# solomontesema/yolo-fpga-accelerator

Measured on AMD Instinct MI355X. Metric: YOLOv2 INT16 416x416 frames/sec, higher is better.
Workload: dtype int16

## Files before the change

### include/yolo2_hip.h

```cpp
#ifndef YOLO2_HIP_H
#define YOLO2_HIP_H

#include <stddef.h>
#include <stdint.h>

#ifdef __cplusplus
extern "C" {
#endif

#define YOLO2_SUCCESS     0
#define YOLO2_ERROR      -1
#define YOLO2_TIMEOUT    -2
#define YOLO2_INIT_ERROR -3
#define YOLO2_MMAP_ERROR -4
#define YOLO2_DMA_ERROR  -5


int  yolo2_accel_init(void);
void yolo2_accel_cleanup(void);
int  yolo2_hip_select_device(int device);
int  yolo2_hip_device_count(void);
const char *yolo2_hip_last_error(void);

void yolo2_set_q_values(int32_t qw, int32_t qa_in, int32_t qa_out, int32_t qb);
int  yolo2_is_busy(void);
int  yolo2_is_done(void);
int  yolo2_wait_for_completion(uint32_t timeout_ms);

uint32_t yolo2_get_status(void);
uint32_t yolo2_read_reg(uint32_t offset);
void     yolo2_write_reg(uint32_t offset, uint32_t value);
long yolo2_hip_driver_calls(void);

int yolo2_execute_conv_layer(uint64_t input_addr, uint64_t output_addr, uint64_t weight_addr,
                             uint64_t beta_addr, int ifm_num, int ofm_num, int ksize, int kstride,
                             int input_w, int input_h, int output_w, int output_h, int padding,
                             int is_nl, int is_bn, int tm, int tn, int tr, int tc, int ofm_num_bound,
                             int mloopsxTM, int mloops_a1xTM, int layer_type, int qw, int qa_in,
                             int qa_out, int qb, uint32_t timeout_ms);

int yolo2_execute_maxpool_layer(uint64_t input_addr, uint64_t output_addr, int channels, int ksize,
                                int kstride, int input_w, int input_h, int output_w, int output_h,
                                int padding, int tm, int tr, int tc, int ofm_num_bound, int mloopsxTM,
                                int mloops_a1xTM, uint32_t timeout_ms);

int yolo2_hip_last_layer_path(void);
int yolo2_hip_last_layer_edge(void);

int yolo2_execute_conv_layer_f32(uint64_t input_addr, uint64_t output_addr, uint64_t weight_addr,
                                 uint64_t beta_addr, int ifm_num, int ofm_num, int ksize, int kstride,
                                 int input_w, int input_h, int output_w, int output_h, int padding,
                                 int is_nl, uint32_t timeout_ms);

#ifndef DMA_BUFFER_MANAGER_H
typedef struct {
    void *ptr;
    size_t size;
    uint64_t phys_addr;
} memory_buffer_t;
typedef struct {
    void *virt_addr;
    uint64_t phys_addr;
    size_t size;
    int fd;
    char device_name[64];
} dma_buffer_t;
#endif
int      dma_buffer_init(void);
void     dma_buffer_cleanup(void);
int      dma_buffer_alloc(size_t size, dma_buffer_t *buffer);
void     dma_buffer_free(dma_buffer_t *buffer);
void     dma_buffer_sync_for_device(dma_buffer_t *buffer, size_t offset, size_t size);
void     dma_buffer_sync_for_cpu(dma_buffer_t *buffer, size_t offset, size_t size);
uint64_t dma_buffer_get_phys(dma_buffer_t *buffer, size_t offset);
int      memory_allocate_ddr(size_t size, size_t alignment, memory_buffer_t *buffer);
void     memory_free_ddr(memory_buffer_t *buffer);
int      memory_allocate_weights(size_t size, memory_buffer_t *buffer);
int      memory_allocate_bias(size_t size, memory_buffer_t *buffer);
int      memory_allocate_inference_buffer(memory_buffer_t *buffer);
uint64_t memory_get_phys_addr(void *virt_addr);
void     memory_flush_cache(void *addr, size_t size);
void     memory_invalidate_cache(void *addr, size_t size);

int  yolo2_hip_alloc(size_t bytes, uint64_t *dev_addr);
void yolo2_hip_free(uint64_t dev_addr);
int  yolo2_hip_memcpy_h2d(uint64_t dst, const void *src, size_t bytes);
int  yolo2_hip_memcpy_d2h(void *dst, uint64_t src, size_t bytes);
int  yolo2_hip_memset(uint64_t dst, int value, size_t bytes);


typedef struct yolo2_hip_ctx yolo2_hip_ctx;

#define YOLO2_N_CONV       23
#define YOLO2_N_WEIGHTS    50941792
#define YOLO2_N_BIAS       10761
#define YOLO2_REGION_ELEMS (425 * 13 * 13)
#define YOLO2_FRAME_ELEMS  (3 * 416 * 416)

int  yolo2_hip_create(int device, yolo2_hip_ctx **ctx);
void yolo2_hip_destroy(yolo2_hip_ctx *ctx);
int  yolo2_hip_ctx_device(yolo2_hip_ctx *ctx);
int  yolo2_hip_alloc_on(yolo2_hip_ctx *ctx, size_t bytes, uint64_t *dev_addr);

int yolo2_hip_load_weights_int16(yolo2_hip_ctx *ctx, const int16_t *weights_reorg, size_t n_weights,
                                 const int16_t *bias, size_t n_bias, const int32_t *weight_q,
                                 int n_weight_q, const int32_t *bias_q, int n_bias_q,
                                 const int32_t *act_q, int n_act_q);
int yolo2_hip_load_weights_int16_dev(yolo2_hip_ctx *ctx, uint64_t weights_reorg_dev, size_t n_weights,
                                     uint64_t bias_dev, size_t n_bias, const int32_t *weight_q,
                                     int n_weight_q, const int32_t *bias_q, int n_bias_q,
                                     const int32_t *act_q, int n_act_q);

int yolo2_hip_layer_path(yolo2_hip_ctx *ctx, int conv_ordinal);
int yolo2_hip_layer_path_counts(yolo2_hip_ctx *ctx, int conv_ordinal, int counts[5]);

int yolo2_hip_set_batch(yolo2_hip_ctx *ctx, int batch);

int yolo2_hip_run_batch_int16(yolo2_hip_ctx *ctx, uint64_t frames_dev, int batch,
                              uint64_t region_dev, int *final_q, void *stream);

int yolo2_hip_run_batch_int16_host(yolo2_hip_ctx *ctx, const float *frames, int batch,
                                   int16_t *region, int *final_q);

int yolo2_hip_run_frames_int16(yolo2_hip_ctx *ctx, const float *frames, int n_frames, int batch,
                               int16_t *region, int *final_q);

int yolo2_hip_load_weights_fp32(yolo2_hip_ctx *ctx, const float *weights_reorg, size_t n_weights,
                                const float *bias, size_t n_bias);
int yolo2_hip_load_weights_fp32_dev(yolo2_hip_ctx *ctx, uint64_t weights_reorg_dev, size_t n_weights,
                                    uint64_t bias_dev, size_t n_bias);
int yolo2_hip_run_batch_fp16(yolo2_hip_ctx *ctx, uint64_t frames_dev, int batch, uint64_t region_dev,
                             void *stream);
int yolo2_hip_run_batch_fp16_host(yolo2_hip_ctx *ctx, const float *frames, int batch, float *region);
const char *yolo2_hip_fp16_layer_kernel(yolo2_hip_ctx *ctx, int layer_idx);
int yolo2_hip_f16_store_check(int store, int pool, int B, int H, int W, int Cp_out, int out_ch_off, int n_store, int dst_B,
                              int dst_H, int dst_W, int dst_Cp);

int yolo2_hip_debug_layer_output(yolo2_hip_ctx *ctx, int layer_idx, int frame, int16_t *out,
                                 size_t capacity_elems, size_t *out_elems);

int yolo2_hip_debug_f16_tensor(yolo2_hip_ctx *ctx, int split, int layer_idx, int frame, int which, uint16_t *out,
                               size_t capacity_halves, int *geom);

int yolo2_hip_set_profiling(yolo2_hip_ctx *ctx, int enable);
int yolo2_hip_layer_times_ms(yolo2_hip_ctx *ctx, float *ms32 );

int yolo2_hip_num_lanes(yolo2_hip_ctx *ctx);
int yolo2_hip_num_lanes_fp16(yolo2_hip_ctx *ctx);
int yolo2_hip_set_fp16_lanes(yolo2_hip_ctx *ctx, int lanes);

int yolo2_hip_run_batch_f32tol(yolo2_hip_ctx *ctx, uint64_t frames_dev, int batch, uint64_t region_dev, void *stream);
int yolo2_hip_run_batch_f32tol_host(yolo2_hip_ctx *ctx, const float *frames, int batch, float *region);
const char *yolo2_hip_f32tol_layer_kernel(yolo2_hip_ctx *ctx, int layer_idx);
int yolo2_hip_num_lanes_f32tol(yolo2_hip_ctx *ctx);

int yolo2_hip_layer_pool_fused(yolo2_hip_ctx *ctx, int layer_idx);

int yolo2_hip_conv_launch_info(yolo2_hip_ctx *ctx, int conv_ordinal, int *grid_x, int *grid_y,
                               int *block, int *lds_bytes, int *pixels_per_lane);

int yolo2_hip_conv_plan_string(yolo2_hip_ctx *ctx, int conv_ordinal, char *buf, int cap);
int yolo2_hip_plan_source(yolo2_hip_ctx *ctx);

int yolo2_hip_set_option(yolo2_hip_ctx *ctx, const char *name, const char *value);
int yolo2_hip_options_string(yolo2_hip_ctx *ctx, char *buf, int cap);

int yolo2_hip_set_plan_cache(yolo2_hip_ctx *ctx, const char *path);
int yolo2_hip_plan_cache_info(yolo2_hip_ctx *ctx, uint64_t *weights_hash, int *bounds_from_file, int *n_lines, int *n_batches);
int yolo2_hip_plan_cache_check(const char *path, uint64_t weights_hash, int *n_lines);

int yolo2_hip_i16_plan_check(int splits, int cg_out, int npix, size_t cap_bytes);
size_t yolo2_hip_ks_scratch_bytes(yolo2_hip_ctx *ctx);
int yolo2_hip_i16_edge_map(int B, int H, int W, int cap, int *tile_cls, int *tile_mask, int *pix, long long *steps);

int yolo2_hip_run_frame_fp32_host(yolo2_hip_ctx *ctx, const float *frame, float *region);

int yolo2_hip_run_batch_fp32(yolo2_hip_ctx *ctx, uint64_t frames_dev, int batch, uint64_t region_dev, void *stream);
int yolo2_hip_run_batch_fp32_host(yolo2_hip_ctx *ctx, const float *frames, int batch, float *region);

int yolo2_hip_letterbox_u8(uint64_t image_dev, int w, int h, int channels, uint64_t frame_dev,
                           int net_w, int net_h, void *stream);

int yolo2_hip_run_images_u8_host(yolo2_hip_ctx *ctx, const uint8_t *const *images, const int *widths,
                                 const int *heights, int channels, int n, int batch,
                                 int16_t *region_host, int *final_q);

typedef struct {
    int frame, det, cls;
    float prob, x, y, w, h;
} yolo2_hip_det;
int yolo2_hip_postprocess_int16(yolo2_hip_ctx *ctx, uint64_t region_dev, int batch, int final_q, const int *im_w,
                                const int *im_h, float thresh, float nms, yolo2_hip_det *dets, int cap_per_frame,
                                int *counts, float *rows, int *totals, float *proc, void *stream);
int yolo2_hip_postprocess_f32(yolo2_hip_ctx *ctx, uint64_t region_dev, int batch, const int *im_w, const int *im_h,
                              float thresh, float nms, yolo2_hip_det *dets, int cap_per_frame, int *counts,
                              float *rows, int *totals, float *proc, void *stream);

#define YOLO2_DETS_BEST_CLASS 1
int yolo2_hip_run_images_u8_dets(yolo2_hip_ctx *ctx, const uint8_t *const *images, const int *widths, const int *heights,
                                 int channels, int n, int batch, float thresh, float nms, int flags, yolo2_hip_det *dets,
                                 int cap_per_frame, int *counts, int *final_q);

int yolo2_hip_run_images_u8_f16_host(yolo2_hip_ctx *ctx, int split, const uint8_t *const *images, const int *widths,
                                     const int *heights, int channels, int n, int batch, float *region_host);
int yolo2_hip_run_images_u8_dets_f16(yolo2_hip_ctx *ctx, int split, const uint8_t *const *images, const int *widths,
                                     const int *heights, int channels, int n, int batch, float thresh, float nms, int flags,
                                     yolo2_hip_det *dets, int cap_per_frame, int *counts);
const char *yolo2_hip_images_layer0_kernel(yolo2_hip_ctx *ctx, int split);

enum { YOLO2_PIX_GREY8 = 1, YOLO2_PIX_RGB24 = 3, YOLO2_PIX_YUYV = 0x56595559  };
int yolo2_hip_letterbox_pix(uint64_t image_dev, int w, int h, int pixfmt, uint64_t frame_dev, int net_w, int net_h, void *stream);
int yolo2_hip_run_images_pix_host(yolo2_hip_ctx *ctx, const uint8_t *const *images, const int *widths, const int *heights,
                                  int pixfmt, int n, int batch, int16_t *region_host, int *final_q);
int yolo2_hip_run_images_pix_dets(yolo2_hip_ctx *ctx, const uint8_t *const *images, const int *widths, const int *heights,
                                  int pixfmt, int n, int batch, float thresh, float nms, int flags, yolo2_hip_det *dets,
                                  int cap_per_frame, int *counts, int *final_q);
int yolo2_hip_run_images_pix_f16_host(yolo2_hip_ctx *ctx, int split, const uint8_t *const *images, const int *widths,
                                      const int *heights, int pixfmt, int n, int batch, float *region_host);
int yolo2_hip_run_images_pix_dets_f16(yolo2_hip_ctx *ctx, int split, const uint8_t *const *images, const int *widths,
                                      const int *heights, int pixfmt, int n, int batch, float thresh, float nms, int flags,
                                      yolo2_hip_det *dets, int cap_per_frame, int *counts);


int yolo2_hip_shard_range(int total, int rank, int world, int *lo, int *hi);

typedef struct yolo2_hip_multi yolo2_hip_multi;
int  yolo2_hip_multi_create(const int *devices, int n_devices, yolo2_hip_multi **m);
void yolo2_hip_multi_destroy(yolo2_hip_multi *m);
int  yolo2_hip_multi_num_devices(yolo2_hip_multi *m);
int  yolo2_hip_multi_uses_rccl(yolo2_hip_multi *m);
yolo2_hip_ctx *yolo2_hip_multi_ctx(yolo2_hip_multi *m, int i);
int  yolo2_hip_multi_load_weights_int16(yolo2_hip_multi *m, const int16_t *weights_reorg, size_t n_weights,
                                        const int16_t *bias, size_t n_bias, const int32_t *weight_q, int n_weight_q,
                                        const int32_t *bias_q, int n_bias_q, const int32_t *act_q, int n_act_q);
int  yolo2_hip_multi_load_weights_fp32(yolo2_hip_multi *m, const float *weights_reorg, size_t n_weights,
                                       const float *bias, size_t n_bias);
int  yolo2_hip_multi_run_frames_int16(yolo2_hip_multi *m, const float *frames, int n_frames, int batch_per_device,
                                      int16_t *region, int *final_q);
int  yolo2_hip_multi_run_images_u8_host(yolo2_hip_multi *m, const uint8_t *const *images, const int *widths,
                                        const int *heights, int channels, int n, int batch_per_device,
                                        int16_t *region_host, int *final_q);

int  yolo2_hip_multi_run_images_u8_dets(yolo2_hip_multi *m, const uint8_t *const *images, const int *widths, const int *heights,
                                        int channels, int n, int batch_per_device, float thresh, float nms, int flags,
                                        yolo2_hip_det *dets, int cap_per_frame, int *counts, int *final_q);
int  yolo2_hip_multi_run_images_u8_dets_f16(yolo2_hip_multi *m, int split, const uint8_t *const *images, const int *widths,
                                            const int *heights, int channels, int n, int batch_per_device, float thresh, float nms,
                                            int flags, yolo2_hip_det *dets, int cap_per_frame, int *counts);
int  yolo2_hip_multi_run_images_pix_host(yolo2_hip_multi *m, const uint8_t *const *images, const int *widths,
                                         const int *heights, int pixfmt, int n, int batch_per_device,
                                         int16_t *region_host, int *final_q);
int  yolo2_hip_multi_run_images_pix_dets(yolo2_hip_multi *m, const uint8_t *const *images, const int *widths, const int *heights,
                                         int pixfmt, int n, int batch_per_device, float thresh, float nms, int flags,
                                         yolo2_hip_det *dets, int cap_per_frame, int *counts, int *final_q);
int  yolo2_hip_multi_run_images_pix_dets_f16(yolo2_hip_multi *m, int split, const uint8_t *const *images, const int *widths,
                                             const int *heights, int pixfmt, int n, int batch_per_device, float thresh, float nms,
                                             int flags, yolo2_hip_det *dets, int cap_per_frame, int *counts);

int  yolo2_hip_rccl_unique_id(void *id128);
int  yolo2_hip_rccl_init_rank(yolo2_hip_ctx *ctx, int device, const void *id128, int nranks, int rank);
void yolo2_hip_rccl_finalize(yolo2_hip_ctx *ctx);
int  yolo2_hip_load_weights_int16_bcast(yolo2_hip_ctx *ctx, const int16_t *weights_reorg, size_t n_weights,
                                        const int16_t *bias, size_t n_bias, const int32_t *weight_q, int n_weight_q,
                                        const int32_t *bias_q, int n_bias_q, const int32_t *act_q, int n_act_q, int root);
int  yolo2_hip_load_weights_fp32_bcast(yolo2_hip_ctx *ctx, const float *weights_reorg, size_t n_weights,
                                       const float *bias, size_t n_bias, int root);

typedef struct {
    int nranks, rank, device;
    int version;
    int bcasts;
    double last_bcast_ms;
    uint64_t last_bcast_bytes;
    char lib_path[256];
} yolo2_hip_rccl_info_t;
int  yolo2_hip_rccl_info(yolo2_hip_ctx *ctx, yolo2_hip_rccl_info_t *out);
int  yolo2_hip_multi_rccl_info(yolo2_hip_multi *m, yolo2_hip_rccl_info_t *out);


int yolo2_hip_num_layers(void);
int yolo2_hip_layer_desc(int layer_idx, int desc[9]);

long yolo2_strip_int16_layer_pad(const int16_t *file, size_t file_elems, const int *layer_len,
                                 int n_layers, int16_t *dst);
extern const int yolo2_weight_len[YOLO2_N_CONV];
extern const int yolo2_bias_len[YOLO2_N_CONV];

#ifdef __cplusplus
}
#endif
#endif
```

### yolo-fpga-accelerator_amd/csrc/conv_common.hpp

```cpp
#pragma once
#include <hip/hip_runtime.h>
#include <cstdint>
#include <type_traits>

#include "layout.hpp"

namespace y2 {

typedef short short2_t __attribute__((ext_vector_type(2)));

struct ConvArgs {
    int B, H, W, Wp, PL;
    int CGin;
    int CGout;
    int npix;
    long in_cg_stride;
    long out_cg_stride;
    long out_base;
    int shift, round;
    int sh_right, sh_left;
    int bs_right, bs_left, bs_mag;
    int leaky;
    int lt_max;
    int xcd_remap;
    const int *mb_list;
    int nwin;
    int oWp, oPL;
    long pool_cg_stride;
    long pool_base;
    unsigned mHW, sHW, mW, sW, mOHW, sOHW, mOW, sOW;
    int ks_S, ks_Q, ks_mb;
    int *ks_trip;
    int edge;
    int e_nt, e_nb;
    int e_band[4];
    int e_int;
    int e_n[5];
    int e_rem[6];
    unsigned mH2, sH2, mW2, sW2, mI2, sI2;
};

inline void set_conv_div(ConvArgs &a)
{
    auto one = [](unsigned d, unsigned &m, unsigned &s) { if (d < 2) { m = 0; s = 32; } else fast_div_magic(d, m, s); };
    one((unsigned)(a.H * a.W), a.mHW, a.sHW);
    one((unsigned)a.W, a.mW, a.sW);
    one((unsigned)((a.H / 2) * (a.W / 2)), a.mOHW, a.sOHW);
    one((unsigned)(a.W / 2), a.mOW, a.sOW);
}
__device__ __forceinline__ int div_c(int n, unsigned m, unsigned s) { return s >= 32 ? n : (int)fast_div((unsigned)n, m, s); }

__device__ __forceinline__ int leaky_i16(int v)
{
    const unsigned u = (unsigned)(-v);
    const int q = (int)((u * 52429u) >> 19);
    return v < 0 ? -q : v;
}

__device__ __forceinline__ int clamp16(int v) { return min(max(v, -32768), 32767); }

__device__ __forceinline__ long shift64(long v, int right, int left, int mag, long round)
{
    if (right) return (v + round) >> mag;
    if (left) return (long)((unsigned long)v << mag);
    return v;
}

__device__ __forceinline__ int flat_of(const ConvArgs &a, int q)
{
    const int b = div_c(q, a.mHW, a.sHW);
    const int r = q - b * (a.H * a.W);
    const int y = div_c(r, a.mW, a.sW);
    const int x = r - y * a.W;
    return b * a.PL + (y + 1) * a.Wp + x;
}

enum { kEdgeTop = 0, kEdgeBottom = 1, kEdgeLeft = 2, kEdgeRight = 3, kEdgeInterior = 4, kEdgeMixed = 5 };

__host__ __device__ constexpr int edge_class_mask(int cls)
{
    return cls == kEdgeTop ? 0x1f8 : cls == kEdgeBottom ? 0x03f : cls == kEdgeLeft ? 0x1b6 : cls == kEdgeRight ? 0x0db : 0x1ff;
}

__host__ __device__ inline unsigned edge_div(unsigned n, unsigned m, unsigned s)
{
    if (s >= 32) return n;
    const unsigned t = (unsigned)(((unsigned long long)m * n) >> 32);
    return (t + ((n - t) >> 1)) >> s;
}

__host__ __device__ inline int edge_tile_class(const ConvArgs &a, int tile, int &ct)
{
    const unsigned nb = (unsigned)a.e_nb, nt = (unsigned)a.e_nt;
    const int c0 = (int)((unsigned)tile * nb / nt), c1 = (int)((unsigned)(tile + 1) * nb / nt);
    if (c1 > c0) {
        int c = 0;
        while (c < 3 && c0 >= a.e_band[c]) ++c;
        ct = c0 - (c ? a.e_band[c - 1] : 0);
        return c;
    }
    const int o = tile - c0;
    if (o < a.e_int) { ct = o; return kEdgeInterior; }
    ct = o - a.e_int;
    return kEdgeMixed;
}

__host__ __device__ inline bool edge_lane_pixel(const ConvArgs &a, int cls, int ct, int lane, int &b, int &y, int &x)
{
    int i = ct * 64 + lane;
    bool valid = true;
    if (cls == kEdgeMixed) {
        const int nm = a.e_rem[5];
        valid = i < nm;
        if (!valid) i = nm - 1;
        int c = 0;
        while (c < 4 && i >= a.e_rem[c + 1]) ++c;
        i = a.e_n[c] - (a.e_rem[c + 1] - a.e_rem[c]) + (i - a.e_rem[c]);
        cls = c;
    }
    if (cls == kEdgeTop || cls == kEdgeBottom) {
        b = (int)edge_div((unsigned)i, a.mW, a.sW);
        x = i - b * a.W;
        y = cls == kEdgeTop ? 0 : a.H - 1;
    } else if (cls == kEdgeLeft || cls == kEdgeRight) {
        b = (int)edge_div((unsigned)i, a.mH2, a.sH2);
        y = 1 + i - b * (a.H - 2);
        x = cls == kEdgeLeft ? 0 : a.W - 1;
    } else {
        b = (int)edge_div((unsigned)i, a.mI2, a.sI2);
        const int r = i - b * ((a.H - 2) * (a.W - 2));
        const int yy = (int)edge_div((unsigned)r, a.mW2, a.sW2);
        y = 1 + yy;
        x = 1 + r - yy * (a.W - 2);
    }
    return valid;
}

constexpr int kEdgeGatherItems = 3 * 64 * 3;

__host__ __device__ inline void edge_band_patch(const ConvArgs &a, int cls, int &org, int &Lf, int &pitch)
{
    const bool rows = cls == kEdgeTop || cls == kEdgeBottom;
    Lf = rows ? 2 * a.Wp + 1 : 2 * a.H;
    pitch = rows ? a.Wp : 2;
    org = cls == kEdgeTop ? a.Wp - 1 : cls == kEdgeBottom ? (a.H - 1) * a.Wp - 1 : cls == kEdgeLeft ? a.Wp : a.Wp + a.W - 2;
}

inline int edge_tiles_plan(ConvArgs &a)
{
    a.edge = 0;
    if (a.H < 3 || a.W < 3) return 0;
    const long B = a.B, H = a.H, W = a.W;
    const long n[5] = {B * W, B * W, B * (H - 2), B * (H - 2), B * (H - 2) * (W - 2)};
    if (n[4] + 2 * n[0] + 2 * n[2] >= (1L << 30)) return 0;
    a.e_rem[0] = 0;
    int nb = 0;
    for (int c = 0; c < 5; ++c) {
        a.e_n[c] = (int)n[c];
        a.e_rem[c + 1] = a.e_rem[c] + (int)(n[c] % 64);
        if (c < 4) { nb += (int)(n[c] / 64); a.e_band[c] = nb; }
    }
    a.e_int = (int)(n[4] / 64);
    a.e_nb = nb;
    a.e_nt = nb + a.e_int + (a.e_rem[5] + 63) / 64;
    if ((unsigned long long)a.e_nt * (unsigned long long)(a.e_nb + 1) >= (1ULL << 32)) return 0;
    auto magic = [](unsigned d, unsigned &m, unsigned &s) { if (d < 2) { m = 0; s = 32; } else fast_div_magic(d, m, s); };
    magic((unsigned)(H - 2), a.mH2, a.sH2);
    magic((unsigned)(W - 2), a.mW2, a.sW2);
    magic((unsigned)((H - 2) * (W - 2)), a.mI2, a.sI2);
    int lt = kEdgeGatherItems;
    for (int c = kEdgeTop; c <= kEdgeRight; ++c) {
        int org, Lf, pitch;
        edge_band_patch(a, c, org, Lf, pitch);
        for (int t = 0; t < a.e_band[c] - (c ? a.e_band[c - 1] : 0); ++t) {
            int b0, b1, y, x;
            edge_lane_pixel(a, c, t, 0, b0, y, x);
            edge_lane_pixel(a, c, t, 63, b1, y, x);
            lt = lt > (b1 - b0 + 1) * Lf ? lt : (b1 - b0 + 1) * Lf;
        }
    }
    for (int t = 0; t < a.e_int; ++t) {
        int b0, y0, x0, b1, y1, x1;
        edge_lane_pixel(a, kEdgeInterior, t, 0, b0, y0, x0);
        edge_lane_pixel(a, kEdgeInterior, t, 63, b1, y1, x1);
        const int f0 = b0 * a.PL + (y0 + 1) * a.Wp + x0, f1 = b1 * a.PL + (y1 + 1) * a.Wp + x1;
        lt = lt > f1 - f0 + 1 + 2 * (a.Wp + 1) ? lt : f1 - f0 + 1 + 2 * (a.Wp + 1);
    }
    a.edge = 1;
    return lt;
}

inline long edge_tiles_steps(const ConvArgs &a)
{
    return 64L * (6L * a.e_nb + 9L * (a.e_nt - a.e_nb));
}

__device__ inline void xcd_partition(int xm_log2, int &tile, int &yb)
{
    const int gx = gridDim.x, gy = gridDim.y, total = gx * gy;
    const int lin = blockIdx.x + blockIdx.y * gx;
    const int xcd = lin & 7, slot = lin >> 3;
    const int q = total >> 3, r = total & 7;
    int L = xcd * q + min(xcd, r) + slot;
    const int Xm = 1 << xm_log2, Xt = 8 >> xm_log2;
    const int qt = gx / Xt, rt = gx - qt * Xt, qm = gy / Xm, rm = gy - qm * Xm;
    tile = 0; yb = 0;
    for (int k = 0; k < 8; ++k) {
        const int kt = k >> xm_log2, km = k & (Xm - 1);
        const int nt = qt + (kt < rt), nm = qm + (km < rm), cnt = nt * nm;
        if (L < cnt) {
            const int dt = L / nm;
            tile = kt * qt + min(kt, rt) + dt;
            yb = km * qm + min(km, rm) + (L - dt * nm);
            break;
        }
        L -= cnt;
    }
}

template <typename T>
__global__ void k_repack_weights(const T *__restrict__ src, T *__restrict__ dst, int C, int N, int KK)
{
    const int CG = (C + kTn - 1) / kTn, MB = (N + kTm - 1) / kTm;
    const long n = (long)MB * CG * KK * 128;
    const long t = (long)blockIdx.x * blockDim.x + threadIdx.x;
    if (t >= n) return;
    const int tn = (int)(t & 3), tm = (int)((t >> 2) & 31);
    const long r = t >> 7;
    const int tap = (int)(r % KK);
    const int cg = (int)((r / KK) % CG);
    const int mb = (int)(r / ((long)KK * CG));
    const int m0 = mb * kTm, n0 = cg * kTn;
    const int tm_min = min(kTm, N - m0), tn_min = min(kTn, C - n0);
    T v = 0;
    if (tm < tm_min && tn < tn_min)
        v = src[(long)m0 * C * KK + (long)tm_min * n0 * KK + (long)tap * tm_min * tn_min + tm * tn_min + tn];
    dst[t] = v;
}

template <typename T>
__global__ void k_pool_ref(const T *__restrict__ in, T *__restrict__ out, int C, int K, int stride, int W, int H,
                           int OW, int OH, T padv)
{
    const int t = blockIdx.x * blockDim.x + threadIdx.x;
    if (t >= C * OH * OW) return;
    const int x = t % OW, y = (t / OW) % OH, c = t / (OW * OH);
    const int W8 = (W + 7) & ~7, OW8 = (OW + 7) & ~7;
    T best = padv;
    for (int i = 0; i < K; ++i)
        for (int j = 0; j < K; ++j) {
            const int sy = y * stride + i, sx = x * stride + j;
            const T v = (sy < H && sx < W) ? in[((long)c * H + sy) * W8 + sx] : padv;
            if (v > best) best = v;
        }
    out[((long)c * OH + y) * OW8 + x] = best;
}

}
```

### yolo-fpga-accelerator_amd/csrc/kernels_int16.hpp

```cpp
#pragma once

#include "conv_common.hpp"
#include "layout.hpp"

namespace y2 {


__device__ __forceinline__ int stepA(int acc, const int2 x, const int2 w, const int r, const int s)
{
    int d = __builtin_amdgcn_sdot2(__builtin_bit_cast(short2_t, x.x), __builtin_bit_cast(short2_t, w.x), r, false);
    d = __builtin_amdgcn_sdot2(__builtin_bit_cast(short2_t, x.y), __builtin_bit_cast(short2_t, w.y), d, false);
    return clamp16(acc + (d >> s));
}

__device__ __forceinline__ void stepC4(int &acc01, int &acc23, const int2 x, const int2 w0, const int2 w1, const int2 w2,
                                       const int2 w3, const int r, const int s)
{
    int t0, t1, t2, t3;
    asm("v_dot2_i32_i16 %2, %6, %14, %16\n\t"
        "v_dot2_i32_i16 %3, %7, %14, %16\n\t"
        "v_dot2_i32_i16 %4, %8, %14, %16\n\t"
        "v_dot2_i32_i16 %5, %9, %14, %16\n\t"
        "v_dot2_i32_i16 %2, %10, %15, %2\n\t"
        "v_dot2_i32_i16 %3, %11, %15, %3\n\t"
// ... 95 lines not shown

__device__ __forceinline__ long step64(long acc, int2 x, int2 w, const ConvArgs &a)
{
    const int x0 = (short)(x.x & 0xffff), x1 = x.x >> 16, x2 = (short)(x.y & 0xffff), x3 = x.y >> 16;
    const int w0 = (short)(w.x & 0xffff), w1 = w.x >> 16, w2 = (short)(w.y & 0xffff), w3 = w.y >> 16;
    const long p = (long)(w0 * x0) + (long)(w1 * x1) + (long)(w2 * x2) + (long)(w3 * x3);
    long v = acc + shift64(p, a.sh_right, a.sh_left, a.shift, a.sh_right && a.shift > 0 ? (1L << (a.shift - 1)) : 0);
    v = v > 32767 ? 32767 : v;
    v = v < -32768 ? -32768 : v;
    return v;
}



#ifndef PREX_MAX_P
#define PREX_MAX_P 2
#endif
#ifndef Y2_I16_ABL
#define Y2_I16_ABL 0
#endif
template <int KS, int P, int MODE, int NST, int GRP = 1, bool EDGE = false>
__global__ __launch_bounds__(256, 2) void k_conv_i16(const int2 *__restrict__ in, int2 *__restrict__ out,
                                                   const int2 *__restrict__ wpk,
                                                   const short *__restrict__ bias, const ConvArgs a)
{
    static_assert(!EDGE || (KS == 3 && P == 1 && GRP == 1 && (MODE == 3 || MODE == 4)), "edge-class tiles: forms C / D, P = 1, 3x3");
    extern __shared__ int2 lds[];
    constexpr bool X64 = MODE == 2;
    typedef typename std::conditional<X64, long, int>::type acc_t;
    constexpr int T = 64 * P;
    constexpr int KT = KS * KS;
    constexpr int KK = KT * GRP;
    constexpr int PFG = KS == 1 ? GRP : 1;
    static_assert(GRP == 1 || KS == 1 || (KS == 3 && GRP == 2), "grouping: 1x1 convs (8 groups per barrier); 3x3 with 2 groups works but measured slower, not launched");
    const int tid = threadIdx.x;
    const int lane = tid & 63;
    const int wave = __builtin_amdgcn_readfirstlane(tid >> 6);
    int tile = blockIdx.x, yb = blockIdx.y;
    if (a.xcd_remap) xcd_partition(a.xcd_remap - 1, tile, yb);
    const int mb = a.mb_list ? a.mb_list[yb] : yb;
    const int halo = (KS == 3) ? a.Wp + 1 : 0;
    int fo[P];
    int rowaddr[P][KS];
    bool valid[P];
    int tile_start, Lt;
    int ecls = kEdgeInterior;
    int soff[NST], loff[NST];
    if (EDGE) {
        int ct, b, y, x;
        ecls = edge_tile_class(a, tile, ct);
        valid[0] = edge_lane_pixel(a, ecls, ct, lane, b, y, x);
        fo[0] = b * a.PL + (y + 1) * a.Wp + x;
        if (ecls == kEdgeInterior) {
            const int fmin = __builtin_amdgcn_readfirstlane(fo[0]), fmax = __builtin_amdgcn_readlane(fo[0], 63);
            tile_start = fmin - halo;
            Lt = min(fmax - fmin + 1 + 2 * halo, a.lt_max);
            const int lo = fo[0] - tile_start;
#pragma unroll
            for (int i = 0; i < KS; ++i) rowaddr[0][i] = (lo + (i - 1) * a.Wp - 1) * 8;
#pragma unroll
            for (int k = 0; k < NST; ++k) { soff[k] = tile_start + tid + k * 256; loff[k] = tid + k * 256; }
        } else if (ecls != kEdgeMixed) {
            const int b0 = __builtin_amdgcn_readfirstlane(b), b1 = __builtin_amdgcn_readlane(b, 63);
            const bool rows = ecls == kEdgeTop || ecls == kEdgeBottom;
            int org, Lf, pitch;
            edge_band_patch(a, ecls, org, Lf, pitch);
            tile_start = 0;
            Lt = min((b1 - b0 + 1) * Lf, a.lt_max);
            const int lo = (b - b0) * Lf + (rows ? fo[0] - b * a.PL - org : 2 * y + (ecls == kEdgeRight));
#pragma unroll
            for (int i = 0; i < KS; ++i) rowaddr[0][i] = (lo + (i - 1) * pitch - 1) * 8;
#pragma unroll
            for (int k = 0; k < NST; ++k) {
                const int s_ = tid + k * 256, fr = s_ / Lf, r_ = s_ - fr * Lf;
                soff[k] = (b0 + fr) * a.PL + org + (rows ? r_ : (r_ >> 1) * a.Wp + (r_ & 1));
                loff[k] = s_;
            }
        } else {
            tile_start = 0;
            Lt = kEdgeGatherItems;
#pragma unroll
            for (int i = 0; i < KS; ++i) rowaddr[0][i] = (i * 64 + lane) * 3 * 8;
#pragma unroll
            for (int k = 0; k < NST; ++k) {
                const int t = wave + 4 * k, ti = t / 3, tj = t - 3 * ti;
                soff[k] = fo[0] + (ti - 1) * a.Wp + (tj - 1);
                loff[k] = (ti * 64 + lane) * 3 + tj;
            }
        }
    } else {
        const int q0 = tile * T;
        const int qlast = min(q0 + T, a.npix) - 1;
        const int fmin = flat_of(a, q0);
        const int fmax = flat_of(a, qlast);
        tile_start = fmin - halo;
        Lt = min(fmax - fmin + 1 + 2 * halo, a.lt_max);
#pragma unroll
        for (int p = 0; p < P; ++p) {
            const int q = q0 + p * 64 + lane;
            valid[p] = q <= qlast;
            fo[p] = flat_of(a, min(q, qlast));
            const int lo = fo[p] - tile_start;
#pragma unroll
            for (int i = 0; i < KS; ++i)
                rowaddr[p][i] = (KS == 3) ? (lo + (i - 1) * a.Wp - 1) * 8 : lo * 8;
        }
    }

    acc_t acc[P][8];
    {
        const short *bp = bias + mb * 32 + wave * 8;
#pragma unroll
        for (int m = 0; m < 8; ++m) {
            acc_t b0;
            if (X64) {
                b0 = (acc_t)shift64((long)bp[m], a.bs_right, a.bs_left, a.bs_mag,
                                    a.bs_right && a.bs_mag > 0 ? (1L << (a.bs_mag - 1)) : 0);
            } else {
                const int b = bp[m];
                b0 = a.bs_right ? (acc_t)((b + (a.bs_mag > 0 ? (1 << (a.bs_mag - 1)) : 0)) >> a.bs_mag)
                                : (a.bs_left ? (acc_t)(b << a.bs_mag) : (acc_t)b);
                if (MODE == 1) b0 = (acc_t)(((int)b0 << a.shift) + a.round);
            }
#pragma unroll
            for (int p = 0; p < P; ++p) acc[p][m] = b0;
        }
        if (MODE == 5) {
#pragma unroll
            for (int p = 0; p < P; ++p)
#pragma unroll
                for (int m = 0; m < 8; ++m) acc[p][m] = (acc_t)((int)acc[p][m] << 16);
        }
        if (MODE == 3 || MODE == 4) {
            int pk[4];
#pragma unroll
            for (int j = 0; j < 4; ++j) pk[j] = ((int)acc[0][2 * j] & 0xffff) | ((int)acc[0][2 * j + 1] << 16);
#pragma unroll
            for (int p = 0; p < P; ++p)
#pragma unroll
                for (int j = 0; j < 4; ++j) acc[p][j] = (acc_t)pk[j];
        }
    }

    const int r = a.round, s = a.shift;
    const int nmask = ~((1 << s) - 1), lo_b = (int)(0xffff8000u << s) + r, hi_b = (32767 << s) + r;
    int r_vgpr = r;
    if (MODE != 2) asm volatile("" : "+v"(r_vgpr));
    const char *lds_b = reinterpret_cast<const char *>(lds);
    const int2 *src = in + kLead + (EDGE ? 0 : tile_start);
    const int2 *wq = wpk + ((long)mb * a.CGin * KT * 32 + wave * 8);

    int2 stage[NST];
    const int buf_items = a.lt_max * GRP;
    auto src_off = [&](int i) -> long { if (GRP == 1) return i; const int g = i / Lt; return (long)g * a.in_cg_stride + (i - g * Lt); };
    auto lds_off = [&](int i) -> int { if (GRP == 1) return i; const int g = i / Lt; return g * a.lt_max + (i - g * Lt); };
    const int LtG = Lt * GRP;
#pragma unroll
    for (int k = 0; k < NST; ++k) {
        const int i = tid + k * 256;
        if (i < LtG) stage[k] = src[EDGE ? soff[k] : src_off(i)];
    }
#pragma unroll
    for (int k = 0; k < NST; ++k) {
        const int i = tid + k * 256;
        if (i < LtG) lds[EDGE ? loff[k] : lds_off(i)] = stage[k];
    }
    __syncthreads();

    int chain = 0;
#if (Y2_I16_ABL & 8)
    int2 abl_w[8];
#pragma unroll
    for (int m = 0; m < 8; ++m) abl_w[m] = wq[m];
#endif
#if (Y2_I16_ABL & 16)
    int2 abl_x = lds[tid & 63];
#endif
    const int niter = a.CGin / GRP;
    auto group_loop = [&](auto mask_c) __attribute__((always_inline)) {
    constexpr int MASK = decltype(mask_c)::value;
    for (int cg = 0; cg < niter; ++cg) {
        src += (cg + 1 < niter) ? a.in_cg_stride * GRP : 0;
#if !(Y2_I16_ABL & 2)
#pragma unroll
        for (int k = 0; k < NST; ++k) {
            const int i = tid + k * 256;
            if (i < LtG) stage[k] = src[EDGE ? soff[k] : src_off(i)];
        }
#endif
        const char *tile = lds_b + (cg & 1) * buf_items * 8;
        constexpr bool PREX = (MODE == 3 || MODE == 4 || MODE == 5) && P <= PREX_MAX_P;
        auto xaddr = [&](int t, int p) -> const int2 * {
            return reinterpret_cast<const int2 *>(tile + (t / KT) * (a.lt_max * 8) + rowaddr[p][(t % KT) / KS] + ((t % KT) % KS) * 8);
        };
#pragma unroll
        for (int gb = 0; gb < GRP / PFG; ++gb) {
        int2 xv[PREX ? KT * PFG : 1][P];
        if (PREX && !(Y2_I16_ABL & 16)) {
#pragma unroll
            for (int tt = 0; tt < KT * PFG; ++tt)
#pragma unroll
                for (int p = 0; p < P; ++p) if ((MASK >> (tt % KT)) & 1) xv[tt][p] = *xaddr(gb * KT * PFG + tt, p);
        }
#pragma unroll
        for (int tt = 0; tt < KT * PFG; ++tt) {
            if (!((MASK >> (tt % KT)) & 1)) continue;
            const int tap = gb * KT * PFG + tt;
            int2 w[8];
#if (Y2_I16_ABL & 8)
#pragma unroll
            for (int m = 0; m < 8; ++m) { w[m] = abl_w[m]; asm volatile("" : "+s"(w[m].x), "+s"(w[m].y)); }
#else
#pragma unroll
            for (int m = 0; m < 8; ++m) w[m] = wq[tap * 32 + m];
#endif
#pragma unroll
            for (int p = 0; p < P; ++p) {
                int2 x;
#if (Y2_I16_ABL & 16)
                x = abl_x; asm volatile("" : "+v"(x.x), "+v"(x.y));
#else
                if (PREX) x = xv[tt][p];
                else x = *xaddr(tap, p);
#endif
                if (MODE == 0) asm volatile("" : "+v"(x.x) : "v"(chain));
                if (MODE == 5) {
                    int ae[8];
#pragma unroll
                    for (int m = 0; m < 8; ++m) ae[m] = (int)acc[p][m];
                    stepE8(ae, x, w, r_vgpr);
#pragma unroll
                    for (int m = 0; m < 8; ++m) acc[p][m] = (acc_t)ae[m];
                } else if (MODE == 4) {
                    int a01 = (int)acc[p][0], a23 = (int)acc[p][1], a45 = (int)acc[p][2], a67 = (int)acc[p][3];
                    stepD8(a01, a23, a45, a67, x, w, r_vgpr, 0x07060302);
                    acc[p][0] = (acc_t)a01; acc[p][1] = (acc_t)a23; acc[p][2] = (acc_t)a45; acc[p][3] = (acc_t)a67;
                } else if (MODE == 3) {
                    int a01 = (int)acc[p][0], a23 = (int)acc[p][1], a45 = (int)acc[p][2], a67 = (int)acc[p][3];
                    stepC4(a01, a23, x, w[0], w[1], w[2], w[3], r_vgpr, s);
                    stepC4(a45, a67, x, w[4], w[5], w[6], w[7], r_vgpr, s);
                    acc[p][0] = (acc_t)a01; acc[p][1] = (acc_t)a23; acc[p][2] = (acc_t)a45; acc[p][3] = (acc_t)a67;
                } else
#pragma unroll
                for (int m = 0; m < 8; ++m) {
                    if (MODE == 2) acc[p][m] = (acc_t)step64((long)acc[p][m], x, w[m], a);
                    else if (MODE == 1) acc[p][m] = (acc_t)stepB((int)acc[p][m], x, w[m], nmask, r_vgpr, lo_b, hi_b);
                    else acc[p][m] = (acc_t)stepA((int)acc[p][m], x, w[m], r_vgpr, s);
                }
                if (MODE == 0) chain = (int)acc[p][7];
            }
            if (MODE == 0) __builtin_amdgcn_sched_barrier(0);
        }
        }
#if !(Y2_I16_ABL & 2)
        {
            int2 *nxt = lds + ((cg + 1) & 1) * buf_items;
#pragma unroll
            for (int k = 0; k < NST; ++k) {
                const int i = tid + k * 256;
                if (i < LtG) nxt[EDGE ? loff[k] : lds_off(i)] = stage[k];
            }
        }
#endif
#if !(Y2_I16_ABL & 1)
        wq += KK * 32;
#else
        asm volatile("" : "+s"(wq));
#endif
#if !(Y2_I16_ABL & 4)
        __syncthreads();
#endif
    }
    };
    if (!EDGE) {
        group_loop(std::integral_constant<int, 0x1ff>());
    } else {
        switch (ecls) {
        case kEdgeTop: group_loop(std::integral_constant<int, edge_class_mask(kEdgeTop)>()); break;
        case kEdgeBottom: group_loop(std::integral_constant<int, edge_class_mask(kEdgeBottom)>()); break;
        case kEdgeLeft: group_loop(std::integral_constant<int, edge_class_mask(kEdgeLeft)>()); break;
        case kEdgeRight: group_loop(std::integral_constant<int, edge_class_mask(kEdgeRight)>()); break;
        default: group_loop(std::integral_constant<int, 0x1ff>()); break;
        }
    }

#pragma unroll
    for (int g = 0; g < 2; ++g) {
        const int cgo = mb * 8 + wave * 2 + g;
        if (cgo >= a.CGout) continue;
        int2 *dst = out + a.out_base + (long)cgo * a.out_cg_stride;
#pragma unroll
        for (int p = 0; p < P; ++p) {
            int v[4];
#pragma unroll
            for (int t = 0; t < 4; ++t) {
                int e = (int)acc[p][g * 4 + t];
                if (MODE == 1) e >>= s;
                if (MODE == 5) e >>= 16;
                if (MODE == 3 || MODE == 4) {
                    const int pr = (int)acc[p][(g * 4 + t) >> 1];
                    e = (t & 1) ? (pr >> 16) : (int)(short)(pr & 0xffff);
                }
                v[t] = a.leaky ? leaky_i16(e) : e;
            }
            int2 o;
            o.x = (v[0] & 0xffff) | (v[1] << 16);
            o.y = (v[2] & 0xffff) | (v[3] << 16);
            if (valid[p]) dst[fo[p]] = o;
        }
    }
}

template <int KS, int P, int MODE, int NST>
__global__ __launch_bounds__(128, 4) void k_conv_i16_w16(const int2 *__restrict__ in, int2 *__restrict__ out, const int2 *__restrict__ wpk,
                                                          const short *__restrict__ bias, const ConvArgs a)
{
    static_assert(MODE == 3 || MODE == 4, "packed-accumulator forms only");
    extern __shared__ int2 lds[];
    constexpr int T = 64 * P, KT = KS * KS;
    const int tid = threadIdx.x, lane = tid & 63;
    const int wave = __builtin_amdgcn_readfirstlane(tid >> 6);
    int tile = blockIdx.x, yb = blockIdx.y;
    if (a.xcd_remap) xcd_partition(a.xcd_remap - 1, tile, yb);
    const int mb = a.mb_list ? a.mb_list[yb] : yb;
    const int q0 = tile * T, qlast = min(q0 + T, a.npix) - 1;
    const int halo = (KS == 3) ? a.Wp + 1 : 0;
    const int fmin = flat_of(a, q0), fmax = flat_of(a, qlast);
    const int tile_start = fmin - halo;
    const int Lt = min(fmax - fmin + 1 + 2 * halo, a.lt_max);

    int fo[P], rowaddr[P][KS];
    bool valid[P];
#pragma unroll
    for (int p = 0; p < P; ++p) {
        const int q = q0 + p * 64 + lane;
        valid[p] = q <= qlast;
        fo[p] = flat_of(a, min(q, qlast));
        const int lo = fo[p] - tile_start;
#pragma unroll
        for (int i = 0; i < KS; ++i) rowaddr[p][i] = (KS == 3) ? (lo + (i - 1) * a.Wp - 1) * 8 : lo * 8;
// ... 787 lines not shown
```

### yolo-fpga-accelerator_amd/csrc/y2_internal.hpp

```cpp
#pragma once
#include <hip/hip_runtime.h>

#include <algorithm>
#include <cstdint>
#include <cstdio>
#include <cstdlib>
#include <cstring>
#include <map>
#include <memory>
#include <mutex>
#include <string>
#include <utility>
#include <vector>

#include "../../include/yolo2_hip.h"
#include "conv_common.hpp"
#include "layout.hpp"


int y2_fail(int code, const char *fmt, ...) __attribute__((format(printf, 2, 3)));
#define fail y2_fail

#define HIP_TRY(expr, code)                                                                      \
    do {                                                                                         \
        hipError_t e_ = (expr);                                                                  \
        if (e_ != hipSuccess) return fail(code, "%s failed: %s (%s:%d)", #expr, hipGetErrorString(e_), __FILE__, __LINE__); \
    } while (0)


struct Y2Options {
    int autotune = -1;
    std::string plan_file;
    std::string plan_write;
    int lanes = 0;
    bool no_lanes = false;
    std::string lane_split;
    int lane_priority = 1;
    bool verbose = false;
    bool no_plan_cache = false;
    int splitk = -1;
    int poolfuse = -1;
    bool no_poolfuse = false, no_hiacc = false, no_ks = false, no_w16 = false, no_grp = false, grp16 = false, no_xcd_remap = false, splitk_no_pack = false,
         no_edge_tiles = false;
    int f16_lanes = 2;
    bool f16_no_lanes = false, f16_no_mfma0 = false, f16_no_glds = false, f16_no_poolfuse = false, f16_no_halo = false, f16_no_persist = false,
         f16_persist_all = false, f16_ring_all = false, f16_no_ring = false, f16_no_c32 = false, f16_m16 = false, f16_w8 = false, f16_no_wide = false,
         f16_no_fuse1x1 = false, f16_no_rw = false, f16_no_rwb = false, f16_no_rwc = false, f16_ring256 = false, f16_ring_sq = false;
    int stamp_layer = -1;
    int f16_skip = 0;
    int force_path = -1, force_p = 0, force_ks = 0, f32_p = 0;
    bool force_w16 = false, force_hiacc = false;

    static Y2Options from_env();
    int set(const char *name, const char *value);
    std::string describe() const;
    bool steered() const { return splitk >= 0 || poolfuse >= 0 || no_poolfuse || no_w16 || no_hiacc || no_ks || no_grp || no_xcd_remap; }
};
const Y2Options &y2_process_options();


struct Y2PlanLine { int path, P, pad, splitk, pp, w16, fuse, hiacc, ks; };
typedef std::pair<int, std::pair<int, int>> Y2PlanKey;
bool y2_plan_line_parse(const char *text, Y2PlanKey *key, Y2PlanLine *pl);
bool y2_plan_table_has_batch(const Y2Options &opt, int B);
bool y2_plan_table_lookup(const Y2Options &opt, int B, int L, int S, Y2PlanLine *out);

bool y2_ks_fits(int splits, int cg_out, int npix, size_t cap_bytes);
size_t y2_ks_bytes(int splits, int cg_out, int npix);

struct Y2PlanCache {
    std::mutex mu;
    std::string path;
    uint64_t hash = 0;
    bool bounds_valid = false;
    struct Bounds { int maxsum = 0, maxbias = 0; std::vector<int> sum_mb, bias_mb, abs_mb, form, scale; };
    Bounds bounds[YOLO2_N_CONV];
    std::map<Y2PlanKey, Y2PlanLine> lines;
    std::map<int, int> per_batch;
    bool dirty = false;
    bool load(uint64_t want_hash, std::string *why);
    bool save();
};
uint64_t y2_hash_bytes(uint64_t seed, const void *data, size_t n);


enum LType { L_CONV, L_MAX, L_ROUTE, L_REORG, L_REGION };
struct LayerDesc {
    LType type;
    int c, h, w, n, size, leaky;
};
extern const LayerDesc kNet[32];

static inline unsigned blocks_for(long n, int bs) { return (unsigned)((n + bs - 1) / bs); }
static inline int round_up(int v, int m) { return (v + m - 1) / m * m; }
static inline long packed_weight_elems(int C, int N, int K)
{
    return (long)((N + y2::kTm - 1) / y2::kTm) * ((C + y2::kTn - 1) / y2::kTn) * K * K * 128;
}


constexpr int kMaxTileItems = 2048;

struct ConvPlan {
    int C = 0, N = 0, K = 0, H = 0, W = 0, leaky = 0;
    int Qw = 0, Qa_in = 0, Qa_out = 0, Qb = 0;
    int path = 0;
    int P = 8;
    int mb_count = 0;
    int splitk_ok = 0;
    int splitk = 0;
    int splitk_pp = 1;
    int splitk_pack = 0;
    size_t ks_cap = 0;
    int ks = 0;
    int hiacc = 0;
    int w16 = 0;
    int grp = 1;
    int pool_fused = 0;
    int lds_pad = 0;
    dim3 grid;
    int lds_bytes = 0;
    y2::ConvArgs args;
};


struct Tensor {
    y2::ActGeom g;
    int2 *d = nullptr;
};

struct Y2PostBufs {
    int cap_frames = 0;
    size_t cap_dets = 0;
    float *rows = nullptr, *rows2 = nullptr;
    int *totals = nullptr, *counts = nullptr;
    void *geom = nullptr;
    yolo2_hip_det *dets = nullptr;
};

struct PipeBufs {
    size_t host_in = 0, dev_in = 0;
    int batch = 0;
    uint8_t *hin[2] = {nullptr, nullptr}, *dbytes[2] = {nullptr, nullptr};
    float *din[2] = {nullptr, nullptr};
    int16_t *hout[2] = {nullptr, nullptr}, *dout[2] = {nullptr, nullptr};
    hipStream_t s_in = nullptr, s_run = nullptr, s_out = nullptr;
    hipEvent_t e_in[2] = {nullptr, nullptr}, e_run[2] = {nullptr, nullptr}, e_out[2] = {nullptr, nullptr};
    hipEvent_t e_lane[2][8] = {};
    int post_batch = 0, post_cap = 0;
    Y2PostBufs post[2];
    uint8_t *hgeom[2] = {nullptr, nullptr};
    yolo2_hip_det *hdets[2] = {nullptr, nullptr};
    int *hcounts[2] = {nullptr, nullptr};
    int regf_batch = 0;
    float *dregf[2] = {nullptr, nullptr}, *hregf[2] = {nullptr, nullptr};
};

struct F16Plan;

struct yolo2_hip_ctx {
    PipeBufs pipe;
    int device = 0;
    Y2Options opt;
    std::shared_ptr<Y2PlanCache> plan_cache;
    bool weights_loaded = false;
    short *wpk = nullptr;
    short *bias_pk = nullptr;
    long wpk_off[YOLO2_N_CONV], bias_off[YOLO2_N_CONV];
    int maxsum[YOLO2_N_CONV], maxbias[YOLO2_N_CONV];
    std::vector<int> weight_q, bias_q, act_q;
    ConvPlan plan[32];
    std::vector<ConvPlan> extra[32];
    std::vector<int> maxsum_mb[YOLO2_N_CONV], maxbias_mb[YOLO2_N_CONV], maxabs_mb[YOLO2_N_CONV];
    std::vector<signed char> wscale_mb[YOLO2_N_CONV];
    std::vector<signed char> form_mb[YOLO2_N_CONV];
    int *mb_lists = nullptr;
    int plan_source = 0;
    int *ks_trip = nullptr;
    size_t ks_trip_bytes = 0;
    std::vector<yolo2_hip_ctx *> lanes;
    std::vector<int> lane_first;
    std::vector<yolo2_hip_ctx *> f16_lanes;
    bool is_lane = false, laned = false;
    hipStream_t lane_stream = nullptr;
    hipEvent_t ev_fork = nullptr, ev_join = nullptr;
    bool fuse_pool[32] = {false};
    ConvPlan fplan[32];
    std::vector<ConvPlan> fextra[32];
    int path_counts[YOLO2_N_CONV][5];
    int reorg_shift = 0, final_q = 0;
    int batch = 0;
    Tensor t_in, t_out[32], t_cat;
    struct HalfTensor {
        int C = 0, Cp = 0, H = 0, W = 0, Wp = 0, PL = 0, B = 0;
        size_t items = 0;
        _Float16 *d = nullptr;
    };
    bool f16_loaded = false;
    bool split = false;
    bool borrows_f32 = false;
    yolo2_hip_ctx *tol = nullptr;
    _Float16 *wh = nullptr;
    float *biasf = nullptr;
    float *w0f = nullptr;
    float *wf32 = nullptr, *bf32 = nullptr;
    F16Plan *f16_plan = nullptr;
    std::string images_l0[2];
    float *wpkf = nullptr, *biasf32_pk = nullptr;
    long wpkf_off[YOLO2_N_CONV], biasf32_off[YOLO2_N_CONV];
    struct FTensor {
        y2::ActGeom g;
        float4 *d = nullptr;
    };
    int f32_batch = 0;
    FTensor f_in, f_out[32], f_cat;
    ConvPlan fp32_plan[32];
    long wh_off[YOLO2_N_CONV], biasf_off[YOLO2_N_CONV];
    int f16_batch = 0;
    int f16_last_batch = 0;
    bool f16_last_laned = false;
    HalfTensor h_in, h_out[32], h_cat;
    static constexpr int kProfSlots = 32;
    bool prof = false;
    hipEvent_t ev[kProfSlots][33];
    bool ev_made = false;
    long prof_runs = 0;
};


void y2_free_activations(yolo2_hip_ctx *c);
void y2_free_f16_activations(yolo2_hip_ctx *c);
void y2_free_f32_activations(yolo2_hip_ctx *c);
void y2_destroy_lanes(yolo2_hip_ctx *c);
int y2_lane_stream_create(hipStream_t *s);
bool y2_lane0_own_stream();
int y2_ensure_prof_events(yolo2_hip_ctx *c);
int y2_ensure(void **p, size_t *cap, size_t need);

void y2_f16_plan_free(yolo2_hip_ctx *c);
int y2_f16_images_ctx(yolo2_hip_ctx *c, int split, yolo2_hip_ctx **run);
bool y2_f16_images_fused(const yolo2_hip_ctx *run);
int y2_f16_run_images(yolo2_hip_ctx *run, const uint8_t *lb, bool yuyv, int batch, float *region_dev, hipStream_t st);
const char *y2_f16_images_kernel(const yolo2_hip_ctx *run, bool yuyv);

int y2_drv_conv_i16(const short *in, short *out, const short *w, const short *beta, int ifm, int ofm, int ksize, int kstride,
                    int iw, int ih, int ow, int oh, int pad, int is_nl, int qw, int qa_in, int qa_out, int qb, int *path_out);
void y2_drv_pool_i16(const short *in, short *out, int channels, int ksize, int kstride, int iw, int ih, int ow, int oh);
void y2_drv_release_i16(void);
void y2_drv_conv_f32(const float *in, float *out, const float *w, const float *beta, int ifm, int ofm, int ksize, int kstride, int iw,
                     int ih, int ow, int oh, int pad, int is_nl);

int y2_post_alloc(int device, int batch, int cap, Y2PostBufs *b);
void y2_post_free(Y2PostBufs *b);
size_t y2_post_geom_bytes(void);
int y2_post_fill_geom(void *geom_host, const int *im_w, const int *im_h, int n);
int y2_post_enqueue_int16(int device, const int16_t *region_dev, int batch, int final_q, float thresh, float nms, int cap, int best_only,
                          Y2PostBufs *b, hipStream_t st);
int y2_post_enqueue_f32(const float *region_dev, int batch, float thresh, float nms, int cap, int best_only, Y2PostBufs *b, hipStream_t st,
                        float *proc_dev = nullptr, float **final_rows = nullptr);
```

### yolo-fpga-accelerator_amd/csrc/yolo2_int16.hip

```cpp
#include <hip/hip_runtime.h>

#include <dlfcn.h>

#include <algorithm>
#include <cstdio>
#include <cstdlib>
#include <cstring>
#include <map>
#include <mutex>
#include <string>
#include <type_traits>
#include <vector>

#include "y2_internal.hpp"
#include "kernels_int16.hpp"

using namespace y2;

constexpr int kKsMaxBatch = 4;


struct ShiftSpec {
    int right, left, mag;
};
static ShiftSpec make_shift(int s)
{
    ShiftSpec sh;
    sh.right = s > 0;
    sh.left = s < 0;
    int a = sh.right ? s : (sh.left ? -s : 0);
    sh.mag = a > 30 ? 30 : a;
    return sh;
}

static int choose_path(int so, int sb, int maxsum, int max_abs_bias, int max_abs_w = -1, int force = -1)
{
    if (so < 0) return 2;
    const ShiftSpec o = make_shift(so), b = make_shift(sb);
    const long long round = o.mag > 0 ? (1LL << (o.mag - 1)) : 0;
    long long bias0 = max_abs_bias;
    if (b.right) bias0 = ((bias0 + (b.mag > 0 ? (1LL << (b.mag - 1)) : 0)) >> b.mag) + 1;
    else if (b.left) bias0 = bias0 << b.mag;
    const long long accmax = std::max<long long>(32768, bias0);
    const long long pmax = (long long)maxsum * 32768;
    if (bias0 > 2147483647LL) return 2;
    int path = 2;
    const bool okA = pmax + round + accmax <= 2147483647LL;
    const bool okB = (accmax << o.mag) + round + pmax <= 2147483647LL;
    const bool okC = okA && bias0 <= 32767 && ((pmax + round) >> o.mag) <= 32767;
    const int k = 16 - so;
    const bool okD = okC && max_abs_w >= 0 && k >= 0 && k <= 15 && ((long long)max_abs_w << k) <= 32767 &&
                     (((long long)maxsum << k) * 32768 + 32768) <= 2147483647LL;
    if (okA) path = 0;
    if (okB) path = 1;
    if (okC) path = 3;
    if (okD) path = 4;
    if (force >= 0) {
        const int f = force;
        if (f == 2 || (f == 0 && okA) || (f == 1 && okB) || (f == 3 && okC) || (f == 4 && okD)) path = f;
    }
    return path;
}

static void plan_conv(ConvPlan &p, const ActGeom &gin, long out_cg_stride, long out_base, int CGout, const Y2Options &opt, int forceP = 0)
{
    const ShiftSpec so = make_shift(p.Qa_in + p.Qw - p.Qa_out), sb = make_shift(p.Qb - p.Qa_out);
    const int npix = gin.B * gin.H * gin.W;
    const int maxP = (p.path == 1 || p.path == 3 || p.path == 4) ? 8 : 4;
    if (forceP) {
        p.P = std::min(forceP, maxP);
    } else {
        p.P = maxP;
        while (p.P > 1 && (long)((npix + 64 * p.P - 1) / (64 * p.P)) * (p.mb_count ? p.mb_count : (p.N + 31) / 32) < 1024) p.P >>= 1;
    }
    const int halo = p.K == 3 ? gin.Wp + 1 : 0;
    while (p.P > 1 && tile_items_bound(gin, 64 * p.P, halo) > kMaxTileItems) p.P >>= 1;
    if (p.splitk) {
        if (p.splitk_pp > 1 && !(p.splitk == 4 && p.K == 3 && p.path == 4 && !opt.splitk_no_pack)) p.splitk_pp = 1;
        const int S = p.splitk, lt = tile_items_bound(gin, 64 / S * p.splitk_pp, halo);
        if ((S != 4 && !(S == 8 && p.K == 1)) || gin.CG % S != 0 || gin.CG < 4 * S || S * (lt + p.K * p.K * 32) > kMaxTileItems) p.splitk = 0;
    }
    if (p.ks) {
        if (p.splitk || p.mb_count || p.path != 4 || p.K != 3 || gin.CG % p.ks != 0 || gin.CG / p.ks < 2 || tile_items_bound(gin, 64, halo) > kMaxTileItems ||
            !y2_ks_fits(p.ks, CGout, npix, p.ks_cap))
            p.ks = 0;
        else { p.P = 1; p.w16 = 0; p.hiacc = 0; }
    }
    if (p.splitk) p.P = 1;
    p.splitk_pack = p.splitk && p.path == 4 && !opt.splitk_no_pack;
    if (p.w16 && (p.splitk || p.K != 3 || (p.path != 3 && p.path != 4) || p.P > 2 || tile_items_bound(gin, 64 * p.P, halo) > 1024)) p.w16 = 0;
    const int T = p.splitk ? 64 / p.splitk * p.splitk_pp : 64 * p.P;
    ConvArgs &a = p.args;
    a.B = gin.B; a.H = gin.H; a.W = gin.W; a.Wp = gin.Wp; a.PL = gin.PL;
    a.CGin = gin.CG;
    a.CGout = CGout;
    a.npix = npix;
    set_conv_div(a);
    a.in_cg_stride = gin.cg_stride;
    a.out_cg_stride = out_cg_stride;
    a.out_base = out_base;
    a.shift = so.mag;
    a.round = (so.right && so.mag > 0) ? (1 << (so.mag - 1)) : 0;
    if (p.path == 4) { a.shift = 16; a.round = 32768; }
    a.sh_right = so.right; a.sh_left = so.left;
    a.bs_right = sb.right; a.bs_left = sb.left; a.bs_mag = sb.mag;
    a.leaky = p.leaky;
    a.lt_max = tile_items_bound(gin, T, halo);
    if (p.w16) p.lds_pad = 0;
    if (p.hiacc && (p.path != 4 || p.splitk || p.w16 || p.P > 4)) p.hiacc = 0;
    p.grp = (!p.splitk && p.K == 1 && p.path != 2 && gin.CG % 8 == 0 && a.lt_max * 8 <= kMaxTileItems && !opt.no_grp) ? 8 : 1;
    if (p.grp == 8 && opt.grp16 && gin.CG % 16 == 0 && a.lt_max * 16 <= kMaxTileItems && p.P <= 2 && (p.path == 3 || p.path == 4) && !p.hiacc) p.grp = 16;
    p.lds_bytes = p.splitk ? p.splitk * (a.lt_max + p.K * p.K * 32 + 4) * 8 * 2 : std::max(a.lt_max * p.grp * 8 * 2, p.lds_pad);
    p.grid = dim3((npix + T - 1) / T, p.mb_count ? p.mb_count : (p.N + 31) / 32, 1);
    a.ks_S = p.ks; a.ks_Q = p.ks ? gin.CG / p.ks : 0; a.ks_mb = (int)p.grid.y;
    if (p.ks) { p.grid.y *= p.ks; p.lds_pad = 0; }
    a.edge = 0;
    if (!opt.no_edge_tiles && p.K == 3 && p.P == 1 && p.grp == 1 && (p.path == 3 || p.path == 4) && !p.hiacc && !p.w16 && !p.splitk && !p.ks) {
        ConvArgs e = a;
        const int lt = edge_tiles_plan(e);
        if (lt > 0 && lt <= kMaxTileItems) {
            a = e;
            a.lt_max = lt;
            p.lds_bytes = std::max(lt * 8 * 2, p.lds_pad);
            p.grid.x = a.e_nt;
        }
    }
    a.xcd_remap = 0;
    if (!opt.no_xcd_remap) {
        const double in_bytes = (double)gin.B * gin.CG * gin.PL * 8;
        const double w_mb = (double)gin.CG * p.K * p.K * 32 * 8;
        const int gy = (int)p.grid.y, gx = (int)p.grid.x;
        double best = 0;
        for (int lg = 0; lg < 4; ++lg) {
            const int Xm = 1 << lg, Xt = 8 >> lg;
            if (Xm > gy || Xt > gx) continue;
            const int own = (gy + Xm - 1) / Xm;
            double G = 1;
            if (own * w_mb > 3.0e6) G = std::max(1.0, ((double)gx / Xt) / std::max(1, 128 / own));
            const double cost = in_bytes * Xm + w_mb * gy * Xt * G;
            if (!a.xcd_remap || cost < best) { best = cost; a.xcd_remap = 1 + lg; }
        }
    }
}

static int pool_tile_items_bound(const ActGeom &g)
{
    const int OW = g.W / 2, OHW = (g.H / 2) * OW;
    const int wraps = std::min(63, (63 + OW - 1) / OW), frames = std::min(63, (63 + OHW - 1) / OHW);
    return 126 + wraps * (g.W + 2) + frames * (g.W + 1) + 3 * g.Wp + 4;
}

static bool plan_conv_pool(ConvPlan &p, const ActGeom &gin, const ActGeom &gpool, int full)
{
    if (p.K != 3 || (p.path != 3 && p.path != 4) || (gin.H & 1) || (gin.W & 1)) return false;
    const int lt = pool_tile_items_bound(gin);
    if (lt > 12 * 256) return false;
    ConvArgs &a = p.args;
    p.splitk = 0; p.splitk_pp = 1; p.grp = 1; p.P = 4; p.lds_pad = 0; p.w16 = 0; p.hiacc = 0; p.ks = 0;
    a.edge = 0;
    p.pool_fused = full ? 2 : 1;
    a.lt_max = lt;
    a.nwin = gin.B * (gin.H / 2) * (gin.W / 2);
    a.oWp = gpool.Wp; a.oPL = gpool.PL;
    a.pool_cg_stride = gpool.cg_stride;
    a.pool_base = kLead;
    p.lds_bytes = lt * 8 * (gin.CG > 1 ? 2 : 1);
    p.grid = dim3((a.nwin + 63) / 64, p.mb_count ? p.mb_count : (p.N + 31) / 32, 1);
    return true;
}

template <int MODE, bool FULL>
static void launch_conv_pool_n(const ConvPlan &p, const int2 *in, int2 *out, int2 *out_pool, const int2 *wpk, const short *bias,
                               hipStream_t st)
{
    const int nst = (p.args.lt_max + 255) / 256;
#define Y2_POOL(NSTV, SINGLEV) hipLaunchKernelGGL((k_conv_i16_pool<MODE, NSTV, FULL, SINGLEV>), p.grid, dim3(256), p.lds_bytes, st, in, out, out_pool, wpk, bias, p.args)
    if (p.args.CGin == 1) {
        if (nst <= 4) Y2_POOL(4, true);
        else Y2_POOL(12, true);
    } else if (nst <= 2) Y2_POOL(2, false);
    else if (nst <= 3) Y2_POOL(3, false);
    else if (nst <= 5) Y2_POOL(5, false);
    else if (nst <= 8) Y2_POOL(8, false);
    else Y2_POOL(12, false);
#undef Y2_POOL
}

template <int KS, int MODE, int P>
static void launch_conv_n(const ConvPlan &p, const int2 *in, int2 *out, const int2 *wpk, const short *bias, hipStream_t st)
{
    const int nst = (p.args.lt_max * p.grp + 255) / 256;
    if (KS == 1 && p.grp == 16 && (MODE == 3 || MODE == 4) && P <= 2) {
        hipLaunchKernelGGL((k_conv_i16<1, (P <= 2 ? P : 1), (MODE == 3 || MODE == 4) ? MODE : 3, 8, KS == 1 ? 16 : 1>), p.grid, dim3(256), p.lds_bytes, st, in, out, wpk, bias, p.args);
        return;
    }
    if (KS == 1 && p.grp == 8 && MODE != 2) {
        if (nst <= 4) hipLaunchKernelGGL((k_conv_i16<1, P, MODE == 2 ? 1 : MODE, 4, KS == 1 ? 8 : 1>), p.grid, dim3(256), p.lds_bytes, st, in, out, wpk, bias, p.args);
        else hipLaunchKernelGGL((k_conv_i16<1, P, MODE == 2 ? 1 : MODE, 8, KS == 1 ? 8 : 1>), p.grid, dim3(256), p.lds_bytes, st, in, out, wpk, bias, p.args);
        return;
    }
    if (nst <= 2) hipLaunchKernelGGL((k_conv_i16<KS, P, MODE, 2>), p.grid, dim3(256), p.lds_bytes, st, in, out, wpk, bias, p.args);
    else if (nst <= 4) hipLaunchKernelGGL((k_conv_i16<KS, P, MODE, 4>), p.grid, dim3(256), p.lds_bytes, st, in, out, wpk, bias, p.args);
    else hipLaunchKernelGGL((k_conv_i16<KS, P, MODE, 8>), p.grid, dim3(256), p.lds_bytes, st, in, out, wpk, bias, p.args);
}

template <int MODE>
static void launch_conv_edge(const ConvPlan &p, const int2 *in, int2 *out, const int2 *wpk, const short *bias, hipStream_t st)
{
    const int nst = (p.args.lt_max + 255) / 256;
    if (nst <= 3) hipLaunchKernelGGL((k_conv_i16<3, 1, MODE, 3, 1, true>), p.grid, dim3(256), p.lds_bytes, st, in, out, wpk, bias, p.args);
    else hipLaunchKernelGGL((k_conv_i16<3, 1, MODE, 8, 1, true>), p.grid, dim3(256), p.lds_bytes, st, in, out, wpk, bias, p.args);
}

template <int KS, int MODE>
static void launch_conv_p(const ConvPlan &p, const int2 *in, int2 *out, const int2 *wpk, const short *bias,
                          hipStream_t st)
{
    switch (p.P) {
    case 8: launch_conv_n<KS, MODE, 8>(p, in, out, wpk, bias, st); break;
    case 4: launch_conv_n<KS, MODE, 4>(p, in, out, wpk, bias, st); break;
    case 2: launch_conv_n<KS, MODE, 2>(p, in, out, wpk, bias, st); break;
    default: launch_conv_n<KS, MODE, 1>(p, in, out, wpk, bias, st); break;
    }
}

static int launch_conv(const ConvPlan &p, const int2 *in, int2 *out, const int2 *wpk, const short *bias, hipStream_t st,
                       int2 *out_pool = nullptr, int *ks_trip = nullptr, size_t ks_trip_bytes = 0)
{
    if (p.pool_fused) {
        if (p.path == 4) {
            if (p.pool_fused == 2) launch_conv_pool_n<4, true>(p, in, out, out_pool, wpk, bias, st);
            else launch_conv_pool_n<4, false>(p, in, out, out_pool, wpk, bias, st);
        } else {
            if (p.pool_fused == 2) launch_conv_pool_n<3, true>(p, in, out, out_pool, wpk, bias, st);
            else launch_conv_pool_n<3, false>(p, in, out, out_pool, wpk, bias, st);
        }
        return YOLO2_SUCCESS;
    }
    if (p.ks) {
        if (!ks_trip || !y2_ks_fits(p.ks, p.args.CGout, p.args.npix, ks_trip_bytes))
            return fail(YOLO2_ERROR, "conv plan asks for a K-split over %d workgroups but the context's triple scratch holds %zu bytes (needs %zu): not launched",
                        p.ks, ks_trip ? ks_trip_bytes : (size_t)0, y2_ks_bytes(p.ks, p.args.CGout, p.args.npix));
        ConvArgs a = p.args;
        a.ks_trip = ks_trip;
        const int nst = (a.lt_max + 255) / 256;
        if (nst <= 2) hipLaunchKernelGGL((k_conv_i16_ks<3, 2>), p.grid, dim3(256), p.lds_bytes, st, in, wpk, a);
        else if (nst <= 4) hipLaunchKernelGGL((k_conv_i16_ks<3, 4>), p.grid, dim3(256), p.lds_bytes, st, in, wpk, a);
        else hipLaunchKernelGGL((k_conv_i16_ks<3, 8>), p.grid, dim3(256), p.lds_bytes, st, in, wpk, a);
        hipLaunchKernelGGL(k_ks_finalize, dim3(blocks_for((long)a.npix * a.CGout, 256)), dim3(256), 0, st, (const int *)ks_trip, out, bias, a);
        return YOLO2_SUCCESS;
    }
    if (p.w16) {
        const int nst = (p.args.lt_max + 127) / 128;
#define Y2_W16(PV, MODEV, NSTV) hipLaunchKernelGGL((k_conv_i16_w16<3, PV, MODEV, NSTV>), p.grid, dim3(128), p.lds_bytes, st, in, out, wpk, bias, p.args)
#define Y2_W16_N(PV, MODEV) do { if (nst <= 2) Y2_W16(PV, MODEV, 2); else if (nst <= 4) Y2_W16(PV, MODEV, 4); else Y2_W16(PV, MODEV, 8); } while (0)
        if (p.path == 4) { if (p.P == 2) Y2_W16_N(2, 4); else Y2_W16_N(1, 4); }
        else { if (p.P == 2) Y2_W16_N(2, 3); else Y2_W16_N(1, 3); }
#undef Y2_W16_N
#undef Y2_W16
        return YOLO2_SUCCESS;
    }
    if (p.splitk) {
        const int nst = (p.splitk * (p.args.lt_max + p.K * p.K * 32) + 255) / 256;
        const bool pack = p.splitk_pack != 0;
#define Y2_SPLITK(KSV, NSTV, PACKV, SV) \
    hipLaunchKernelGGL((k_conv_i16_splitk<KSV, NSTV, PACKV, SV>), p.grid, dim3(256), p.lds_bytes, st, in, out, wpk, bias, p.args)
#define Y2_SPLITK_S(KSV, NSTV, PACKV) do { if (p.splitk == 8) Y2_SPLITK(KSV, NSTV, PACKV, 8); else Y2_SPLITK(KSV, NSTV, PACKV, 4); } while (0)
        if (pack) {
            if (p.K == 3 && p.splitk_pp == 4) hipLaunchKernelGGL((k_conv_i16_splitk<3, 8, true, 4, 4>), p.grid, dim3(256), p.lds_bytes, st, in, out, wpk, bias, p.args);
            else if (p.K == 3 && p.splitk_pp == 2) hipLaunchKernelGGL((k_conv_i16_splitk<3, 8, true, 4, 2>), p.grid, dim3(256), p.lds_bytes, st, in, out, wpk, bias, p.args);
            else if (p.K == 3) Y2_SPLITK(3, 8, true, 4);
            else if (nst <= 2) Y2_SPLITK_S(1, 2, true);
            else Y2_SPLITK_S(1, 8, true);
        } else {
            if (p.K == 3) Y2_SPLITK(3, 8, false, 4);
            else if (nst <= 2) Y2_SPLITK_S(1, 2, false);
            else Y2_SPLITK_S(1, 8, false);
        }
#undef Y2_SPLITK_S
#undef Y2_SPLITK
        return YOLO2_SUCCESS;
    }
    if (p.K == 3) {
        if (p.args.edge && p.path == 4) launch_conv_edge<4>(p, in, out, wpk, bias, st);
        else if (p.args.edge && p.path == 3) launch_conv_edge<3>(p, in, out, wpk, bias, st);
        else if (p.path == 2) launch_conv_p<3, 2>(p, in, out, wpk, bias, st);
        else if (p.path == 4 && p.hiacc) launch_conv_p<3, 5>(p, in, out, wpk, bias, st);
        else if (p.path == 4) launch_conv_p<3, 4>(p, in, out, wpk, bias, st);
        else if (p.path == 3) launch_conv_p<3, 3>(p, in, out, wpk, bias, st);
        else if (p.path == 1) launch_conv_p<3, 1>(p, in, out, wpk, bias, st);
        else launch_conv_p<3, 0>(p, in, out, wpk, bias, st);
    } else {
        if (p.path == 2) launch_conv_p<1, 2>(p, in, out, wpk, bias, st);
        else if (p.path == 4 && p.hiacc) launch_conv_p<1, 5>(p, in, out, wpk, bias, st);
        else if (p.path == 4) launch_conv_p<1, 4>(p, in, out, wpk, bias, st);
        else if (p.path == 3) launch_conv_p<1, 3>(p, in, out, wpk, bias, st);
        else if (p.path == 1) launch_conv_p<1, 1>(p, in, out, wpk, bias, st);
        else launch_conv_p<1, 0>(p, in, out, wpk, bias, st);
    }
    return YOLO2_SUCCESS;
}

static int resolve_q(yolo2_hip_ctx *c)
{
    std::vector<int> lists;
    const int na = (int)c->act_q.size();
    int current_Qa = na ? c->act_q[0] : 0, route24_q = 0, pending = -1, ord = 0;
    c->reorg_shift = 0;
    for (int i = 0; i < 32; ++i) {
        const LayerDesc &l = kNet[i];
        if (l.type == L_CONV) {
// ... 223 lines not shown
    } else {
    HIP_TRY(hipMemcpy(c->maxsum, bound, sizeof(int) * YOLO2_N_CONV, hipMemcpyDeviceToHost), YOLO2_DMA_ERROR);
    {
        std::vector<int> hm(mb_total), ha(mb_total);
        HIP_TRY(hipMemcpy(hm.data(), bound_mb, sizeof(int) * mb_total, hipMemcpyDeviceToHost), YOLO2_DMA_ERROR);
        HIP_TRY(hipMemcpy(ha.data(), bound_abs, sizeof(int) * mb_total, hipMemcpyDeviceToHost), YOLO2_DMA_ERROR);
        int o = 0;
        for (int i = 0; i < 32; ++i)
            if (kNet[i].type == L_CONV) {
                const int MB = (kNet[i].n + 31) / 32;
                c->maxsum_mb[o].assign(hm.begin() + mb_offs[o], hm.begin() + mb_offs[o] + MB);
                c->maxabs_mb[o].assign(ha.begin() + mb_offs[o], ha.begin() + mb_offs[o] + MB);
                o++;
            }
    }
    }
    (void)hipFree(bound);
    (void)hipFree(bound_mb);
    (void)hipFree(bound_abs);
    {
        const int rq = resolve_q(c);
        if (rq) return rq;
    }
    if (pc) {
        std::lock_guard<std::mutex> lk(pc->mu);
        if (bounds_cached) {
            bool same = true;
            for (int o = 0; o < YOLO2_N_CONV && same; ++o)
                for (size_t mb = 0; mb < c->form_mb[o].size() && same; ++mb)
                    same = pc->bounds[o].form[mb] == c->form_mb[o][mb] && pc->bounds[o].scale[mb] == c->wscale_mb[o][mb];
            if (!same) { pc->lines.clear(); pc->per_batch.clear(); }
            pc->bounds_valid = true;
        } else if (pc->hash) {
            pc->lines.clear();
            pc->per_batch.clear();
            pc->bounds_valid = false;
        }
        for (int o = 0; o < YOLO2_N_CONV; ++o) {
            Y2PlanCache::Bounds &b = pc->bounds[o];
            b.maxsum = c->maxsum[o]; b.maxbias = c->maxbias[o];
            b.sum_mb = c->maxsum_mb[o]; b.bias_mb = c->maxbias_mb[o]; b.abs_mb = c->maxabs_mb[o];
            b.form.assign(c->form_mb[o].begin(), c->form_mb[o].end());
            b.scale.assign(c->wscale_mb[o].begin(), c->wscale_mb[o].end());
        }
    }
    c->weights_loaded = true;
    if (c->batch) {
        const int b = c->batch;
        c->batch = 0;
        return yolo2_hip_set_batch(c, b);
    }
    return YOLO2_SUCCESS;
}

extern "C" int yolo2_hip_load_weights_int16_dev(yolo2_hip_ctx *c, uint64_t weights_reorg_dev, size_t n_weights,
                                                uint64_t bias_dev, size_t n_bias, const int32_t *weight_q, int n_weight_q,
                                                const int32_t *bias_q, int n_bias_q, const int32_t *act_q, int n_act_q)
{
    if (!c) return fail(YOLO2_ERROR, "null ctx");
    if (!weights_reorg_dev || !bias_dev || !weight_q || !bias_q || !act_q) return fail(YOLO2_ERROR, "null argument");
    HIP_TRY(hipSetDevice(c->device), YOLO2_INIT_ERROR);
    return load_common(c, (const short *)(uintptr_t)weights_reorg_dev, n_weights, (const short *)(uintptr_t)bias_dev, n_bias,
                       weight_q, n_weight_q, bias_q, n_bias_q, act_q, n_act_q);
}

extern "C" int yolo2_hip_load_weights_int16(yolo2_hip_ctx *c, const int16_t *weights_reorg, size_t n_weights,
                                            const int16_t *bias, size_t n_bias, const int32_t *weight_q, int n_weight_q,
                                            const int32_t *bias_q, int n_bias_q, const int32_t *act_q, int n_act_q)
{
    if (!c) return fail(YOLO2_ERROR, "null ctx");
    if (!weights_reorg || !bias || !weight_q || !bias_q || !act_q) return fail(YOLO2_ERROR, "null argument");
    if (n_weights < YOLO2_N_WEIGHTS) return fail(YOLO2_ERROR, "weights file too small");
    if (n_bias < YOLO2_N_BIAS) return fail(YOLO2_ERROR, "bias file too small");
    HIP_TRY(hipSetDevice(c->device), YOLO2_INIT_ERROR);
    short *wd = nullptr, *bd = nullptr;
    HIP_TRY(hipMalloc((void **)&wd, (size_t)YOLO2_N_WEIGHTS * 2), YOLO2_MMAP_ERROR);
    HIP_TRY(hipMalloc((void **)&bd, (size_t)YOLO2_N_BIAS * 2), YOLO2_MMAP_ERROR);
    HIP_TRY(hipMemcpy(wd, weights_reorg, (size_t)YOLO2_N_WEIGHTS * 2, hipMemcpyHostToDevice), YOLO2_DMA_ERROR);
    HIP_TRY(hipMemcpy(bd, bias, (size_t)YOLO2_N_BIAS * 2, hipMemcpyHostToDevice), YOLO2_DMA_ERROR);
    const int rc = load_common(c, wd, YOLO2_N_WEIGHTS, bd, YOLO2_N_BIAS, weight_q, n_weight_q, bias_q, n_bias_q, act_q, n_act_q);
    (void)hipDeviceSynchronize();
    (void)hipFree(wd);
    (void)hipFree(bd);
    return rc;
}

extern "C" int yolo2_hip_layer_path(yolo2_hip_ctx *c, int ord)
{
    if (!c || !c->weights_loaded || ord < 0 || ord >= YOLO2_N_CONV) return -1;
    int o = 0;
    for (int i = 0; i < 32; ++i)
        if (kNet[i].type == L_CONV) {
            if (o == ord) return c->plan[i].path;
            o++;
        }
    return -1;
}

extern "C" int yolo2_hip_layer_path_counts(yolo2_hip_ctx *c, int ord, int counts[5])
{
    if (!c || !c->weights_loaded || ord < 0 || ord >= YOLO2_N_CONV || !counts) return YOLO2_ERROR;
    for (int k = 0; k < 5; ++k) counts[k] = c->path_counts[ord][k];
    return YOLO2_SUCCESS;
}

static int alloc_tensor(Tensor &t, int C, int H, int W, int B)
{
    t.g = make_geom(C, H, W, B);
    HIP_TRY(hipMalloc((void **)&t.d, (size_t)t.g.items * 8), YOLO2_MMAP_ERROR);
    HIP_TRY(hipMemset(t.d, 0, (size_t)t.g.items * 8), YOLO2_DMA_ERROR);
    return YOLO2_SUCCESS;
}

static int autotune(yolo2_hip_ctx *c)
{
    hipEvent_t e0, e1;
    HIP_TRY(hipEventCreate(&e0), YOLO2_ERROR);
    HIP_TRY(hipEventCreate(&e1), YOLO2_ERROR);
    const size_t flush_bytes = (size_t)64 << 20;
    void *flush = nullptr;
    HIP_TRY(hipMalloc(&flush, flush_bytes), YOLO2_MMAP_ERROR);
    int ord = 0;
    for (int i = 0; i < 32; ++i) {
        if (kNet[i].type != L_CONV) continue;
        const Tensor &tin = i == 0 ? c->t_in : (i == 26 ? c->t_out[16] : (i == 29 ? c->t_cat : c->t_out[i - 1]));
        const Tensor &tout = c->t_out[i];
        const long out_base = kLead + (i == 24 ? (long)64 * tout.g.cg_stride : 0);
        const int CGout = (kNet[i].n + 3) / 4;
        std::vector<ConvPlan *> subs{&c->plan[i]};
        for (auto &e : c->extra[i]) subs.push_back(&e);
        for (ConvPlan *sp : subs) {
            float best = 1e30f;
            int bestP = sp->P, bestPad = 0;
            int bestSplit = 0, bestPP = 1, bestW16 = 0, bestHi = 0, bestKs = 0;
            const Y2Options &o = c->opt;
            const int fs = o.splitk;
            for (int cfgx = 0; cfgx < 18 + 12 + 4; ++cfgx) {
                const int ks = cfgx >= 30 ? 2 << (cfgx - 30) : 0;
                const int cfg = ks ? 3 : (cfgx >= 18 ? cfgx - 18 : cfgx);
                const bool hiacc = cfgx >= 18 && !ks;
                if (hiacc && (sp->path != 4 || o.no_hiacc)) continue;
                if (ks && (c->batch > kKsMaxBatch || !c->ks_trip || o.no_ks || fs >= 0)) continue;
                const bool w16 = cfg >= 16;
                const int P = w16 ? cfg - 15 : (cfg >= 12 ? 1 : 8 >> (cfg & 3));
                const int pad = cfg >= 12 ? 0 : ((cfg >> 2) == 0 ? 0 : ((cfg >> 2) == 1 ? 160 * 1024 / 6 : 160 * 1024 / 4));
                if (pad && P > 2) continue;
                ConvPlan cand = *sp;
                cand.lds_pad = pad;
                cand.splitk = 0;
                cand.splitk_pp = 1;
                cand.w16 = w16 ? 1 : 0;
                cand.hiacc = hiacc ? 1 : 0;
                cand.ks = ks;
                if (w16 && o.no_w16) continue;
                if (cfg >= 12 && !w16) {
                    if (!sp->splitk_ok || !c->extra[i].empty() || fs == 0) continue;
                    cand.splitk = cfg == 13 ? 8 : 4;
                    cand.splitk_pp = cfg == 14 ? 2 : (cfg == 15 ? 4 : 1);
                } else if (fs == 1 && sp->splitk_ok && c->extra[i].empty()) {
                    ConvPlan probe = *sp;
                    probe.splitk = 4;
                    plan_conv(probe, tin.g, tout.g.cg_stride, out_base, CGout, o, 1);
                    if (probe.splitk) continue;
                }
                plan_conv(cand, tin.g, tout.g.cg_stride, out_base, CGout, o, P);
                if (w16 && !cand.w16) continue;
                if (hiacc && !cand.hiacc) continue;
                if (ks && cand.ks != ks) continue;
                if (cfg >= 12 && !w16 && !cand.splitk) continue;
                if (cfg == 14 && cand.splitk_pp != 2) continue;
                if (cfg == 15 && cand.splitk_pp != 4) continue;
                if (cand.P != P) continue;
                float tmin = 1e30f;
                for (int rep = 0; rep < 3; ++rep) {
                    (void)hipMemsetAsync(flush, rep, flush_bytes, nullptr);
                    (void)hipEventRecord(e0, nullptr);
                    const int lrc = launch_conv(cand, tin.d, tout.d, (const int2 *)(c->wpk + c->wpk_off[ord]), c->bias_pk + c->bias_off[ord], nullptr, nullptr,
                                                c->ks_trip, c->ks_trip_bytes);
                    if (lrc) return lrc;
                    (void)hipEventRecord(e1, nullptr);
                    HIP_TRY(hipEventSynchronize(e1), YOLO2_ERROR);
                    float t = 0;
                    HIP_TRY(hipEventElapsedTime(&t, e0, e1), YOLO2_ERROR);
                    tmin = std::min(tmin, t);
                }
                if (o.verbose)
                    fprintf(stderr, "[yolo2_hip] tune L%d path %d: P=%d pad=%d splitk=%d w16=%d hiacc=%d ks=%d grid=(%u,%u) %.1f us\n", i, cand.path, P, pad,
                            cand.splitk, cand.w16, cand.hiacc, cand.ks, cand.grid.x, cand.grid.y, tmin * 1e3);
                if (tmin < best) { best = tmin; bestP = P; bestPad = pad; bestSplit = cand.splitk; bestPP = cand.splitk_pp; bestW16 = cand.w16; bestHi = cand.hiacc; bestKs = cand.ks; }
            }
            sp->lds_pad = bestPad;
            sp->splitk = bestSplit;
            sp->splitk_pp = bestPP;
            sp->w16 = bestW16;
            sp->hiacc = bestHi;
            sp->ks = bestKs;
            plan_conv(*sp, tin.g, tout.g.cg_stride, out_base, CGout, o, bestP);
        }
        ord++;
    }
    (void)hipEventDestroy(e0);
    (void)hipEventDestroy(e1);
    (void)hipFree(flush);
    HIP_TRY(hipGetLastError(), YOLO2_ERROR);
    return YOLO2_SUCCESS;
}

static int set_batch_single(yolo2_hip_ctx *c, int batch);
static int setup_pool_fusion(yolo2_hip_ctx *c, bool timed, bool default_on);


static size_t ks_potential_bytes(const yolo2_hip_ctx *c, int batch)
{
    if (batch > kKsMaxBatch || c->opt.no_ks) return 0;
    return (size_t)16 * 24 * (size_t)64 * 2704 * (size_t)batch;
}

static size_t ks_needed_bytes(const yolo2_hip_ctx *c)
{
    size_t need = 0;
    for (int i = 0; i < 32; ++i)
        if (kNet[i].type == L_CONV && c->plan[i].ks) need = std::max(need, y2_ks_bytes(c->plan[i].ks, c->plan[i].args.CGout, c->plan[i].args.npix));
    return need;
}

static int ensure_ks_scratch(yolo2_hip_ctx *c, size_t bytes)
{
    if (c->ks_trip_bytes == bytes) return YOLO2_SUCCESS;
    HIP_TRY(hipDeviceSynchronize(), YOLO2_ERROR);
    if (c->ks_trip) (void)hipFree(c->ks_trip);
    c->ks_trip = nullptr;
    c->ks_trip_bytes = 0;
    if (bytes) {
        HIP_TRY(hipMalloc((void **)&c->ks_trip, bytes), YOLO2_MMAP_ERROR);
        c->ks_trip_bytes = bytes;
    }
    return YOLO2_SUCCESS;
}

typedef bool (*Y2LineLookup)(yolo2_hip_ctx *c, int B, int L, int S, Y2PlanLine *out);
static bool lookup_table(yolo2_hip_ctx *c, int B, int L, int S, Y2PlanLine *out) { return y2_plan_table_lookup(c->opt, B, L, S, out); }
static bool lookup_cache(yolo2_hip_ctx *c, int B, int L, int S, Y2PlanLine *out)
{
    if (!c->plan_cache) return false;
    std::lock_guard<std::mutex> lk(c->plan_cache->mu);
    auto it = c->plan_cache->lines.find({B, {L, S}});
    if (it == c->plan_cache->lines.end()) return false;
    *out = it->second;
    return true;
}

static int apply_plan_lines(yolo2_hip_ctx *c, Y2LineLookup look, const char *what, bool *known)
{
    *known = false;
    struct Todo { ConvPlan *dst; ConvPlan cand; };
    std::vector<Todo> todo;
    bool fuse[32] = {false};
    for (int i = 0; i < 32; ++i) {
        if (kNet[i].type != L_CONV) continue;
        const Tensor &tin = i == 0 ? c->t_in : (i == 26 ? c->t_out[16] : (i == 29 ? c->t_cat : c->t_out[i - 1]));
        const Tensor &tout = c->t_out[i];
        const long out_base = kLead + (i == 24 ? (long)64 * tout.g.cg_stride : 0);
        std::vector<ConvPlan *> subs{&c->plan[i]};
        for (auto &e : c->extra[i]) subs.push_back(&e);
        for (size_t s = 0; s < subs.size(); ++s) {
            Y2PlanLine pl;
            if (!look(c, c->batch, i, (int)s, &pl) || pl.path != subs[s]->path) return YOLO2_SUCCESS;
            ConvPlan cand = *subs[s];
            cand.lds_pad = pl.pad; cand.splitk = pl.splitk; cand.splitk_pp = pl.pp; cand.w16 = pl.w16; cand.hiacc = pl.hiacc; cand.ks = pl.ks;
            cand.ks_cap = s == 0 ? ks_potential_bytes(c, c->batch) : 0;
            plan_conv(cand, tin.g, tout.g.cg_stride, out_base, (kNet[i].n + 3) / 4, c->opt, pl.P);
            if (cand.P != pl.P || cand.lds_pad != pl.pad || cand.splitk != pl.splitk || cand.splitk_pp != pl.pp || cand.w16 != pl.w16 ||
                cand.hiacc != pl.hiacc || cand.ks != pl.ks) {
                if (c->opt.verbose)
                    fprintf(stderr, "[yolo2_hip] %s: layer %d launch %zu at batch %d: the planner refuses the line (P %d/%d pad %d/%d splitk %d/%d pp %d/%d "
                            "w16 %d/%d hiacc %d/%d ks %d/%d) - timing instead\n", what, i, s, c->batch, cand.P, pl.P, cand.lds_pad, pl.pad, cand.splitk, pl.splitk,
                            cand.splitk_pp, pl.pp, cand.w16, pl.w16, cand.hiacc, pl.hiacc, cand.ks, pl.ks);
                return YOLO2_SUCCESS;
            }
            todo.push_back({subs[s], cand});
            if (s == 0) fuse[i] = pl.fuse != 0;
        }
    }
    for (Todo &t : todo) *t.dst = t.cand;
    int rc = ensure_ks_scratch(c, ks_needed_bytes(c));
    if (rc) return rc;
    rc = setup_pool_fusion(c, false, true);
    if (rc) return rc;
    for (int i = 0; i < 32; ++i) c->fuse_pool[i] = c->fuse_pool[i] && fuse[i];
    HIP_TRY(hipDeviceSynchronize(), YOLO2_ERROR);
    *known = true;
    return YOLO2_SUCCESS;
}

static void record_plan(yolo2_hip_ctx *c)
{
    FILE *f = c->opt.plan_write.empty() ? nullptr : fopen(c->opt.plan_write.c_str(), "a");
    Y2PlanCache *pc = c->plan_cache && !c->opt.no_plan_cache && c->plan_cache->hash && c->opt.force_path < 0 ? c->plan_cache.get() : nullptr;
    if (!f && !pc) return;
    for (int i = 0; i < 32; ++i) {
        if (kNet[i].type != L_CONV) continue;
        std::vector<const ConvPlan *> subs{&c->plan[i]};
        for (auto &e : c->extra[i]) subs.push_back(&e);
        for (size_t s = 0; s < subs.size(); ++s) {
            const Y2PlanLine pl{subs[s]->path, subs[s]->P, subs[s]->lds_pad, subs[s]->splitk, subs[s]->splitk_pp, subs[s]->w16,
                                s == 0 && c->fuse_pool[i] ? 1 : 0, subs[s]->hiacc, subs[s]->ks};
            if (f) fprintf(f, "%d %d %zu %d %d %d %d %d %d %d %d %d\n", c->batch, i, s, pl.path, pl.P, pl.pad, pl.splitk, pl.pp, pl.w16, pl.fuse, pl.hiacc, pl.ks);
            if (pc) {
                std::lock_guard<std::mutex> lk(pc->mu);
                const Y2PlanKey k{c->batch, {i, (int)s}};
                if (!pc->lines.count(k)) pc->per_batch[c->batch]++;
                pc->lines[k] = pl;
                pc->dirty = true;
            }
        }
    }
    if (f) fclose(f);
    if (pc && !pc->save() && c->opt.verbose) fprintf(stderr, "[yolo2_hip] plan cache %s could not be written (the plan is kept for this process only)\n", pc->path.c_str());
}

static void launch_maxpool(const Tensor &tin, const Tensor &tout, int B, hipStream_t st)
{
    const ActGeom &gi = tin.g, &go = tout.g;
    const long n = (long)go.CG * B * go.H * go.W;
    hipLaunchKernelGGL(k_maxpool2, dim3(blocks_for(n, 256)), dim3(256), 0, st, tin.d, tout.d, go.CG, B, go.H, go.W, gi.Wp, gi.PL,
                       go.Wp, go.PL);
}

static int setup_pool_fusion(yolo2_hip_ctx *c, bool timed, bool default_on)
{
    for (bool &f : c->fuse_pool) f = false;
    if (c->opt.no_poolfuse) return YOLO2_SUCCESS;
    const bool force = c->opt.poolfuse == 1;
    if (!default_on && !force) return YOLO2_SUCCESS;
    hipEvent_t e0 = nullptr, e1 = nullptr;
    void *flush = nullptr;
    const size_t flush_bytes = (size_t)64 << 20;
    if (timed && !force) {
        HIP_TRY(hipEventCreate(&e0), YOLO2_ERROR);
        HIP_TRY(hipEventCreate(&e1), YOLO2_ERROR);
        HIP_TRY(hipMalloc(&flush, flush_bytes), YOLO2_MMAP_ERROR);
    }
    int ord = 0;
    for (int i = 0; i < 31; ++i) {
        if (kNet[i].type != L_CONV) continue;
        const int o = ord++;
        if (kNet[i + 1].type != L_MAX) continue;
        const Tensor &tin = i == 0 ? c->t_in : c->t_out[i - 1];
        const Tensor &tout = c->t_out[i], &tpool = c->t_out[i + 1];
        const int full = i == 16 ? 1 : 0;
        ConvPlan fp = c->plan[i];
        bool ok = plan_conv_pool(fp, tin.g, tpool.g, full);
        std::vector<ConvPlan> fx;
        for (const auto &e : c->extra[i]) {
            ConvPlan fe2 = e;
            ok = ok && plan_conv_pool(fe2, tin.g, tpool.g, full);
            fx.push_back(fe2);
        }
        if (!ok) continue;
        c->fplan[i] = fp;
        c->fextra[i] = fx;
        if (!timed || force) { c->fuse_pool[i] = true; continue; }
        const int2 *wp = (const int2 *)(c->wpk + c->wpk_off[o]);
        const short *bp = c->bias_pk + c->bias_off[o];
        float best[2] = {1e30f, 1e30f};
        for (int variant = 0; variant < 2; ++variant)
            for (int rep = 0; rep < 2; ++rep) {
                (void)hipMemsetAsync(flush, rep, flush_bytes, nullptr);
                (void)hipEventRecord(e0, nullptr);
                int lrc = YOLO2_SUCCESS;
                if (variant == 0) {
                    lrc = launch_conv(c->plan[i], tin.d, tout.d, wp, bp, nullptr, nullptr, c->ks_trip, c->ks_trip_bytes);
                    for (const auto &e : c->extra[i]) if (!lrc) lrc = launch_conv(e, tin.d, tout.d, wp, bp, nullptr);
                    launch_maxpool(tout, tpool, c->batch, nullptr);
                } else {
                    lrc = launch_conv(fp, tin.d, tout.d, wp, bp, nullptr, tpool.d);
                    for (const auto &e : fx) if (!lrc) lrc = launch_conv(e, tin.d, tout.d, wp, bp, nullptr, tpool.d);
                }
                if (lrc) return lrc;
                (void)hipEventRecord(e1, nullptr);
                HIP_TRY(hipEventSynchronize(e1), YOLO2_ERROR);
                float t = 0;
                HIP_TRY(hipEventElapsedTime(&t, e0, e1), YOLO2_ERROR);
                best[variant] = std::min(best[variant], t);
            }
        c->fuse_pool[i] = best[1] < best[0] * 1.05f;
        if (c->opt.verbose)
            fprintf(stderr, "[yolo2_hip] L%d conv+pool: separate %.1f us, fused %.1f us -> %s\n", i, best[0] * 1e3, best[1] * 1e3,
                    c->fuse_pool[i] ? "fused" : "separate");
    }
    if (e0) (void)hipEventDestroy(e0);
    if (e1) (void)hipEventDestroy(e1);
    if (flush) (void)hipFree(flush);
    HIP_TRY(hipGetLastError(), YOLO2_ERROR);
    return YOLO2_SUCCESS;
}

static int make_lane(yolo2_hip_ctx *p, bool own_stream, yolo2_hip_ctx **out)
{
    yolo2_hip_ctx *l = new (std::nothrow) yolo2_hip_ctx();
    if (!l) return fail(YOLO2_ERROR, "out of host memory");
    l->device = p->device;
    l->is_lane = true;
    l->opt = p->opt;
    l->plan_cache = p->plan_cache;
    l->wpk = p->wpk;
    l->bias_pk = p->bias_pk;
    memcpy(l->wpk_off, p->wpk_off, sizeof(p->wpk_off));
    memcpy(l->bias_off, p->bias_off, sizeof(p->bias_off));
    memcpy(l->maxsum, p->maxsum, sizeof(p->maxsum));
    memcpy(l->maxbias, p->maxbias, sizeof(p->maxbias));
    for (int o = 0; o < YOLO2_N_CONV; ++o) {
        l->maxsum_mb[o] = p->maxsum_mb[o];
        l->maxbias_mb[o] = p->maxbias_mb[o];
        l->maxabs_mb[o] = p->maxabs_mb[o];
    }
    l->weight_q = p->weight_q;
    l->bias_q = p->bias_q;
    l->act_q = p->act_q;
    int rc = resolve_q(l);
    if (rc == YOLO2_SUCCESS && own_stream) rc = y2_lane_stream_create(&l->lane_stream);
    if (rc == YOLO2_SUCCESS && own_stream && hipEventCreateWithFlags(&l->ev_join, hipEventDisableTiming) != hipSuccess) rc = fail(YOLO2_ERROR, "hipEventCreate failed");
    if (rc) { yolo2_hip_destroy(l); return rc; }
    l->weights_loaded = true;
    *out = l;
    return YOLO2_SUCCESS;
}

extern "C" int yolo2_hip_set_batch(yolo2_hip_ctx *c, int batch)
{
    if (!c) return fail(YOLO2_ERROR, "null ctx");
    if (batch <= 0 || batch > 4096) return fail(YOLO2_ERROR, "batch %d out of range", batch);
    if (!c->weights_loaded) return fail(YOLO2_ERROR, "load weights before set_batch");
    HIP_TRY(hipSetDevice(c->device), YOLO2_INIT_ERROR);
    int nl = (batch >= 48 && batch < 128) ? 3 : 2;
    if (c->opt.lanes > 0) nl = c->opt.lanes;
    const bool want_lanes = !c->is_lane && nl > 1 && batch >= 8 * nl && !c->opt.no_lanes;
    if (!want_lanes) {
        if (c->laned) c->batch = 0;
        y2_destroy_lanes(c);
        return set_batch_single(c, batch);
    }
    if (c->laned && c->batch == batch && (int)c->lanes.size() == nl) return YOLO2_SUCCESS;
    y2_destroy_lanes(c);
    y2_free_activations(c);
    if (!c->ev_fork) HIP_TRY(hipEventCreateWithFlags(&c->ev_fork, hipEventDisableTiming), YOLO2_ERROR);
    c->lane_first.clear();
    int first = 0;
    for (int i = 0; i < nl; ++i) {
        yolo2_hip_ctx *l = nullptr;
        int frames = batch / nl + (i >= nl - batch % nl ? 1 : 0);
        if (!c->opt.lane_split.empty()) {
            std::vector<int> v;
            for (const char *q = c->opt.lane_split.c_str(); *q;) { v.push_back(atoi(q)); while (*q && *q != ',') ++q; if (*q) ++q; }
            int sum = 0;
            for (int x : v) sum += x;
            if ((int)v.size() == nl && sum == batch) frames = v[i];
        }
        int rc = make_lane(c, i > 0 || y2_lane0_own_stream(), &l);
        if (rc == YOLO2_SUCCESS) {
            c->lanes.push_back(l);
            c->lane_first.push_back(first);
            rc = set_batch_single(l, frames);
        }
        if (rc) { y2_destroy_lanes(c); return rc; }
        first += frames;
    }
    if (c->prof) (void)yolo2_hip_set_profiling(c->lanes[0], 1);
    c->batch = batch;
    c->laned = true;
    return YOLO2_SUCCESS;
}

static int set_batch_single(yolo2_hip_ctx *c, int batch)
{
    if (c->batch != batch) {
        y2_free_activations(c);
        int rc;
        if ((rc = alloc_tensor(c->t_in, 3, 416, 416, batch))) return rc;
        if ((rc = alloc_tensor(c->t_cat, 1280, 13, 13, batch))) return rc;
        for (int i = 0; i < 31; ++i) {
            const LayerDesc &l = kNet[i];
            if (l.type == L_CONV && i != 24) {
                if ((rc = alloc_tensor(c->t_out[i], l.n, l.h, l.w, batch))) return rc;
            } else if (l.type == L_MAX) {
                if ((rc = alloc_tensor(c->t_out[i], l.c, l.h / 2, l.w / 2, batch))) return rc;
            }
        }
        c->t_out[24] = c->t_cat;
        c->t_out[27] = c->t_cat;
        c->batch = batch;
    }
    const Y2Options &o = c->opt;
    const size_t ks_pot = ks_potential_bytes(c, batch);
    auto geom_of = [&](int i, const Tensor *&tin, const Tensor *&tout, long &out_base) {
        tin = i == 0 ? &c->t_in : (i == 26 ? &c->t_out[16] : (i == 29 ? &c->t_cat : &c->t_out[i - 1]));
        tout = &c->t_out[i];
        out_base = kLead + (i == 24 ? (long)64 * tout->g.cg_stride : 0);
    };
    for (int i = 0; i < 32; ++i) {
        if (kNet[i].type != L_CONV) continue;
        const Tensor *tin, *tout;
        long out_base;
        geom_of(i, tin, tout, out_base);
        const int CGout = (kNet[i].n + 3) / 4;
        c->plan[i].ks_cap = ks_pot;
        c->plan[i].ks = 0;
        plan_conv(c->plan[i], tin->g, tout->g.cg_stride, out_base, CGout, o);
        for (auto &e : c->extra[i]) { e.ks_cap = 0; e.ks = 0; plan_conv(e, tin->g, tout->g.cg_stride, out_base, CGout, o); }
    }
    if (o.force_p > 0) {
        for (int i = 0; i < 32; ++i) {
            if (kNet[i].type != L_CONV) continue;
            c->plan[i].w16 = o.force_w16;
            c->plan[i].hiacc = o.force_hiacc;
            c->plan[i].ks = (o.force_ks > 0 && batch <= kKsMaxBatch) ? o.force_ks : 0;
            for (auto &e : c->extra[i]) { e.w16 = o.force_w16; e.hiacc = o.force_hiacc; }
            const Tensor *tin, *tout;
            long out_base;
            geom_of(i, tin, tout, out_base);
            plan_conv(c->plan[i], tin->g, tout->g.cg_stride, out_base, (kNet[i].n + 3) / 4, o, o.force_p);
            for (auto &e : c->extra[i]) plan_conv(e, tin->g, tout->g.cg_stride, out_base, (kNet[i].n + 3) / 4, o, o.force_p);
        }
        c->plan_source = 4;
        const int rc = ensure_ks_scratch(c, ks_needed_bytes(c));
        if (rc) return rc;
        HIP_TRY(hipDeviceSynchronize(), YOLO2_ERROR);
        return setup_pool_fusion(c, false, false);
    }
    if (o.autotune != 1 && !o.steered()) {
        bool known = false;
        if (c->plan_cache && !o.no_plan_cache && c->plan_cache->hash) {
            const int rc = apply_plan_lines(c, lookup_cache, "weight cache", &known);
            if (rc) return rc;
            if (known) { c->plan_source = 5; return YOLO2_SUCCESS; }
        }
        if (y2_plan_table_has_batch(o, batch)) {
            const int rc = apply_plan_lines(c, lookup_table, "plan table", &known);
            if (rc) return rc;
            if (known) { c->plan_source = 1; return YOLO2_SUCCESS; }
        }
    }
    if (o.autotune != 0) {
        c->plan_source = 2;
        int rc = ensure_ks_scratch(c, o.splitk >= 0 ? 0 : ks_pot);
        if (rc == YOLO2_SUCCESS) rc = autotune(c);
        if (rc == YOLO2_SUCCESS) rc = setup_pool_fusion(c, true, true);
        if (rc == YOLO2_SUCCESS) rc = ensure_ks_scratch(c, ks_needed_bytes(c));
        if (rc == YOLO2_SUCCESS && !o.steered()) record_plan(c);
        return rc;
    }
    c->plan_source = 3;
    {
        const int rc = ensure_ks_scratch(c, 0);
        if (rc) return rc;
    }
    HIP_TRY(hipDeviceSynchronize(), YOLO2_ERROR);
    return setup_pool_fusion(c, false, true);
}

extern "C" int yolo2_hip_plan_source(yolo2_hip_ctx *c)
{
    if (!c) return 0;
    if (c->laned && !c->lanes.empty()) return c->lanes[0]->plan_source;
    return c->plan_source;
}

extern "C" size_t yolo2_hip_ks_scratch_bytes(yolo2_hip_ctx *c)
{
    if (!c) return 0;
    if (c->laned && !c->lanes.empty()) return c->lanes[0]->ks_trip_bytes;
    return c->ks_trip_bytes;
}

extern "C" int yolo2_hip_layer_pool_fused(yolo2_hip_ctx *c, int layer_idx)
{
    if (!c || layer_idx < 0 || layer_idx > 31 || !c->batch) return 0;
    if (c->laned) return yolo2_hip_layer_pool_fused(c->lanes[0], layer_idx);
    return c->fuse_pool[layer_idx] ? 1 : 0;
}

extern "C" int yolo2_hip_conv_launch_info(yolo2_hip_ctx *c, int ord, int *grid_x, int *grid_y, int *block, int *lds_bytes,
                                          int *ppl)
{
    if (!c || !c->batch) return fail(YOLO2_ERROR, "set_batch first");
    if (c->laned) return yolo2_hip_conv_launch_info(c->lanes[0], ord, grid_x, grid_y, block, lds_bytes, ppl);
    int o = 0;
    for (int i = 0; i < 32; ++i)
        if (kNet[i].type == L_CONV) {
            if (o == ord) {
                const ConvPlan &pl = c->fuse_pool[i] ? c->fplan[i] : c->plan[i];
                if (grid_x) *grid_x = pl.grid.x;
                if (grid_y) *grid_y = pl.grid.y;
                if (block) *block = pl.w16 ? 128 : 256;
                if (lds_bytes) *lds_bytes = pl.lds_bytes;
                if (ppl) *ppl = pl.ks ? -pl.ks : (pl.splitk ? 0 : pl.P);
                return YOLO2_SUCCESS;
            }
            o++;
        }
    return fail(YOLO2_ERROR, "bad conv ordinal %d", ord);
}

extern "C" int yolo2_hip_conv_plan_string(yolo2_hip_ctx *c, int ord, char *buf, int cap)
{
    if (!c || !buf || cap <= 0) return fail(YOLO2_ERROR, "null argument");
    if (!c->batch) return fail(YOLO2_ERROR, "set_batch first");
    if (c->laned) return yolo2_hip_conv_plan_string(c->lanes[0], ord, buf, cap);
    int o = 0;
    for (int i = 0; i < 32; ++i)
        if (kNet[i].type == L_CONV) {
            if (o == ord) {
                const ConvPlan &pl = c->fuse_pool[i] ? c->fplan[i] : c->plan[i];
                snprintf(buf, (size_t)cap, "P=%d pad=%d w16=%d hiacc=%d ks=%d splitk=%d pp=%d grp=%d fused=%d form=%d extra=%zu edge=%d", pl.P, pl.lds_pad, pl.w16,
                         pl.hiacc, pl.ks, pl.splitk, pl.splitk_pp, pl.grp, pl.pool_fused, pl.path, c->extra[i].size(), pl.args.edge);
                return YOLO2_SUCCESS;
            }
            o++;
        }
    return fail(YOLO2_ERROR, "bad conv ordinal %d", ord);
}

extern "C" int yolo2_hip_run_batch_int16(yolo2_hip_ctx *c, uint64_t frames_dev, int batch, uint64_t region_dev,
                                         int *final_q, void *stream)
{
    if (!c) return fail(YOLO2_ERROR, "null ctx");
    if (!c->weights_loaded) return fail(YOLO2_ERROR, "weights not loaded");
    if (!frames_dev || !region_dev) return fail(YOLO2_ERROR, "null buffer address");
    if (batch != c->batch) {
        const int rc = yolo2_hip_set_batch(c, batch);
        if (rc) return rc;
    }
    hipStream_t st = (hipStream_t)stream;
    if (c->laned) {
        const int nl = (int)c->lanes.size();
        HIP_TRY(hipEventRecord(c->ev_fork, st), YOLO2_ERROR);
        for (int k = 0; k < nl; ++k) {
            const int i = (k + 1) % nl;
            yolo2_hip_ctx *l = c->lanes[i];
            hipStream_t ls = l->lane_stream ? l->lane_stream : st;
            const uint64_t first = (uint64_t)c->lane_first[i];
            if (l->lane_stream) HIP_TRY(hipStreamWaitEvent(ls, c->ev_fork, 0), YOLO2_ERROR);
            const int rc = yolo2_hip_run_batch_int16(l, frames_dev + first * YOLO2_FRAME_ELEMS * sizeof(float), l->batch,
                                                     region_dev + first * YOLO2_REGION_ELEMS * sizeof(int16_t), final_q, ls);
            if (rc) return rc;
            if (l->lane_stream) HIP_TRY(hipEventRecord(l->ev_join, ls), YOLO2_ERROR);
        }
        for (int i = 0; i < nl; ++i)
            if (c->lanes[i]->lane_stream) HIP_TRY(hipStreamWaitEvent(st, c->lanes[i]->ev_join, 0), YOLO2_ERROR);
        c->final_q = c->lanes[0]->final_q;
        return YOLO2_SUCCESS;
    }
    const float *frames = (const float *)(uintptr_t)frames_dev;
    short *region = (short *)(uintptr_t)region_dev;
    const int B = batch;
    const float scale = ldexpf(1.0f, c->act_q[0]);

    if (c->prof) {
        const int rc = y2_ensure_prof_events(c);
        if (rc) return rc;
    }
    hipEvent_t *ev = c->prof ? c->ev[c->prof_runs % yolo2_hip_ctx::kProfSlots] : nullptr;
    if (ev) HIP_TRY(hipEventRecord(ev[0], st), YOLO2_ERROR);
    {
        const ActGeom &g = c->t_in.g;
        hipLaunchKernelGGL(k_pack_input, dim3(blocks_for((long)B * g.H * g.W, 256)), dim3(256), 0, st, frames, c->t_in.d, B,
                           g.H, g.W, g.Wp, g.PL, scale);
    }
    int ord = 0;
    const Tensor *cur = &c->t_in;
    for (int i = 0; i < 32; ++i) {
        const LayerDesc &l = kNet[i];
        switch (l.type) {
        case L_CONV: {
            const Tensor *tin = i == 26 ? &c->t_out[16] : (i == 29 ? &c->t_cat : cur);
            const int2 *wp = (const int2 *)(c->wpk + c->wpk_off[ord]);
            const short *bp = c->bias_pk + c->bias_off[ord];
            int lrc;
            if (c->fuse_pool[i]) {
                lrc = launch_conv(c->fplan[i], tin->d, c->t_out[i].d, wp, bp, st, c->t_out[i + 1].d);
                for (const auto &e : c->fextra[i]) if (!lrc) lrc = launch_conv(e, tin->d, c->t_out[i].d, wp, bp, st, c->t_out[i + 1].d);
            } else {
                lrc = launch_conv(c->plan[i], tin->d, c->t_out[i].d, wp, bp, st, nullptr, c->ks_trip, c->ks_trip_bytes);
                for (const auto &e : c->extra[i])
                    if (!lrc) lrc = launch_conv(e, tin->d, c->t_out[i].d, wp, bp, st);
            }
            if (lrc) return lrc;
            cur = &c->t_out[i];
            ord++;
            break;
        }
        case L_MAX: {
            if (!c->fuse_pool[i - 1]) launch_maxpool(*cur, c->t_out[i], B, st);
            cur = &c->t_out[i];
            break;
        }
        case L_REORG: {
            const ActGeom &gi = cur->g, &go = c->t_cat.g;
            hipLaunchKernelGGL(k_reorg, dim3(blocks_for((long)B * 256 * 169, 256)), dim3(256), 0, st, (const short *)cur->d,
                               (short *)c->t_cat.d, B, gi.Wp, gi.PL, gi.cg_stride, go.Wp, go.PL, go.cg_stride, c->reorg_shift);
            cur = &c->t_cat;
            break;
        }
        case L_ROUTE:
            break;
        case L_REGION: {
            const ActGeom &g = cur->g;
            hipLaunchKernelGGL(k_unpack_dense, dim3(blocks_for((long)B * 425 * 169, 256)), dim3(256), 0, st,
                               (const short *)cur->d, region, B, 425, 13, 13, g.Wp, g.PL, g.cg_stride);
            break;
        }
        }
        if (ev) (void)hipEventRecord(ev[i + 1], st);
    }
    HIP_TRY(hipGetLastError(), YOLO2_ERROR);
    if (ev) c->prof_runs++;
    if (final_q) *final_q = c->final_q;
    return YOLO2_SUCCESS;
}

extern "C" int yolo2_hip_run_batch_int16_host(yolo2_hip_ctx *c, const float *frames, int batch, int16_t *region,
                                              int *final_q)
{
    if (!c || !frames || !region) return fail(YOLO2_ERROR, "null argument");
    HIP_TRY(hipSetDevice(c->device), YOLO2_INIT_ERROR);
    float *fd = nullptr;
    short *rd = nullptr;
    HIP_TRY(hipMalloc((void **)&fd, (size_t)batch * YOLO2_FRAME_ELEMS * 4), YOLO2_MMAP_ERROR);
    HIP_TRY(hipMalloc((void **)&rd, (size_t)batch * YOLO2_REGION_ELEMS * 2), YOLO2_MMAP_ERROR);
    HIP_TRY(hipMemcpy(fd, frames, (size_t)batch * YOLO2_FRAME_ELEMS * 4, hipMemcpyHostToDevice), YOLO2_DMA_ERROR);
    int rc = yolo2_hip_run_batch_int16(c, (uint64_t)(uintptr_t)fd, batch, (uint64_t)(uintptr_t)rd, final_q, nullptr);
    if (rc == YOLO2_SUCCESS) {
        hipError_t e = hipMemcpy(region, rd, (size_t)batch * YOLO2_REGION_ELEMS * 2, hipMemcpyDeviceToHost);
        if (e != hipSuccess) rc = fail(YOLO2_DMA_ERROR, "D2H of region tensor failed: %s", hipGetErrorString(e));
    }
    (void)hipFree(fd);
    (void)hipFree(rd);
    return rc;
}

extern "C" int yolo2_hip_debug_layer_output(yolo2_hip_ctx *c, int layer_idx, int frame, int16_t *out, size_t cap,
                                            size_t *out_elems)
{
    if (!c || !out) return fail(YOLO2_ERROR, "null argument");
    if (layer_idx < -1 || layer_idx > 30 || !c->batch || frame < 0 || frame >= c->batch) return fail(YOLO2_ERROR, "bad layer/frame");
    if (c->laned) {
        int li = (int)c->lanes.size() - 1;
        while (li > 0 && frame < c->lane_first[li]) --li;
        return yolo2_hip_debug_layer_output(c->lanes[li], layer_idx, frame - c->lane_first[li], out, cap, out_elems);
    }
    if (layer_idx >= 0 && c->fuse_pool[layer_idx] && layer_idx != 16)
        return fail(YOLO2_ERROR, "layer %d's tensor is not materialised: conv + pool run fused (YOLO2_NO_POOLFUSE=1 keeps it)", layer_idx);
    const LayerDesc &l = kNet[layer_idx < 0 ? 0 : layer_idx];
    if (layer_idx >= 0 && l.type == L_ROUTE) return fail(YOLO2_ERROR, "route layers have no tensor of their own");
    const Tensor &t = layer_idx < 0 ? c->t_in : c->t_out[layer_idx];
    int C = layer_idx < 0 ? 3 : (l.type == L_MAX ? l.c : l.n), H = t.g.H, W = t.g.W;
    const short *base = (const short *)t.d;
    if (layer_idx == 24) base += (long)64 * t.g.cg_stride * 4;
    const int W8 = (W + 7) & ~7;
    const size_t n = (size_t)C * H * W8;
    if (out_elems) *out_elems = n;
    if (cap < n) return fail(YOLO2_ERROR, "output buffer too small (%zu < %zu)", cap, n);
    HIP_TRY(hipSetDevice(c->device), YOLO2_INIT_ERROR);
    short *tmp = nullptr;
    HIP_TRY(hipMalloc((void **)&tmp, n * 2), YOLO2_MMAP_ERROR);
    HIP_TRY(hipMemset(tmp, 0, n * 2), YOLO2_DMA_ERROR);
    hipLaunchKernelGGL(k_items_to_ref, dim3(blocks_for((long)C * H * W, 256)), dim3(256), 0, nullptr, base, tmp, C, H, W, W8,
                       t.g.Wp, t.g.PL, t.g.cg_stride, frame);
    hipError_t e = hipMemcpy(out, tmp, n * 2, hipMemcpyDeviceToHost);
    (void)hipFree(tmp);
    if (e != hipSuccess) return fail(YOLO2_DMA_ERROR, "D2H failed: %s", hipGetErrorString(e));
    return YOLO2_SUCCESS;
}


namespace {
struct DrvScratch {
    void *in_items = nullptr, *out_items = nullptr, *wpk = nullptr, *bias_pk = nullptr;
    size_t in_cap = 0, out_cap = 0, wpk_cap = 0, bias_cap = 0;
    int *bound = nullptr;
} g_scr;
}

void y2_drv_release_i16(void)
{
    for (void *p : {g_scr.in_items, g_scr.out_items, g_scr.wpk, g_scr.bias_pk, (void *)g_scr.bound})
        if (p) (void)hipFree(p);
    g_scr = DrvScratch();
}

static int max_abs_i16_dev(const short *dev, int n, int *out)
{
    std::vector<short> h(n);
    HIP_TRY(hipMemcpy(h.data(), dev, (size_t)n * 2, hipMemcpyDeviceToHost), YOLO2_DMA_ERROR);
    int m = 0;
    for (short v : h) m = std::max(m, std::abs((int)v));
    *out = m;
    return YOLO2_SUCCESS;
}

static int g_last_edge = 0;
extern "C" int yolo2_hip_last_layer_edge(void) { return g_last_edge; }

int y2_drv_conv_i16(const short *in, short *out, const short *w, const short *beta, int ifm_num, int ofm_num, int ksize, int kstride,
                    int input_w, int input_h, int output_w, int output_h, int padding, int is_nl, int qw, int qa_in, int qa_out, int qb,
                    int *path_out)
{
    hipStream_t st = nullptr;
    g_last_edge = 0;
    const int so = qa_in + qw - qa_out, sb = qb - qa_out;
    if (!g_scr.bound) HIP_TRY(hipMalloc((void **)&g_scr.bound, 4 * sizeof(int)), YOLO2_MMAP_ERROR);
    bool tiled = kstride == 1 && ((ksize == 3 && padding == 1) || (ksize == 1 && padding == 0));
    if (tiled) {
        const ActGeom g = make_geom(ifm_num, input_h, input_w, 1);
        if (tile_items_bound(g, 64, ksize == 3 ? g.Wp + 1 : 0) > kMaxTileItems) tiled = false;
    }
    if (!tiled) {
        *path_out = -1;
        const int n = ofm_num * output_h * output_w;
        hipLaunchKernelGGL(k_conv_ref_i16, dim3(blocks_for(n, 256)), dim3(256), 0, st, in, out, w, beta, ifm_num, ofm_num,
                           ksize, kstride, input_w, input_h, output_w, output_h, padding, is_nl ? 1 : 0, so, sb);
        HIP_TRY(hipGetLastError(), YOLO2_ERROR);
        return YOLO2_SUCCESS;
    }

    const ActGeom gi = make_geom(ifm_num, input_h, input_w, 1), go = make_geom(ofm_num, output_h, output_w, 1);
    const long wpk_elems = packed_weight_elems(ifm_num, ofm_num, ksize);
    const int MB = (ofm_num + 31) / 32;
    int rc;
    if ((rc = y2_ensure(&g_scr.in_items, &g_scr.in_cap, (size_t)gi.items * 8))) return rc;
    if ((rc = y2_ensure(&g_scr.out_items, &g_scr.out_cap, (size_t)go.items * 8))) return rc;
    if ((rc = y2_ensure(&g_scr.wpk, &g_scr.wpk_cap, (size_t)wpk_elems * 2))) return rc;
    if ((rc = y2_ensure(&g_scr.bias_pk, &g_scr.bias_cap, (size_t)MB * 32 * 2))) return rc;
    HIP_TRY(hipMemsetAsync(g_scr.in_items, 0, (size_t)gi.items * 8, st), YOLO2_DMA_ERROR);
    HIP_TRY(hipMemsetAsync(g_scr.bias_pk, 0, (size_t)MB * 32 * 2, st), YOLO2_DMA_ERROR);
    HIP_TRY(hipMemsetAsync(g_scr.bound, 0, sizeof(int), st), YOLO2_DMA_ERROR);
    HIP_TRY(hipMemcpyAsync(g_scr.bias_pk, beta, (size_t)ofm_num * 2, hipMemcpyDeviceToDevice, st), YOLO2_DMA_ERROR);
    hipLaunchKernelGGL(k_ref_to_items, dim3(blocks_for((long)ifm_num * input_h * input_w, 256)), dim3(256), 0, st, in,
                       (short *)g_scr.in_items, ifm_num, input_h, input_w, (input_w + 7) & ~7, gi.Wp, gi.cg_stride);
    hipLaunchKernelGGL((k_repack_weights<short>), dim3(blocks_for(wpk_elems, 256)), dim3(256), 0, st, w, (short *)g_scr.wpk,
                       ifm_num, ofm_num, ksize * ksize);
    hipLaunchKernelGGL(k_weight_bound, dim3(std::min<unsigned>(blocks_for(wpk_elems / 4, 256), 1024)), dim3(256), 0, st,
                       (const short *)g_scr.wpk, wpk_elems / 4, g_scr.bound);
    hipLaunchKernelGGL(k_weight_bound_mb, dim3(1), dim3(256), 0, st, (const short *)g_scr.wpk, wpk_elems / 4, g_scr.bound + 1,
                       g_scr.bound + 2);
    int hbound[3] = {0, 0, 0}, maxb = 0;
    HIP_TRY(hipMemcpy(hbound, g_scr.bound, sizeof(hbound), hipMemcpyDeviceToHost), YOLO2_DMA_ERROR);
    const int maxsum = hbound[0], maxabs = hbound[2];
    if ((rc = max_abs_i16_dev(beta, ofm_num, &maxb))) return rc;

    ConvPlan p;
    p.args.mb_list = nullptr;
    p.C = ifm_num; p.N = ofm_num; p.K = ksize; p.H = input_h; p.W = input_w; p.leaky = is_nl ? 1 : 0;
    p.Qw = qw; p.Qa_in = qa_in; p.Qa_out = qa_out; p.Qb = qb;
    const Y2Options &popt = y2_process_options();
    p.path = choose_path(so, sb, maxsum, maxb, maxabs, popt.force_path);
    if (p.path == 4) {
        HIP_TRY(hipMemsetAsync(g_scr.bound + 3, 16 - so, 1, st), YOLO2_DMA_ERROR);
        hipLaunchKernelGGL(k_scale_weight_blocks, dim3(std::min<unsigned>(blocks_for(wpk_elems, 256), 256), 1), dim3(256), 0, st,
                           (short *)g_scr.wpk, wpk_elems, (const signed char *)(g_scr.bound + 3));
    }
    plan_conv(p, gi, go.cg_stride, kLead, go.CG, popt);
    *path_out = p.path;
    g_last_edge = p.args.edge;
    if ((rc = launch_conv(p, (const int2 *)g_scr.in_items, (int2 *)g_scr.out_items, (const int2 *)g_scr.wpk, (const short *)g_scr.bias_pk, st))) return rc;
    hipLaunchKernelGGL(k_items_to_ref, dim3(blocks_for((long)ofm_num * output_h * output_w, 256)), dim3(256), 0, st,
                       (const short *)g_scr.out_items, out, ofm_num, output_h, output_w, (output_w + 7) & ~7, go.Wp, go.PL,
                       go.cg_stride, 0);
    HIP_TRY(hipGetLastError(), YOLO2_ERROR);
    return YOLO2_SUCCESS;
}

void y2_drv_pool_i16(const short *in, short *out, int channels, int ksize, int kstride, int input_w, int input_h, int output_w, int output_h)
{
    const int n = channels * output_h * output_w;
    hipLaunchKernelGGL((k_pool_ref<short>), dim3(blocks_for(n, 256)), dim3(256), 0, nullptr, in, out, channels, ksize, kstride, input_w,
                       input_h, output_w, output_h, (short)-32768);
}
```

### yolo-fpga-accelerator_amd/csrc/yolo2_plan.hip

```cpp
#include <hip/hip_runtime.h>

#include <dlfcn.h>
#include <unistd.h>

#include <cctype>
#include <cstdio>
#include <cstdlib>
#include <cstring>
#include <initializer_list>

#include "y2_internal.hpp"


namespace {
struct FlagOpt { const char *name; bool Y2Options::*m; };
struct IntOpt { const char *name; int Y2Options::*m; int lo, hi; };
struct StrOpt { const char *name; std::string Y2Options::*m; };

const FlagOpt kFlags[] = {
    {"no_lanes", &Y2Options::no_lanes}, {"verbose", &Y2Options::verbose}, {"no_plan_cache", &Y2Options::no_plan_cache},
    {"no_poolfuse", &Y2Options::no_poolfuse}, {"no_hiacc", &Y2Options::no_hiacc}, {"no_ks", &Y2Options::no_ks},
    {"no_w16", &Y2Options::no_w16}, {"no_grp", &Y2Options::no_grp}, {"grp16", &Y2Options::grp16}, {"no_xcd_remap", &Y2Options::no_xcd_remap},
    {"no_edge_tiles", &Y2Options::no_edge_tiles}, {"splitk_no_pack", &Y2Options::splitk_no_pack}, {"force_w16", &Y2Options::force_w16}, {"force_hiacc", &Y2Options::force_hiacc},
    {"f16_no_lanes", &Y2Options::f16_no_lanes}, {"f16_no_mfma0", &Y2Options::f16_no_mfma0}, {"f16_no_glds", &Y2Options::f16_no_glds},
    {"f16_no_poolfuse", &Y2Options::f16_no_poolfuse}, {"f16_no_halo", &Y2Options::f16_no_halo}, {"f16_no_persist", &Y2Options::f16_no_persist},
    {"f16_persist_all", &Y2Options::f16_persist_all}, {"f16_ring_all", &Y2Options::f16_ring_all}, {"f16_no_ring", &Y2Options::f16_no_ring},
    {"f16_no_c32", &Y2Options::f16_no_c32}, {"f16_m16", &Y2Options::f16_m16}, {"f16_w8", &Y2Options::f16_w8}, {"f16_no_wide", &Y2Options::f16_no_wide},
    {"f16_no_fuse1x1", &Y2Options::f16_no_fuse1x1}, {"f16_no_rw", &Y2Options::f16_no_rw}, {"f16_no_rwb", &Y2Options::f16_no_rwb}, {"f16_no_rwc", &Y2Options::f16_no_rwc}, {"f16_ring256", &Y2Options::f16_ring256}, {"f16_ring_sq", &Y2Options::f16_ring_sq},
};
const IntOpt kInts[] = {
    {"autotune", &Y2Options::autotune, -1, 1}, {"lanes", &Y2Options::lanes, 0, 8}, {"lane_priority", &Y2Options::lane_priority, 0, 1},
    {"splitk", &Y2Options::splitk, -1, 1}, {"poolfuse", &Y2Options::poolfuse, -1, 1}, {"f16_lanes", &Y2Options::f16_lanes, 1, 8},
    {"stamp_layer", &Y2Options::stamp_layer, -1, 31}, {"f16_skip", &Y2Options::f16_skip, 0, 63}, {"force_path", &Y2Options::force_path, -1, 4}, {"force_p", &Y2Options::force_p, 0, 8},
    {"force_ks", &Y2Options::force_ks, 0, 16}, {"f32_p", &Y2Options::f32_p, 0, 4},
};
const StrOpt kStrs[] = {
    {"plan_file", &Y2Options::plan_file}, {"plan_write", &Y2Options::plan_write}, {"lane_split", &Y2Options::lane_split},
};
}

int Y2Options::set(const char *name, const char *value)
{
    if (!name) return -1;
    const Y2Options dflt;
    const bool clear = !value || !value[0];
    for (const FlagOpt &f : kFlags)
        if (!strcmp(name, f.name)) {
            this->*f.m = clear ? dflt.*f.m : strcmp(value, "0") != 0;
            return 0;
        }
    for (const IntOpt &o : kInts)
        if (!strcmp(name, o.name)) {
            if (clear) { this->*o.m = dflt.*o.m; return 0; }
            char *end = nullptr;
            const long v = strtol(value, &end, 10);
            if (end == value || *end || v < o.lo || v > o.hi) return -1;
            this->*o.m = (int)v;
            return 0;
        }
    for (const StrOpt &o : kStrs)
        if (!strcmp(name, o.name)) {
            this->*o.m = clear ? std::string() : std::string(value);
            return 0;
        }
    return -1;
}

Y2Options Y2Options::from_env()
{
    Y2Options o;
    auto env_name = [](const char *name) {
        std::string e = "YOLO2_";
        for (const char *p = name; *p; ++p) e += (char)toupper((unsigned char)*p);
        return e;
    };
    auto take = [&](const char *name) {
        const char *v = getenv(env_name(name).c_str());
        if (!v) return;
        if (o.set(name, v[0] ? v : "1") != 0)
            fprintf(stderr, "[yolo2_hip] ignoring %s=%s (out of range)\n", env_name(name).c_str(), v);
    };
    for (const FlagOpt &f : kFlags) take(f.name);
    for (const IntOpt &i : kInts) take(i.name);
    for (const StrOpt &s : kStrs) take(s.name);
    return o;
}

std::string Y2Options::describe() const
{
    const Y2Options d;
    std::string out;
    auto add = [&](const std::string &kv) { out += (out.empty() ? "" : " ") + kv; };
    for (const FlagOpt &f : kFlags)
        if (this->*f.m != d.*f.m) add(std::string(f.name) + "=" + (this->*f.m ? "1" : "0"));
    for (const IntOpt &i : kInts)
        if (this->*i.m != d.*i.m) add(std::string(i.name) + "=" + std::to_string(this->*i.m));
    for (const StrOpt &s : kStrs)
        if (this->*s.m != d.*s.m) add(std::string(s.name) + "=" + this->*s.m);
    return out;
}

static Y2Options &process_options_mut()
{
    static Y2Options o = Y2Options::from_env();
    return o;
}
const Y2Options &y2_process_options() { return process_options_mut(); }

extern "C" int yolo2_hip_set_option(yolo2_hip_ctx *c, const char *name, const char *value)
{
    if (!name) return fail(YOLO2_ERROR, "null argument");
    if (!c) {
        if (process_options_mut().set(name, value) != 0) return fail(YOLO2_ERROR, "unknown option or value out of range: %s=%s", name, value ? value : "");
        return YOLO2_SUCCESS;
    }
    if (c->opt.set(name, value) != 0) return fail(YOLO2_ERROR, "unknown option or value out of range: %s=%s", name, value ? value : "");
    for (yolo2_hip_ctx *l : c->lanes) l->opt = c->opt;
    return YOLO2_SUCCESS;
}

extern "C" int yolo2_hip_options_string(yolo2_hip_ctx *c, char *buf, int cap)
{
    if (!c || !buf || cap <= 0) return fail(YOLO2_ERROR, "null argument");
    snprintf(buf, (size_t)cap, "%s", c->opt.describe().c_str());
    return YOLO2_SUCCESS;
}


size_t y2_ks_bytes(int splits, int cg_out, int npix) { return (size_t)splits * (size_t)cg_out * (size_t)npix * 24; }

bool y2_ks_fits(int splits, int cg_out, int npix, size_t cap_bytes)
{
    if (splits <= 0 || cg_out <= 0 || npix <= 0 || cap_bytes == 0) return false;
    return y2_ks_bytes(splits, cg_out, npix) <= cap_bytes;
}

extern "C" int yolo2_hip_i16_plan_check(int splits, int cg_out, int npix, size_t cap_bytes)
{
    if (splits != 2 && splits != 4 && splits != 8 && splits != 16) return fail(YOLO2_ERROR, "K-split: %d splits (2, 4, 8 or 16)", splits);
    if (cg_out <= 0 || npix <= 0) return fail(YOLO2_ERROR, "K-split: empty output (%d items x %d pixels)", cg_out, npix);
    if (cap_bytes == 0) return fail(YOLO2_ERROR, "K-split: this context holds no triple scratch (batch > 4 or scratch not allocated): the plan is refused");
    if (!y2_ks_fits(splits, cg_out, npix, cap_bytes))
        return fail(YOLO2_ERROR, "K-split: %d splits x %d items x %d pixels x 24 B = %zu bytes of triples do not fit the %zu-byte scratch", splits, cg_out,
                    npix, y2_ks_bytes(splits, cg_out, npix), cap_bytes);
    return YOLO2_SUCCESS;
}

extern "C" int yolo2_hip_i16_edge_map(int B, int H, int W, int cap, int *tile_cls, int *tile_mask, int *pix, long long *steps)
{
    if (B <= 0 || H <= 0 || W <= 0) return fail(YOLO2_ERROR, "edge tiles: empty geometry %d x %d x %d", B, H, W);
    const y2::ActGeom g = y2::make_geom(4, H, W, B);
    y2::ConvArgs a{};
    a.B = B; a.H = H; a.W = W; a.Wp = g.Wp; a.PL = g.PL;
    a.npix = B * H * W;
    y2::set_conv_div(a);
    if (!y2::edge_tiles_plan(a)) return 0;
    if (steps) *steps = y2::edge_tiles_steps(a);
    if (tile_cls && tile_mask && pix) {
        if (cap < a.e_nt) return fail(YOLO2_ERROR, "edge tiles: %d tiles, room for %d", a.e_nt, cap);
        for (int t = 0; t < a.e_nt; ++t) {
            int ct;
            const int cls = y2::edge_tile_class(a, t, ct);
            tile_cls[t] = cls;
            tile_mask[t] = y2::edge_class_mask(cls);
            for (int lane = 0; lane < 64; ++lane) {
                int b, y, x;
                const bool ok = y2::edge_lane_pixel(a, cls, ct, lane, b, y, x);
                pix[64L * t + lane] = ok ? (b * H + y) * W + x : -1;
            }
        }
    }
    return a.e_nt;
}


bool y2_plan_line_parse(const char *line, Y2PlanKey *key, Y2PlanLine *out)
{
    int B, L, S;
    Y2PlanLine pl;
    pl.hiacc = pl.ks = 0;
    if (line[0] == '#' || sscanf(line, "%d %d %d %d %d %d %d %d %d %d %d %d", &B, &L, &S, &pl.path, &pl.P, &pl.pad, &pl.splitk, &pl.pp, &pl.w16, &pl.fuse,
                                 &pl.hiacc, &pl.ks) < 10)
        return false;
    auto one_of = [](int v, std::initializer_list<int> ok) { for (int o : ok) if (v == o) return true; return false; };
    if (B <= 0 || B > 4096 || L < 0 || L >= 32 || S < 0 || S > 8 || !one_of(pl.path, {0, 1, 2, 3, 4}) || !one_of(pl.P, {1, 2, 4, 8}) ||
        !one_of(pl.pad, {0, 160 * 1024 / 6, 160 * 1024 / 4}) || !one_of(pl.splitk, {0, 4, 8}) || !one_of(pl.pp, {1, 2, 4}) ||
        !one_of(pl.w16, {0, 1}) || !one_of(pl.fuse, {0, 1}) || !one_of(pl.hiacc, {0, 1}) || !one_of(pl.ks, {0, 2, 4, 8, 16}))
        return false;
    *key = {B, {L, S}};
    *out = pl;
    return true;
}

namespace {
struct PlanTable {
    std::map<Y2PlanKey, Y2PlanLine> lines;
    std::map<int, int> per_batch;
};
std::mutex g_tables_mu;
std::map<std::string, std::shared_ptr<PlanTable>> g_tables;

std::string default_plan_path()
{
    Dl_info info;
    if (!dladdr((const void *)&y2_plan_line_parse, &info) || !info.dli_fname) return "";
    std::string lib = info.dli_fname;
    const size_t slash = lib.rfind('/');
    const std::string dir = slash == std::string::npos ? std::string(".") : lib.substr(0, slash);
    for (const std::string &cand : {dir + "/config/plan_gfx950.txt", dir + "/../config/plan_gfx950.txt"}) {
        FILE *f = fopen(cand.c_str(), "r");
        if (f) { fclose(f); return cand; }
    }
    return "";
}

std::shared_ptr<PlanTable> table_for(const Y2Options &opt)
{
    const std::string path = !opt.plan_file.empty() ? opt.plan_file : default_plan_path();
    std::lock_guard<std::mutex> lk(g_tables_mu);
    auto it = g_tables.find(path);
    if (it != g_tables.end()) return it->second;
    auto t = std::make_shared<PlanTable>();
    FILE *f = path.empty() ? nullptr : fopen(path.c_str(), "r");
    if (f) {
        char line[256];
        while (fgets(line, sizeof(line), f)) {
            Y2PlanKey k;
            Y2PlanLine pl;
            if (!y2_plan_line_parse(line, &k, &pl)) continue;
            if (!t->lines.count(k)) t->per_batch[k.first]++;
            t->lines[k] = pl;
        }
        fclose(f);
    }
    g_tables[path] = t;
    return t;
}
}

bool y2_plan_table_has_batch(const Y2Options &opt, int B) { return table_for(opt)->per_batch.count(B) != 0; }

bool y2_plan_table_lookup(const Y2Options &opt, int B, int L, int S, Y2PlanLine *out)
{
    auto t = table_for(opt);
    auto it = t->lines.find({B, {L, S}});
    if (it == t->lines.end()) return false;
    *out = it->second;
    return true;
}


uint64_t y2_hash_bytes(uint64_t h, const void *data, size_t n)
{
    const unsigned char *p = (const unsigned char *)data;
    if (!h) h = 1469598103934665603ull;
    for (size_t i = 0; i < n; ++i) { h ^= p[i]; h *= 1099511628211ull; }
    return h;
}

static const char kCacheMagic[] = "Y2PLAN 2 gfx950";

bool Y2PlanCache::load(uint64_t want_hash, std::string *why)
{
    std::lock_guard<std::mutex> lk(mu);
    lines.clear();
    per_batch.clear();
    bounds_valid = false;
    dirty = false;
    hash = want_hash;
    for (auto &b : bounds) b = Bounds();
    auto no = [&](const char *w) { if (why) *why = w; lines.clear(); per_batch.clear(); for (auto &b : bounds) b = Bounds(); return false; };
    FILE *f = path.empty() ? nullptr : fopen(path.c_str(), "r");
    if (!f) return no("no cache file");
    std::string body;
    char line[4096];
    bool magic = false, hash_ok = false, sum_seen = false;
    int n_bounds = 0;
    while (fgets(line, sizeof(line), f)) {
        if (sum_seen) { fclose(f); return no("data after the checksum line"); }
        if (!strncmp(line, "sum ", 4)) {
            unsigned long long s = 0;
            if (sscanf(line + 4, "%llx", &s) != 1 || s != y2_hash_bytes(0, body.data(), body.size())) { fclose(f); return no("checksum mismatch (damaged file)"); }
            sum_seen = true;
            continue;
        }
        body += line;
        if (!magic) {
            if (strncmp(line, kCacheMagic, sizeof(kCacheMagic) - 1)) { fclose(f); return no("not a plan cache of this format / architecture"); }
            magic = true;
            continue;
        }
        if (!strncmp(line, "hash ", 5)) {
            unsigned long long h = 0;
            if (sscanf(line + 5, "%llx", &h) != 1 || h != want_hash) { fclose(f); return no("made for another weight set (hash differs)"); }
            hash_ok = true;
            continue;
        }
        if (!strncmp(line, "bound ", 6)) {
            int ord, ms, mb, MB, used = 0;
            if (sscanf(line + 6, "%d %d %d %d%n", &ord, &ms, &mb, &MB, &used) != 4 || ord < 0 || ord >= YOLO2_N_CONV || MB <= 0 || MB > 64) { fclose(f); return no("bad bound line"); }
            Bounds &b = bounds[ord];
            b.maxsum = ms; b.maxbias = mb;
            const char *p = line + 6 + used;
            for (int k = 0; k < MB; ++k) {
                int v[5], u = 0;
                if (sscanf(p, "%d %d %d %d %d%n", &v[0], &v[1], &v[2], &v[3], &v[4], &u) != 5) { fclose(f); return no("bad bound line"); }
                b.sum_mb.push_back(v[0]); b.bias_mb.push_back(v[1]); b.abs_mb.push_back(v[2]); b.form.push_back(v[3]); b.scale.push_back(v[4]);
                p += u;
            }
            ++n_bounds;
            continue;
        }
        if (!strncmp(line, "plan ", 5)) {
            Y2PlanKey k;
            Y2PlanLine pl;
            if (!y2_plan_line_parse(line + 5, &k, &pl)) { fclose(f); return no("bad plan line"); }
            if (!lines.count(k)) per_batch[k.first]++;
            lines[k] = pl;
            continue;
        }
        if (line[0] == '#' || line[0] == '\n') continue;
        fclose(f);
        return no("unknown line");
    }
    fclose(f);
    if (!magic || !hash_ok || !sum_seen) return no("truncated file");
    if (n_bounds != YOLO2_N_CONV) return no("bounds of some conv layers are missing");
    bounds_valid = true;
    return true;
}

bool Y2PlanCache::save()
{
    std::lock_guard<std::mutex> lk(mu);
    if (path.empty() || !hash) return false;
    std::string body = std::string(kCacheMagic) + "\n";
    char buf[256];
    body += "# weight-side plan cache of libyolo2_hip.so: bounds behind the arithmetic-form proofs, forms / scale shifts per block of 32\n"
            "# output channels, and the timed conv plan per batch (same fields as config/plan_gfx950.txt).  Delete it to re-time.\n";
    snprintf(buf, sizeof(buf), "hash %016llx\n", (unsigned long long)hash);
    body += buf;
    for (int o = 0; o < YOLO2_N_CONV; ++o) {
        const Bounds &b = bounds[o];
        snprintf(buf, sizeof(buf), "bound %d %d %d %zu", o, b.maxsum, b.maxbias, b.sum_mb.size());
        body += buf;
        for (size_t k = 0; k < b.sum_mb.size(); ++k) {
            snprintf(buf, sizeof(buf), " %d %d %d %d %d", b.sum_mb[k], b.bias_mb[k], b.abs_mb[k], b.form[k], b.scale[k]);
            body += buf;
        }
        body += "\n";
    }
    for (const auto &kv : lines) {
        const Y2PlanLine &p = kv.second;
        snprintf(buf, sizeof(buf), "plan %d %d %d %d %d %d %d %d %d %d %d %d\n", kv.first.first, kv.first.second.first, kv.first.second.second, p.path, p.P,
                 p.pad, p.splitk, p.pp, p.w16, p.fuse, p.hiacc, p.ks);
        body += buf;
    }
    snprintf(buf, sizeof(buf), "sum %016llx\n", (unsigned long long)y2_hash_bytes(0, body.data(), body.size()));
    const std::string tmp = path + ".tmp." + std::to_string((long)getpid());
    FILE *f = fopen(tmp.c_str(), "w");
    if (!f) return false;
    const bool ok = fwrite(body.data(), 1, body.size(), f) == body.size() && fputs(buf, f) >= 0;
    if (fclose(f) != 0 || !ok || rename(tmp.c_str(), path.c_str()) != 0) { remove(tmp.c_str()); return false; }
    dirty = false;
    return true;
}

extern "C" int yolo2_hip_set_plan_cache(yolo2_hip_ctx *c, const char *path)
{
    if (!c) return fail(YOLO2_ERROR, "null ctx");
    if (c->is_lane) return fail(YOLO2_ERROR, "lanes share their parent's plan cache");
    if (!path || !path[0]) { c->plan_cache.reset(); return YOLO2_SUCCESS; }
    c->plan_cache = std::make_shared<Y2PlanCache>();
    c->plan_cache->path = path;
    return YOLO2_SUCCESS;
}

extern "C" int yolo2_hip_plan_cache_info(yolo2_hip_ctx *c, uint64_t *weights_hash, int *bounds_from_file, int *n_lines, int *n_batches)
{
    if (!c || !c->plan_cache) return fail(YOLO2_ERROR, "no plan cache bound (yolo2_hip_set_plan_cache)");
    std::lock_guard<std::mutex> lk(c->plan_cache->mu);
    if (weights_hash) *weights_hash = c->plan_cache->hash;
    if (bounds_from_file) *bounds_from_file = c->plan_cache->bounds_valid ? 1 : 0;
    if (n_lines) *n_lines = (int)c->plan_cache->lines.size();
    if (n_batches) *n_batches = (int)c->plan_cache->per_batch.size();
    return YOLO2_SUCCESS;
}

extern "C" int yolo2_hip_plan_cache_check(const char *path, uint64_t weights_hash, int *n_lines)
{
    if (!path) return fail(YOLO2_ERROR, "null path");
    Y2PlanCache pc;
    pc.path = path;
    std::string why;
    if (!pc.load(weights_hash, &why)) return fail(YOLO2_ERROR, "plan cache %s refused: %s", path, why.c_str());
    if (n_lines) *n_lines = (int)pc.lines.size();
    return YOLO2_SUCCESS;
}
```

### yolo-fpga-accelerator_amd/yolo2_amd/hipdrv.py

```python
import ctypes as C
import os
import subprocess

import numpy as np

from . import net

PKG_DIR = os.path.dirname(os.path.dirname(os.path.abspath(__file__)))
LIB_PATH = os.environ.get("YOLO2_HIP_LIB") or os.path.join(PKG_DIR, "libyolo2_hip.so")

YOLO2_SUCCESS, YOLO2_ERROR, YOLO2_TIMEOUT, YOLO2_INIT_ERROR, YOLO2_MMAP_ERROR, YOLO2_DMA_ERROR = 0, -1, -2, -3, -4, -5

EXPORTS = [
    "yolo2_accel_init", "yolo2_accel_cleanup", "yolo2_hip_select_device", "yolo2_hip_device_count",
    "yolo2_hip_last_error", "yolo2_set_q_values", "yolo2_is_busy", "yolo2_is_done", "yolo2_wait_for_completion",
    "yolo2_execute_conv_layer", "yolo2_execute_maxpool_layer", "yolo2_execute_conv_layer_f32",
    "memory_allocate_ddr", "memory_free_ddr", "memory_allocate_weights", "memory_allocate_bias",
    "memory_allocate_inference_buffer", "memory_get_phys_addr", "memory_flush_cache", "memory_invalidate_cache",
    "yolo2_hip_alloc", "yolo2_hip_free", "yolo2_hip_memcpy_h2d", "yolo2_hip_memcpy_d2h", "yolo2_hip_memset",
    "yolo2_hip_create", "yolo2_hip_destroy", "yolo2_hip_load_weights_int16", "yolo2_hip_load_weights_int16_dev",
    "yolo2_hip_layer_path", "yolo2_hip_set_batch", "yolo2_hip_run_batch_int16", "yolo2_hip_run_batch_int16_host",
    "yolo2_hip_debug_layer_output", "yolo2_hip_set_profiling", "yolo2_hip_layer_times_ms",
    "yolo2_hip_conv_launch_info", "yolo2_strip_int16_layer_pad", "yolo2_weight_len", "yolo2_bias_len",
    "yolo2_hip_num_layers", "yolo2_hip_layer_desc",
    "yolo2_hip_layer_path_counts", "yolo2_hip_run_frames_int16", "yolo2_hip_num_lanes", "yolo2_hip_load_weights_fp32", "yolo2_hip_run_batch_fp16", "yolo2_hip_run_batch_fp16_host",
    "yolo2_hip_letterbox_u8", "yolo2_hip_run_images_u8_host", "yolo2_hip_last_layer_path", "yolo2_hip_run_frame_fp32_host", "yolo2_hip_num_lanes_fp16",
    "yolo2_hip_layer_pool_fused", "yolo2_get_status", "yolo2_read_reg", "yolo2_write_reg", "yolo2_hip_driver_calls",
    "dma_buffer_init", "dma_buffer_cleanup", "dma_buffer_alloc", "dma_buffer_free", "dma_buffer_sync_for_device",
    "dma_buffer_sync_for_cpu", "dma_buffer_get_phys",
    "yolo2_hip_run_batch_fp32", "yolo2_hip_run_batch_fp32_host", "yolo2_hip_load_weights_fp32_dev", "yolo2_hip_postprocess_int16", "yolo2_hip_postprocess_f32",
    "yolo2_hip_shard_range", "yolo2_hip_multi_create", "yolo2_hip_multi_destroy", "yolo2_hip_multi_num_devices",
    "yolo2_hip_multi_uses_rccl", "yolo2_hip_multi_ctx", "yolo2_hip_multi_load_weights_int16", "yolo2_hip_multi_load_weights_fp32",
    "yolo2_hip_multi_run_frames_int16", "yolo2_hip_multi_run_images_u8_host", "yolo2_hip_rccl_unique_id",
    "yolo2_hip_rccl_init_rank", "yolo2_hip_rccl_finalize", "yolo2_hip_load_weights_int16_bcast", "yolo2_hip_load_weights_fp32_bcast",
    "yolo2_hip_rccl_info", "yolo2_hip_multi_rccl_info", "yolo2_hip_ctx_device", "yolo2_hip_alloc_on",
    "yolo2_hip_fp16_layer_kernel", "yolo2_hip_f16_store_check",
    "yolo2_hip_run_images_u8_dets", "yolo2_hip_multi_run_images_u8_dets", "yolo2_hip_set_fp16_lanes", "yolo2_hip_conv_plan_string", "yolo2_hip_plan_source",
    "yolo2_hip_set_option", "yolo2_hip_options_string", "yolo2_hip_set_plan_cache", "yolo2_hip_plan_cache_info", "yolo2_hip_plan_cache_check",
    "yolo2_hip_i16_plan_check", "yolo2_hip_ks_scratch_bytes", "yolo2_hip_i16_edge_map", "yolo2_hip_last_layer_edge",
    "yolo2_hip_run_batch_f32tol", "yolo2_hip_run_batch_f32tol_host", "yolo2_hip_f32tol_layer_kernel", "yolo2_hip_num_lanes_f32tol",
    "yolo2_hip_debug_f16_tensor",
    "yolo2_hip_run_images_u8_f16_host", "yolo2_hip_run_images_u8_dets_f16", "yolo2_hip_multi_run_images_u8_dets_f16",
    "yolo2_hip_images_layer0_kernel",
    "yolo2_hip_letterbox_pix", "yolo2_hip_run_images_pix_host", "yolo2_hip_run_images_pix_dets", "yolo2_hip_run_images_pix_f16_host",
    "yolo2_hip_run_images_pix_dets_f16", "yolo2_hip_multi_run_images_pix_host", "yolo2_hip_multi_run_images_pix_dets",
    "yolo2_hip_multi_run_images_pix_dets_f16",
]

PIXFMTS = {"grey8": 1, "rgb24": 3, "yuyv": 0x56595559}


def _pix_code(pixfmt, imgs) -> int:
    if pixfmt not in PIXFMTS:
        raise ValueError(f"pixfmt must be None or one of {tuple(PIXFMTS)}, not {pixfmt!r}")
    last = {"grey8": None, "rgb24": 3, "yuyv": 2}[pixfmt]
    for im in imgs:
        if (im.ndim != 2 if last is None else im.ndim != 3 or im.shape[2] != last):
            raise ValueError(f"a {pixfmt} image is uint8 [h][w]{'' if last is None else f'[{last}]'}, not {im.shape}")
    return PIXFMTS[pixfmt]


def letterbox_pix(image: np.ndarray, pixfmt: str, net_w: int = 416, net_h: int = 416) -> np.ndarray:
    return letterbox_u8(image, net_w, net_h, pixfmt=pixfmt)


def letterbox_u8(image_hwc: np.ndarray, net_w: int = 416, net_h: int = 416, pixfmt=None) -> np.ndarray:
    im = np.ascontiguousarray(image_hwc, dtype=np.uint8)
    ch = 1 if im.ndim == 2 else im.shape[2]
    code = None if pixfmt is None else _pix_code(pixfmt, [im])
    L = lib()
    src, dst = C.c_uint64(0), C.c_uint64(0)
    out = np.empty((3, net_h, net_w), dtype=np.float32)
    check(L.yolo2_hip_alloc(im.nbytes, C.byref(src)), "alloc")
    check(L.yolo2_hip_alloc(out.nbytes, C.byref(dst)), "alloc")
    try:
        check(L.yolo2_hip_memcpy_h2d(src, im.ctypes.data_as(C.c_void_p), im.nbytes), "h2d")
        if code is None:
            check(L.yolo2_hip_letterbox_u8(src, im.shape[1], im.shape[0], ch, dst, net_w, net_h, None), "yolo2_hip_letterbox_u8")
        else:
            check(L.yolo2_hip_letterbox_pix(src, im.shape[1], im.shape[0], code, dst, net_w, net_h, None), "yolo2_hip_letterbox_pix")
        check(L.yolo2_hip_memcpy_d2h(out.ctypes.data_as(C.c_void_p), dst, out.nbytes), "d2h")
    finally:
        L.yolo2_hip_free(src)
        L.yolo2_hip_free(dst)
    return out


class Yolo2HipError(RuntimeError):
    pass


def build(force: bool = False) -> str:
    srcs = [os.path.join(PKG_DIR, "csrc", f) for f in os.listdir(os.path.join(PKG_DIR, "csrc"))]
    srcs.append(os.path.join(os.path.dirname(PKG_DIR), "include", "yolo2_hip.h"))
    if force or not os.path.exists(LIB_PATH) or any(os.path.getmtime(s) > os.path.getmtime(LIB_PATH) for s in srcs):
        subprocess.run(["make", "-s", "-C", PKG_DIR], check=True)
    return LIB_PATH


_lib = None


def lib():
    global _lib
    if _lib is not None:
        return _lib
    if not os.path.exists(LIB_PATH):
        raise Yolo2HipError(f"{LIB_PATH} is missing: build it with `make -C {PKG_DIR}` "
                            "(the GPU path has no CPU fallback)")
    L = C.CDLL(LIB_PATH)
    u64, i32, u32, vp = C.c_uint64, C.c_int, C.c_uint32, C.c_void_p
    L.yolo2_hip_last_error.restype = C.c_char_p
    L.yolo2_execute_conv_layer.argtypes = [u64] * 4 + [i32] * 23 + [u32]
    L.yolo2_execute_maxpool_layer.argtypes = [u64] * 2 + [i32] * 14 + [u32]
    L.yolo2_execute_conv_layer_f32.argtypes = [u64] * 4 + [i32] * 10 + [u32]
    L.yolo2_hip_alloc.argtypes = [C.c_size_t, C.POINTER(u64)]
    L.yolo2_hip_free.argtypes = [u64]
    L.yolo2_hip_memcpy_h2d.argtypes = [u64, vp, C.c_size_t]
    L.yolo2_hip_memcpy_d2h.argtypes = [vp, u64, C.c_size_t]
    L.yolo2_hip_memset.argtypes = [u64, i32, C.c_size_t]
    L.yolo2_hip_create.argtypes = [i32, C.POINTER(vp)]
    L.yolo2_hip_destroy.argtypes = [vp]
    L.yolo2_hip_load_weights_int16.argtypes = [vp, vp, C.c_size_t, vp, C.c_size_t, vp, i32, vp, i32, vp, i32]
    L.yolo2_hip_load_weights_int16_dev.argtypes = [vp, u64, C.c_size_t, u64, C.c_size_t, vp, i32, vp, i32, vp, i32]
    L.yolo2_hip_layer_path.argtypes = [vp, i32]
    L.yolo2_hip_num_lanes.argtypes = [vp]
    L.yolo2_hip_layer_pool_fused.argtypes = [vp, i32]
    L.yolo2_hip_run_frames_int16.argtypes = [vp, vp, i32, i32, vp, C.POINTER(i32)]
    L.yolo2_hip_layer_path_counts.argtypes = [vp, i32, C.POINTER(i32)]
    L.yolo2_hip_set_batch.argtypes = [vp, i32]
    L.yolo2_hip_run_batch_int16.argtypes = [vp, u64, i32, u64, C.POINTER(i32), vp]
    L.yolo2_hip_run_batch_int16_host.argtypes = [vp, vp, i32, vp, C.POINTER(i32)]
    L.yolo2_hip_debug_layer_output.argtypes = [vp, i32, i32, vp, C.c_size_t, C.POINTER(C.c_size_t)]
    L.yolo2_hip_set_profiling.argtypes = [vp, i32]
    L.yolo2_hip_layer_times_ms.argtypes = [vp, vp]
    L.yolo2_hip_conv_launch_info.argtypes = [vp, i32] + [C.POINTER(i32)] * 5
    L.yolo2_strip_int16_layer_pad.argtypes = [vp, C.c_size_t, vp, i32, vp]
    L.yolo2_strip_int16_layer_pad.restype = C.c_long
    L.yolo2_hip_load_weights_fp32.argtypes = [vp, vp, C.c_size_t, vp, C.c_size_t]
    L.yolo2_hip_run_batch_fp16.argtypes = [vp, u64, i32, u64, vp]
    L.yolo2_hip_run_batch_fp16_host.argtypes = [vp, vp, i32, vp]
    L.yolo2_hip_run_frame_fp32_host.argtypes = [vp, vp, vp]
    L.yolo2_hip_run_batch_fp32.argtypes = [vp, u64, i32, u64, vp]
    L.yolo2_hip_run_batch_fp32_host.argtypes = [vp, vp, i32, vp]
    L.yolo2_hip_letterbox_u8.argtypes = [u64, i32, i32, i32, u64, i32, i32, vp]
    L.yolo2_hip_run_images_u8_host.argtypes = [vp, vp, vp, vp, i32, i32, i32, vp, C.POINTER(i32)]
    L.memory_get_phys_addr.restype = u64
    pi32 = C.POINTER(i32)
    L.yolo2_hip_load_weights_fp32_dev.argtypes = [vp, u64, C.c_size_t, u64, C.c_size_t]
    L.yolo2_hip_postprocess_int16.argtypes = [vp, u64, i32, i32, vp, vp, C.c_float, C.c_float, vp, i32, vp, vp, vp, vp, vp]
    L.yolo2_hip_postprocess_f32.argtypes = [vp, u64, i32, vp, vp, C.c_float, C.c_float, vp, i32, vp, vp, vp, vp, vp]
    L.yolo2_hip_shard_range.argtypes = [i32, i32, i32, pi32, pi32]
    def sig(name, argtypes, restype=None):
        f = getattr(L, name, None)
        if f is not None:
            f.argtypes = argtypes
            if restype is not None:
                f.restype = restype
    sig("yolo2_hip_set_option", [vp, C.c_char_p, C.c_char_p])
    sig("yolo2_hip_options_string", [vp, C.c_char_p, i32])
    sig("yolo2_hip_set_plan_cache", [vp, C.c_char_p])
    sig("yolo2_hip_plan_cache_info", [vp, C.POINTER(u64), pi32, pi32, pi32])
    sig("yolo2_hip_plan_cache_check", [C.c_char_p, u64, pi32])
    sig("yolo2_hip_i16_plan_check", [i32, i32, i32, C.c_size_t])
    sig("yolo2_hip_i16_edge_map", [i32, i32, i32, i32, vp, vp, vp, vp])
    sig("yolo2_hip_last_layer_edge", [], i32)
    sig("yolo2_hip_run_batch_f32tol", [vp, u64, i32, u64, vp])
    sig("yolo2_hip_run_batch_f32tol_host", [vp, vp, i32, vp])
    sig("yolo2_hip_f32tol_layer_kernel", [vp, i32], C.c_char_p)
    sig("yolo2_hip_num_lanes_f32tol", [vp])
    sig("yolo2_hip_ks_scratch_bytes", [vp], C.c_size_t)
    sig("yolo2_hip_debug_f16_tensor", [vp, i32, i32, i32, i32, vp, C.c_size_t, pi32])
    sig("yolo2_hip_run_images_u8_f16_host", [vp, i32, vp, vp, vp, i32, i32, i32, vp])
    sig("yolo2_hip_run_images_u8_dets_f16", [vp, i32, vp, vp, vp, i32, i32, i32, C.c_float, C.c_float, i32, vp, i32, vp])
    sig("yolo2_hip_multi_run_images_u8_dets_f16", [vp, i32, vp, vp, vp, i32, i32, i32, C.c_float, C.c_float, i32, vp, i32, vp])
    sig("yolo2_hip_images_layer0_kernel", [vp, i32], C.c_char_p)
    L.yolo2_hip_multi_create.argtypes = [vp, i32, C.POINTER(vp)]
    L.yolo2_hip_multi_destroy.argtypes = [vp]
    L.yolo2_hip_multi_num_devices.argtypes = [vp]
    L.yolo2_hip_multi_uses_rccl.argtypes = [vp]
    L.yolo2_hip_multi_ctx.argtypes = [vp, i32]
    L.yolo2_hip_multi_ctx.restype = vp
    L.yolo2_hip_multi_load_weights_int16.argtypes = [vp, vp, C.c_size_t, vp, C.c_size_t, vp, i32, vp, i32, vp, i32]
    L.yolo2_hip_multi_load_weights_fp32.argtypes = [vp, vp, C.c_size_t, vp, C.c_size_t]
    L.yolo2_hip_multi_run_frames_int16.argtypes = [vp, vp, i32, i32, vp, pi32]
    L.yolo2_hip_multi_run_images_u8_host.argtypes = [vp, vp, vp, vp, i32, i32, i32, vp, pi32]
    L.yolo2_hip_rccl_unique_id.argtypes = [vp]
    L.yolo2_hip_rccl_init_rank.argtypes = [vp, i32, vp, i32, i32]
    L.yolo2_hip_rccl_finalize.argtypes = [vp]
    L.yolo2_hip_load_weights_int16_bcast.argtypes = [vp, vp, C.c_size_t, vp, C.c_size_t, vp, i32, vp, i32, vp, i32, i32]
    L.yolo2_hip_load_weights_fp32_bcast.argtypes = [vp, vp, C.c_size_t, vp, C.c_size_t, i32]
    L.yolo2_hip_run_images_u8_dets.argtypes = [vp, vp, vp, vp, i32, i32, i32, C.c_float, C.c_float, i32, vp, i32, vp, C.POINTER(i32)]
    L.yolo2_hip_multi_run_images_u8_dets.argtypes = [vp, vp, vp, vp, i32, i32, i32, C.c_float, C.c_float, i32, vp, i32, vp, C.POINTER(i32)]
    L.yolo2_hip_set_fp16_lanes.argtypes = [vp, i32]
    L.yolo2_hip_conv_plan_string.argtypes = [vp, i32, C.c_char_p, i32]
    L.yolo2_hip_plan_source.argtypes = [vp]
    L.yolo2_hip_rccl_info.argtypes = [vp, vp]
    L.yolo2_hip_multi_rccl_info.argtypes = [vp, vp]
    L.yolo2_hip_ctx_device.argtypes = [vp]
    L.yolo2_hip_alloc_on.argtypes = [vp, C.c_size_t, C.POINTER(u64)]
    L.yolo2_hip_fp16_layer_kernel.argtypes = [vp, i32]
    L.yolo2_hip_fp16_layer_kernel.restype = C.c_char_p
    L.yolo2_hip_f16_store_check.argtypes = [i32] * 12
    L.yolo2_get_status.restype = u32
    L.yolo2_read_reg.restype = u32
    L.yolo2_read_reg.argtypes = [u32]
    L.yolo2_write_reg.argtypes = [u32, u32]
    L.yolo2_hip_driver_calls.restype = C.c_long
    L.yolo2_set_q_values.argtypes = [i32] * 4
    L.dma_buffer_alloc.argtypes = [C.c_size_t, vp]
    L.dma_buffer_free.argtypes = [vp]
    L.dma_buffer_get_phys.restype = u64
    L.dma_buffer_get_phys.argtypes = [vp, C.c_size_t]
    L.dma_buffer_sync_for_device.argtypes = [vp, C.c_size_t, C.c_size_t]
    L.dma_buffer_sync_for_cpu.argtypes = [vp, C.c_size_t, C.c_size_t]
    L.memory_get_phys_addr.argtypes = [vp]
    sig("yolo2_hip_letterbox_pix", L.yolo2_hip_letterbox_u8.argtypes)
    for name in ("run_images_pix_host", "multi_run_images_pix_host"):
        sig("yolo2_hip_" + name, L.yolo2_hip_run_images_u8_host.argtypes)
    for name in ("run_images_pix_dets", "multi_run_images_pix_dets"):
        sig("yolo2_hip_" + name, L.yolo2_hip_run_images_u8_dets.argtypes)
    sig("yolo2_hip_run_images_pix_f16_host", L.yolo2_hip_run_images_u8_f16_host.argtypes)
    for name in ("run_images_pix_dets_f16", "multi_run_images_pix_dets_f16"):
        sig("yolo2_hip_" + name, L.yolo2_hip_run_images_u8_dets_f16.argtypes)
    _lib = L
    return L


def check(rc: int, what: str = ""):
    if rc != YOLO2_SUCCESS:
        raise Yolo2HipError(f"{what} failed with status {rc}: {lib().yolo2_hip_last_error().decode()}")



class DevBuf:

    def __init__(self, arr: np.ndarray = None, nbytes: int = None, fill: int = 0):
        self.nbytes = arr.nbytes if arr is not None else nbytes
        a = C.c_uint64(0)
        check(lib().yolo2_hip_alloc(max(self.nbytes, 16), C.byref(a)), "yolo2_hip_alloc")
        self.addr = a.value
        if arr is not None:
            arr = np.ascontiguousarray(arr)
            check(lib().yolo2_hip_memcpy_h2d(self.addr, arr.ctypes.data_as(C.c_void_p), arr.nbytes), "h2d")
        else:
            check(lib().yolo2_hip_memset(self.addr, fill, self.nbytes), "memset")

    def get(self, dtype, shape) -> np.ndarray:
        out = np.empty(shape, dtype=dtype)
        check(lib().yolo2_hip_memcpy_d2h(out.ctypes.data_as(C.c_void_p), self.addr, out.nbytes), "d2h")
        return out

    def free(self):
        if self.addr:
            lib().yolo2_hip_free(self.addr)
            self.addr = 0

    def __del__(self):
        try:
            self.free()
        except Exception:
            pass


def w8(w):
    return (w + 7) // 8 * 8


def conv_layer_i16(x, w_reorg, bias, C_, N, K, stride, W, H, pad, leaky, Qw, Qa_in, Qa_out, Qb, fill=0):
    OW = (W - K + 2 * pad) // stride + 1
    OH = (H - K + 2 * pad) // stride + 1
    TR = min(min((27 - K) // stride + 1, 13), OH)
    TC = min(min((27 - K) // stride + 1, 13), OW)
    TM, TN = min(N, 32), min(C_, 4)
    mLoops = -(-N // TM)
    bx, bw, bb = DevBuf(x), DevBuf(w_reorg), DevBuf(bias)
    out0 = np.full((N, OH, w8(OW)), fill, dtype=np.int16)
    by = DevBuf(out0)
    rc = lib().yolo2_execute_conv_layer(bx.addr, by.addr, bw.addr, bb.addr, C_, N, K, stride, W, H, OW, OH, pad,
                                        int(leaky), 0, TM, TN, TR, TC, (mLoops + 1) * TM, mLoops * TM,
                                        (mLoops + 1) * TM, 0, Qw, Qa_in, Qa_out, Qb, 60000)
    check(rc, "yolo2_execute_conv_layer")
    y = by.get(np.int16, (N, OH, w8(OW)))
    for b in (bx, bw, bb, by):
        b.free()
    return y


def conv_layer_f32(x, w_reorg, bias, C_, N, K, stride, W, H, pad, leaky):
    OW = (W - K + 2 * pad) // stride + 1
    OH = (H - K + 2 * pad) // stride + 1
    bx, bw, bb = DevBuf(x), DevBuf(w_reorg), DevBuf(bias)
    by = DevBuf(np.zeros((N, OH, w8(OW)), dtype=np.float32))
    check(lib().yolo2_execute_conv_layer_f32(bx.addr, by.addr, bw.addr, bb.addr, C_, N, K, stride, W, H, OW, OH,
                                             pad, int(leaky), 60000), "yolo2_execute_conv_layer_f32")
    y = by.get(np.float32, (N, OH, w8(OW)))
    for b in (bx, bw, bb, by):
        b.free()
    return y


def maxpool_layer_i16(x, C_, W, H, K=2, stride=2):
    OW, OH = W // stride, H // stride
    TR = min((27 - K) // stride + 1, 13, OH)
    TC = min((27 - K) // stride + 1, 13, OW)
    TM = min(4, C_)
    mLoops = -(-C_ // TM)
    bx = DevBuf(x)
    by = DevBuf(np.zeros((C_, OH, w8(OW)), dtype=np.int16))
    check(lib().yolo2_execute_maxpool_layer(bx.addr, by.addr, C_, K, stride, W, H, OW, OH, 1, TM, TR, TC,
                                            (mLoops + 2) * TM, mLoops * TM, (mLoops + 1) * TM, 60000),
          "yolo2_execute_maxpool_layer")
    y = by.get(np.int16, (C_, OH, w8(OW)))
    bx.free(); by.free()
    return y



# ... 421 lines not shown
```

Baseline: 3249.

## Add autotuned edge-tile ordering modes and 32-bit byte offsets for grouped loads

Adds two alternative orderings for the edge-classified conv tiles: interior first, and frame-windowed interleaving of the classes. The autotuner now times all three orders per edge layer and stores the choice in the plan cache. This is meant to improve cache locality and load balance across the tile schedule. Grouped tile staging switches to 32-bit byte offsets, guarded by a stride limit, to cut address arithmetic. A multi-frame mode for the single-layer driver and an all-taps debug flag are also added.

New measurement: 3270 (median of 6 runs). No clear change (+0.6%).

```diff
diff --git a/include/yolo2_hip.h b/include/yolo2_hip.h
--- a/include/yolo2_hip.h
+++ b/include/yolo2_hip.h
@@ -172,6 +172,7 @@
 int yolo2_hip_i16_plan_check(int splits, int cg_out, int npix, size_t cap_bytes);
 size_t yolo2_hip_ks_scratch_bytes(yolo2_hip_ctx *ctx);
 int yolo2_hip_i16_edge_map(int B, int H, int W, int cap, int *tile_cls, int *tile_mask, int *pix, long long *steps);
+int yolo2_hip_i16_edge_map2(int B, int H, int W, int order, int cap, int *tile_cls, int *tile_mask, int *pix, long long *steps);
 
 int yolo2_hip_run_frame_fp32_host(yolo2_hip_ctx *ctx, const float *frame, float *region);
 
diff --git a/yolo-fpga-accelerator_amd/csrc/conv_common.hpp b/yolo-fpga-accelerator_amd/csrc/conv_common.hpp
--- a/yolo-fpga-accelerator_amd/csrc/conv_common.hpp
+++ b/yolo-fpga-accelerator_amd/csrc/conv_common.hpp
@@ -38,6 +38,9 @@
     int e_n[5];
     int e_rem[6];
     unsigned mH2, sH2, mW2, sW2, mI2, sI2;
+    int e_order;
+    int e_F;
+    int e_pf[5];
 };
 
 inline void set_conv_div(ConvArgs &a)
@@ -79,6 +82,9 @@
 
 __host__ __device__ constexpr int edge_class_mask(int cls)
 {
+#ifdef Y2_EDGE_ALL_TAPS
+    return 0x1ff;
+#endif
     return cls == kEdgeTop ? 0x1f8 : cls == kEdgeBottom ? 0x03f : cls == kEdgeLeft ? 0x1b6 : cls == kEdgeRight ? 0x0db : 0x1ff;
 }
 
@@ -89,8 +95,50 @@
     return (t + ((n - t) >> 1)) >> s;
 }
 
+__host__ __device__ inline int edge_class_tiles(const ConvArgs &a, int c)
+{
+    return c == kEdgeInterior ? a.e_int : a.e_band[c] - (c ? a.e_band[c - 1] : 0);
+}
+
+__host__ __device__ inline int edge_tiles_before_frame(const ConvArgs &a, int c, int f)
+{
+    const int v = (f * a.e_pf[c] + 63) >> 6, T = edge_class_tiles(a, c);
+    return v < T ? v : T;
+}
+__host__ __device__ inline int edge_tiles_before_window(const ConvArgs &a, int w)
+{
+    const int f = w * a.e_F < a.B ? w * a.e_F : a.B;
+    int s = 0;
+    for (int c = 0; c < 5; ++c) s += edge_tiles_before_frame(a, c, f);
+    return s;
+}
+
 __host__ __device__ inline int edge_tile_class(const ConvArgs &a, int tile, int &ct)
 {
+    if (a.e_order) {
+        const int nf = a.e_nb + a.e_int;
+        if (tile >= nf) { ct = tile - nf; return kEdgeMixed; }
+        int w0 = 0, w1 = 0, o = tile;
+        if (a.e_order == 2) {
+            int lo = 0, hi = (a.B + a.e_F - 1) / a.e_F - 1;
+            while (lo < hi) {
+                const int mid = (lo + hi + 1) >> 1;
+                if (edge_tiles_before_window(a, mid) <= tile) lo = mid; else hi = mid - 1;
+            }
+            o = tile - edge_tiles_before_window(a, lo);
+            w0 = lo * a.e_F;
+            w1 = w0 + a.e_F < a.B ? w0 + a.e_F : a.B;
+        }
+        for (int k = 0; k < 5; ++k) {
+            const int c = k ? k - 1 : kEdgeInterior;
+            const int t0 = a.e_order == 2 ? edge_tiles_before_frame(a, c, w0) : 0;
+            const int t1 = a.e_order == 2 ? edge_tiles_before_frame(a, c, w1) : edge_class_tiles(a, c);
+            if (o < t1 - t0) { ct = t0 + o; return c; }
+            o -= t1 - t0;
+        }
+        ct = 0;
+        return kEdgeMixed;
+    }
     const unsigned nb = (unsigned)a.e_nb, nt = (unsigned)a.e_nt;
     const int c0 = (int)((unsigned)tile * nb / nt), c1 = (int)((unsigned)(tile + 1) * nb / nt);
     if (c1 > c0) {
@@ -154,9 +202,12 @@
     const long n[5] = {B * W, B * W, B * (H - 2), B * (H - 2), B * (H - 2) * (W - 2)};
     if (n[4] + 2 * n[0] + 2 * n[2] >= (1L << 30)) return 0;
     a.e_rem[0] = 0;
+    a.e_order = 0;
+    a.e_F = a.B;
     int nb = 0;
     for (int c = 0; c < 5; ++c) {
         a.e_n[c] = (int)n[c];
+        a.e_pf[c] = (int)(n[c] / B);
         a.e_rem[c + 1] = a.e_rem[c] + (int)(n[c] % 64);
         if (c < 4) { nb += (int)(n[c] / 64); a.e_band[c] = nb; }
     }
@@ -190,6 +241,22 @@
     return lt;
 }
 
+inline void edge_order_plan(ConvArgs &a, int order, int gy)
+{
+    a.e_order = order < 0 || order > 2 ? 0 : order;
+    a.e_F = a.B;
+    if (a.e_order != 2) return;
+    int span = 1;
+    for (int c = 0; c < 5; ++c)
+        if (edge_class_tiles(a, c) > 0) span = span > (63 + a.e_pf[c]) / a.e_pf[c] + 1 ? span : (63 + a.e_pf[c]) / a.e_pf[c] + 1;
+    const long gen_tiles = 2048 / (gy > 0 ? gy : 1) > 0 ? 2048 / (gy > 0 ? gy : 1) : 1;
+    long F = (gen_tiles * a.B + a.e_nt / 2) / a.e_nt;
+    if (F > (a.B + 1) / 2) F = (a.B + 1) / 2;
+    if (F < span) F = span;
+    if (F > a.B) F = a.B;
+    a.e_F = (int)F;
+}
+
 inline long edge_tiles_steps(const ConvArgs &a)
 {
     return 64L * (6L * a.e_nb + 9L * (a.e_nt - a.e_nb));
diff --git a/yolo-fpga-accelerator_amd/csrc/kernels_int16.hpp b/yolo-fpga-accelerator_amd/csrc/kernels_int16.hpp
--- a/yolo-fpga-accelerator_amd/csrc/kernels_int16.hpp
+++ b/yolo-fpga-accelerator_amd/csrc/kernels_int16.hpp
@@ -271,13 +271,14 @@
 
     int2 stage[NST];
     const int buf_items = a.lt_max * GRP;
-    auto src_off = [&](int i) -> long { if (GRP == 1) return i; const int g = i / Lt; return (long)g * a.in_cg_stride + (i - g * Lt); };
+    auto src_off = [&](int i) -> unsigned { const int g = i / Lt; return (unsigned)(((long)g * a.in_cg_stride + (i - g * Lt)) * 8); };
     auto lds_off = [&](int i) -> int { if (GRP == 1) return i; const int g = i / Lt; return g * a.lt_max + (i - g * Lt); };
+    auto src_at = [&](unsigned byte_off) -> int2 { return *reinterpret_cast<const int2 *>(reinterpret_cast<const char *>(src) + byte_off); };
     const int LtG = Lt * GRP;
 #pragma unroll
     for (int k = 0; k < NST; ++k) {
         const int i = tid + k * 256;
-        if (i < LtG) stage[k] = src[EDGE ? soff[k] : src_off(i)];
+        if (i < LtG) stage[k] = EDGE ? src[soff[k]] : (GRP == 1 ? src[i] : src_at(src_off(i)));
     }
 #pragma unroll
     for (int k = 0; k < NST; ++k) {
@@ -304,7 +305,7 @@
 #pragma unroll
         for (int k = 0; k < NST; ++k) {
             const int i = tid + k * 256;
-            if (i < LtG) stage[k] = src[EDGE ? soff[k] : src_off(i)];
+            if (i < LtG) stage[k] = EDGE ? src[soff[k]] : (GRP == 1 ? src[i] : src_at(src_off(i)));
         }
 #endif
         const char *tile = lds_b + (cg & 1) * buf_items * 8;
diff --git a/yolo-fpga-accelerator_amd/csrc/y2_internal.hpp b/yolo-fpga-accelerator_amd/csrc/y2_internal.hpp
--- a/yolo-fpga-accelerator_amd/csrc/y2_internal.hpp
+++ b/yolo-fpga-accelerator_amd/csrc/y2_internal.hpp
@@ -42,6 +42,7 @@
     int poolfuse = -1;
     bool no_poolfuse = false, no_hiacc = false, no_ks = false, no_w16 = false, no_grp = false, grp16 = false, no_xcd_remap = false, splitk_no_pack = false,
          no_edge_tiles = false;
+    int edge_order = -1;
     int f16_lanes = 2;
     bool f16_no_lanes = false, f16_no_mfma0 = false, f16_no_glds = false, f16_no_poolfuse = false, f16_no_halo = false, f16_no_persist = false,
          f16_persist_all = false, f16_ring_all = false, f16_no_ring = false, f16_no_c32 = false, f16_m16 = false, f16_w8 = false, f16_no_wide = false,
@@ -49,6 +50,7 @@
     int stamp_layer = -1;
     int f16_skip = 0;
     int force_path = -1, force_p = 0, force_ks = 0, f32_p = 0;
+    int drv_frames = 1;
     bool force_w16 = false, force_hiacc = false;
 
     static Y2Options from_env();
@@ -59,7 +61,8 @@
 const Y2Options &y2_process_options();
 
 
-struct Y2PlanLine { int path, P, pad, splitk, pp, w16, fuse, hiacc, ks; };
+struct Y2PlanLine { int path, P, pad, splitk, pp, w16, fuse, hiacc, ks, order; };
+std::string y2_plan_line_text(int B, int L, int S, const Y2PlanLine &pl);
 typedef std::pair<int, std::pair<int, int>> Y2PlanKey;
 bool y2_plan_line_parse(const char *text, Y2PlanKey *key, Y2PlanLine *pl);
 bool y2_plan_table_has_batch(const Y2Options &opt, int B);
@@ -115,6 +118,7 @@
     int ks = 0;
     int hiacc = 0;
     int w16 = 0;
+    int order = 0;
     int grp = 1;
     int pool_fused = 0;
     int lds_pad = 0;
diff --git a/yolo-fpga-accelerator_amd/csrc/yolo2_int16.hip b/yolo-fpga-accelerator_amd/csrc/yolo2_int16.hip
--- a/yolo-fpga-accelerator_amd/csrc/yolo2_int16.hip
+++ b/yolo-fpga-accelerator_amd/csrc/yolo2_int16.hip
@@ -108,7 +108,7 @@
     a.lt_max = tile_items_bound(gin, T, halo);
     if (p.w16) p.lds_pad = 0;
     if (p.hiacc && (p.path != 4 || p.splitk || p.w16 || p.P > 4)) p.hiacc = 0;
-    p.grp = (!p.splitk && p.K == 1 && p.path != 2 && gin.CG % 8 == 0 && a.lt_max * 8 <= kMaxTileItems && !opt.no_grp) ? 8 : 1;
+    p.grp = (!p.splitk && p.K == 1 && p.path != 2 && gin.CG % 8 == 0 && a.lt_max * 8 <= kMaxTileItems && gin.cg_stride < (1L << 25) && !opt.no_grp) ? 8 : 1;
     if (p.grp == 8 && opt.grp16 && gin.CG % 16 == 0 && a.lt_max * 16 <= kMaxTileItems && p.P <= 2 && (p.path == 3 || p.path == 4) && !p.hiacc) p.grp = 16;
     p.lds_bytes = p.splitk ? p.splitk * (a.lt_max + p.K * p.K * 32 + 4) * 8 * 2 : std::max(a.lt_max * p.grp * 8 * 2, p.lds_pad);
     p.grid = dim3((npix + T - 1) / T, p.mb_count ? p.mb_count : (p.N + 31) / 32, 1);
@@ -123,8 +123,10 @@
             a.lt_max = lt;
             p.lds_bytes = std::max(lt * 8 * 2, p.lds_pad);
             p.grid.x = a.e_nt;
-        }
-    }
+            edge_order_plan(a, opt.edge_order >= 0 ? opt.edge_order : p.order, (int)p.grid.y);
+        }
+    }
+    if (!a.edge) p.order = 0;
     a.xcd_remap = 0;
     if (!opt.no_xcd_remap) {
         const double in_bytes = (double)gin.B * gin.CG * gin.PL * 8;
@@ -156,7 +158,7 @@
     const int lt = pool_tile_items_bound(gin);
     if (lt > 12 * 256) return false;
     ConvArgs &a = p.args;
-    p.splitk = 0; p.splitk_pp = 1; p.grp = 1; p.P = 4; p.lds_pad = 0; p.w16 = 0; p.hiacc = 0; p.ks = 0;
+    p.splitk = 0; p.splitk_pp = 1; p.grp = 1; p.P = 4; p.lds_pad = 0; p.w16 = 0; p.hiacc = 0; p.ks = 0; p.order = 0;
     a.edge = 0;
     p.pool_fused = full ? 2 : 1;
     a.lt_max = lt;
@@ -686,6 +688,7 @@
                 cand.w16 = w16 ? 1 : 0;
                 cand.hiacc = hiacc ? 1 : 0;
                 cand.ks = ks;
+                cand.order = 0;
                 if (w16 && o.no_w16) continue;
                 if (cfg >= 12 && !w16) {
                     if (!sp->splitk_ok || !c->extra[i].empty() || fs == 0) continue;
@@ -729,7 +732,32 @@
             sp->w16 = bestW16;
             sp->hiacc = bestHi;
             sp->ks = bestKs;
+            sp->order = 0;
             plan_conv(*sp, tin.g, tout.g.cg_stride, out_base, CGout, o, bestP);
+            if (sp->args.edge && o.edge_order < 0) {
+                float tord[3] = {1e30f, 1e30f, 1e30f};
+                for (int rep = 0; rep < 3; ++rep)
+                    for (int k = 0; k < 3; ++k) {
+                        ConvPlan cand = *sp;
+                        cand.order = k;
+                        plan_conv(cand, tin.g, tout.g.cg_stride, out_base, CGout, o, bestP);
+                        (void)hipMemsetAsync(flush, rep, flush_bytes, nullptr);
+                        (void)hipEventRecord(e0, nullptr);
+                        const int lrc = launch_conv(cand, tin.d, tout.d, (const int2 *)(c->wpk + c->wpk_off[ord]), c->bias_pk + c->bias_off[ord], nullptr);
+                        if (lrc) return lrc;
+                        (void)hipEventRecord(e1, nullptr);
+                        HIP_TRY(hipEventSynchronize(e1), YOLO2_ERROR);
+                        float t = 0;
+                        HIP_TRY(hipEventElapsedTime(&t, e0, e1), YOLO2_ERROR);
+                        tord[k] = std::min(tord[k], t);
+                    }
+                int bestO = 0;
+                for (int k = 1; k < 3; ++k)
+                    if (tord[k] < tord[0] * 0.99f && tord[k] < tord[bestO]) bestO = k;
+                if (o.verbose) fprintf(stderr, "[yolo2_hip] tune L%d path %d: tile order 0 / 1 / 2: %.1f / %.1f / %.1f us -> %d\n", i, sp->path, tord[0] * 1e3, tord[1] * 1e3, tord[2] * 1e3, bestO);
+                sp->order = bestO;
+                plan_conv(*sp, tin.g, tout.g.cg_stride, out_base, CGout, o, bestP);
+            }
         }
         ord++;
     }
@@ -802,10 +830,11 @@
             if (!look(c, c->batch, i, (int)s, &pl) || pl.path != subs[s]->path) return YOLO2_SUCCESS;
             ConvPlan cand = *subs[s];
             cand.lds_pad = pl.pad; cand.splitk = pl.splitk; cand.splitk_pp = pl.pp; cand.w16 = pl.w16; cand.hiacc = pl.hiacc; cand.ks = pl.ks;
+            cand.order = pl.order;
             cand.ks_cap = s == 0 ? ks_potential_bytes(c, c->batch) : 0;
             plan_conv(cand, tin.g, tout.g.cg_stride, out_base, (kNet[i].n + 3) / 4, c->opt, pl.P);
             if (cand.P != pl.P || cand.lds_pad != pl.pad || cand.splitk != pl.splitk || cand.splitk_pp != pl.pp || cand.w16 != pl.w16 ||
-                cand.hiacc != pl.hiacc || cand.ks != pl.ks) {
+                cand.hiacc != pl.hiacc || cand.ks != pl.ks || cand.order != pl.order) {
                 if (c->opt.verbose)
                     fprintf(stderr, "[yolo2_hip] %s: layer %d launch %zu at batch %d: the planner refuses the line (P %d/%d pad %d/%d splitk %d/%d pp %d/%d "
                             "w16 %d/%d hiacc %d/%d ks %d/%d) - timing instead\n", what, i, s, c->batch, cand.P, pl.P, cand.lds_pad, pl.pad, cand.splitk, pl.splitk,
@@ -838,8 +867,8 @@
         for (auto &e : c->extra[i]) subs.push_back(&e);
         for (size_t s = 0; s < subs.size(); ++s) {
             const Y2PlanLine pl{subs[s]->path, subs[s]->P, subs[s]->lds_pad, subs[s]->splitk, subs[s]->splitk_pp, subs[s]->w16,
-                                s == 0 && c->fuse_pool[i] ? 1 : 0, subs[s]->hiacc, subs[s]->ks};
-            if (f) fprintf(f, "%d %d %zu %d %d %d %d %d %d %d %d %d\n", c->batch, i, s, pl.path, pl.P, pl.pad, pl.splitk, pl.pp, pl.w16, pl.fuse, pl.hiacc, pl.ks);
+                                s == 0 && c->fuse_pool[i] ? 1 : 0, subs[s]->hiacc, subs[s]->ks, s == 0 && c->fuse_pool[i] ? 0 : subs[s]->order};
+            if (f) fprintf(f, "%s\n", y2_plan_line_text(c->batch, i, (int)s, pl).c_str());
             if (pc) {
                 std::lock_guard<std::mutex> lk(pc->mu);
                 const Y2PlanKey k{c->batch, {i, (int)s}};
@@ -1146,8 +1175,8 @@
         if (kNet[i].type == L_CONV) {
             if (o == ord) {
                 const ConvPlan &pl = c->fuse_pool[i] ? c->fplan[i] : c->plan[i];
-                snprintf(buf, (size_t)cap, "P=%d pad=%d w16=%d hiacc=%d ks=%d splitk=%d pp=%d grp=%d fused=%d form=%d extra=%zu edge=%d", pl.P, pl.lds_pad, pl.w16,
-                         pl.hiacc, pl.ks, pl.splitk, pl.splitk_pp, pl.grp, pl.pool_fused, pl.path, c->extra[i].size(), pl.args.edge);
+                snprintf(buf, (size_t)cap, "P=%d pad=%d w16=%d hiacc=%d ks=%d splitk=%d pp=%d grp=%d fused=%d form=%d extra=%zu edge=%d order=%d", pl.P, pl.lds_pad, pl.w16,
+                         pl.hiacc, pl.ks, pl.splitk, pl.splitk_pp, pl.grp, pl.pool_fused, pl.path, c->extra[i].size(), pl.args.edge, pl.args.edge ? pl.args.e_order : 0);
                 return YOLO2_SUCCESS;
             }
             o++;
@@ -1342,14 +1371,17 @@
 {
     hipStream_t st = nullptr;
     g_last_edge = 0;
+    const Y2Options &popt = y2_process_options();
+    const int B = popt.drv_frames;
     const int so = qa_in + qw - qa_out, sb = qb - qa_out;
     if (!g_scr.bound) HIP_TRY(hipMalloc((void **)&g_scr.bound, 4 * sizeof(int)), YOLO2_MMAP_ERROR);
     bool tiled = kstride == 1 && ((ksize == 3 && padding == 1) || (ksize == 1 && padding == 0));
     if (tiled) {
-        const ActGeom g = make_geom(ifm_num, input_h, input_w, 1);
+        const ActGeom g = make_geom(ifm_num, input_h, input_w, B);
         if (tile_items_bound(g, 64, ksize == 3 ? g.Wp + 1 : 0) > kMaxTileItems) tiled = false;
     }
     if (!tiled) {
+        if (B != 1) return fail(YOLO2_ERROR, "drv_frames = %d: only the tiled kernels (stride 1, 3x3 pad 1 or 1x1 pad 0) take several frames", B);
         *path_out = -1;
         const int n = ofm_num * output_h * output_w;
         hipLaunchKernelGGL(k_conv_ref_i16, dim3(blocks_for(n, 256)), dim3(256), 0, st, in, out, w, beta, ifm_num, ofm_num,
@@ -1358,7 +1390,7 @@
         return YOLO2_SUCCESS;
     }
 
-    const ActGeom gi = make_geom(ifm_num, input_h, input_w, 1), go = make_geom(ofm_num, output_h, output_w, 1);
+    const ActGeom gi = make_geom(ifm_num, input_h, input_w, B), go = make_geom(ofm_num, output_h, output_w, B);
     const long wpk_elems = packed_weight_elems(ifm_num, ofm_num, ksize);
     const int MB = (ofm_num + 31) / 32;
     int rc;
@@ -1370,8 +1402,10 @@
     HIP_TRY(hipMemsetAsync(g_scr.bias_pk, 0, (size_t)MB * 32 * 2, st), YOLO2_DMA_ERROR);
     HIP_TRY(hipMemsetAsync(g_scr.bound, 0, sizeof(int), st), YOLO2_DMA_ERROR);
     HIP_TRY(hipMemcpyAsync(g_scr.bias_pk, beta, (size_t)ofm_num * 2, hipMemcpyDeviceToDevice, st), YOLO2_DMA_ERROR);
-    hipLaunchKernelGGL(k_ref_to_items, dim3(blocks_for((long)ifm_num * input_h * input_w, 256)), dim3(256), 0, st, in,
-                       (short *)g_scr.in_items, ifm_num, input_h, input_w, (input_w + 7) & ~7, gi.Wp, gi.cg_stride);
+    for (int b = 0; b < B; ++b)
+        hipLaunchKernelGGL(k_ref_to_items, dim3(blocks_for((long)ifm_num * input_h * input_w, 256)), dim3(256), 0, st,
+                           in + (long)b * ifm_num * input_h * ((input_w + 7) & ~7), (short *)g_scr.in_items + (long)b * gi.PL * 4, ifm_num, input_h, input_w,
+                           (input_w + 7) & ~7, gi.Wp, gi.cg_stride);
     hipLaunchKernelGGL((k_repack_weights<short>), dim3(blocks_for(wpk_elems, 256)), dim3(256), 0, st, w, (short *)g_scr.wpk,
                        ifm_num, ofm_num, ksize * ksize);
     hipLaunchKernelGGL(k_weight_bound, dim3(std::min<unsigned>(blocks_for(wpk_elems / 4, 256), 1024)), dim3(256), 0, st,
@@ -1387,7 +1421,6 @@
     p.args.mb_list = nullptr;
     p.C = ifm_num; p.N = ofm_num; p.K = ksize; p.H = input_h; p.W = input_w; p.leaky = is_nl ? 1 : 0;
     p.Qw = qw; p.Qa_in = qa_in; p.Qa_out = qa_out; p.Qb = qb;
-    const Y2Options &popt = y2_process_options();
     p.path = choose_path(so, sb, maxsum, maxb, maxabs, popt.force_path);
     if (p.path == 4) {
         HIP_TRY(hipMemsetAsync(g_scr.bound + 3, 16 - so, 1, st), YOLO2_DMA_ERROR);
@@ -1398,9 +1431,10 @@
     *path_out = p.path;
     g_last_edge = p.args.edge;
     if ((rc = launch_conv(p, (const int2 *)g_scr.in_items, (int2 *)g_scr.out_items, (const int2 *)g_scr.wpk, (const short *)g_scr.bias_pk, st))) return rc;
-    hipLaunchKernelGGL(k_items_to_ref, dim3(blocks_for((long)ofm_num * output_h * output_w, 256)), dim3(256), 0, st,
-                       (const short *)g_scr.out_items, out, ofm_num, output_h, output_w, (output_w + 7) & ~7, go.Wp, go.PL,
-                       go.cg_stride, 0);
+    for (int b = 0; b < B; ++b)
+        hipLaunchKernelGGL(k_items_to_ref, dim3(blocks_for((long)ofm_num * output_h * output_w, 256)), dim3(256), 0, st,
+                           (const short *)g_scr.out_items, out + (long)b * ofm_num * output_h * ((output_w + 7) & ~7), ofm_num, output_h, output_w,
+                           (output_w + 7) & ~7, go.Wp, go.PL, go.cg_stride, b);
     HIP_TRY(hipGetLastError(), YOLO2_ERROR);
     return YOLO2_SUCCESS;
 }
diff --git a/yolo-fpga-accelerator_amd/csrc/yolo2_plan.hip b/yolo-fpga-accelerator_amd/csrc/yolo2_plan.hip
--- a/yolo-fpga-accelerator_amd/csrc/yolo2_plan.hip
+++ b/yolo-fpga-accelerator_amd/csrc/yolo2_plan.hip
@@ -32,7 +32,8 @@
     {"autotune", &Y2Options::autotune, -1, 1}, {"lanes", &Y2Options::lanes, 0, 8}, {"lane_priority", &Y2Options::lane_priority, 0, 1},
     {"splitk", &Y2Options::splitk, -1, 1}, {"poolfuse", &Y2Options::poolfuse, -1, 1}, {"f16_lanes", &Y2Options::f16_lanes, 1, 8},
     {"stamp_layer", &Y2Options::stamp_layer, -1, 31}, {"f16_skip", &Y2Options::f16_skip, 0, 63}, {"force_path", &Y2Options::force_path, -1, 4}, {"force_p", &Y2Options::force_p, 0, 8},
-    {"force_ks", &Y2Options::force_ks, 0, 16}, {"f32_p", &Y2Options::f32_p, 0, 4},
+    {"force_ks", &Y2Options::force_ks, 0, 16}, {"f32_p", &Y2Options::f32_p, 0, 4}, {"edge_order", &Y2Options::edge_order, -1, 2},
+    {"drv_frames", &Y2Options::drv_frames, 1, 64},
 };
 const StrOpt kStrs[] = {
     {"plan_file", &Y2Options::plan_file}, {"plan_write", &Y2Options::plan_write}, {"lane_split", &Y2Options::lane_split},
@@ -148,6 +149,12 @@
 
 extern "C" int yolo2_hip_i16_edge_map(int B, int H, int W, int cap, int *tile_cls, int *tile_mask, int *pix, long long *steps)
 {
+    return yolo2_hip_i16_edge_map2(B, H, W, 0, cap, tile_cls, tile_mask, pix, steps);
+}
+
+extern "C" int yolo2_hip_i16_edge_map2(int B, int H, int W, int order, int cap, int *tile_cls, int *tile_mask, int *pix, long long *steps)
+{
+    if (order < 0 || order > 2) return fail(YOLO2_ERROR, "edge tiles: order %d (0, 1 or 2)", order);
     if (B <= 0 || H <= 0 || W <= 0) return fail(YOLO2_ERROR, "edge tiles: empty geometry %d x %d x %d", B, H, W);
     const y2::ActGeom g = y2::make_geom(4, H, W, B);
     y2::ConvArgs a{};
@@ -155,6 +162,7 @@
     a.npix = B * H * W;
     y2::set_conv_div(a);
     if (!y2::edge_tiles_plan(a)) return 0;
+    y2::edge_order_plan(a, order, 1);
     if (steps) *steps = y2::edge_tiles_steps(a);
     if (tile_cls && tile_mask && pix) {
         if (cap < a.e_nt) return fail(YOLO2_ERROR, "edge tiles: %d tiles, room for %d", a.e_nt, cap);
@@ -178,18 +186,26 @@
 {
     int B, L, S;
     Y2PlanLine pl;
-    pl.hiacc = pl.ks = 0;
-    if (line[0] == '#' || sscanf(line, "%d %d %d %d %d %d %d %d %d %d %d %d", &B, &L, &S, &pl.path, &pl.P, &pl.pad, &pl.splitk, &pl.pp, &pl.w16, &pl.fuse,
-                                 &pl.hiacc, &pl.ks) < 10)
+    pl.hiacc = pl.ks = pl.order = 0;
+    if (line[0] == '#' || sscanf(line, "%d %d %d %d %d %d %d %d %d %d %d %d %d", &B, &L, &S, &pl.path, &pl.P, &pl.pad, &pl.splitk, &pl.pp, &pl.w16, &pl.fuse,
+                                 &pl.hiacc, &pl.ks, &pl.order) < 10)
         return false;
     auto one_of = [](int v, std::initializer_list<int> ok) { for (int o : ok) if (v == o) return true; return false; };
     if (B <= 0 || B > 4096 || L < 0 || L >= 32 || S < 0 || S > 8 || !one_of(pl.path, {0, 1, 2, 3, 4}) || !one_of(pl.P, {1, 2, 4, 8}) ||
         !one_of(pl.pad, {0, 160 * 1024 / 6, 160 * 1024 / 4}) || !one_of(pl.splitk, {0, 4, 8}) || !one_of(pl.pp, {1, 2, 4}) ||
-        !one_of(pl.w16, {0, 1}) || !one_of(pl.fuse, {0, 1}) || !one_of(pl.hiacc, {0, 1}) || !one_of(pl.ks, {0, 2, 4, 8, 16}))
+        !one_of(pl.w16, {0, 1}) || !one_of(pl.fuse, {0, 1}) || !one_of(pl.hiacc, {0, 1}) || !one_of(pl.ks, {0, 2, 4, 8, 16}) || !one_of(pl.order, {0, 1, 2}))
         return false;
     *key = {B, {L, S}};
     *out = pl;
     return true;
+}
+
+std::string y2_plan_line_text(int B, int L, int S, const Y2PlanLine &p)
+{
+    char buf[160];
+    int n = snprintf(buf, sizeof(buf), "%d %d %d %d %d %d %d %d %d %d %d %d", B, L, S, p.path, p.P, p.pad, p.splitk, p.pp, p.w16, p.fuse, p.hiacc, p.ks);
+    if (p.order) snprintf(buf + n, sizeof(buf) - (size_t)n, " %d", p.order);
+    return buf;
 }
 
 namespace {
@@ -352,9 +368,7 @@
     }
     for (const auto &kv : lines) {
         const Y2PlanLine &p = kv.second;
-        snprintf(buf, sizeof(buf), "plan %d %d %d %d %d %d %d %d %d %d %d %d\n", kv.first.first, kv.first.second.first, kv.first.second.second, p.path, p.P,
-                 p.pad, p.splitk, p.pp, p.w16, p.fuse, p.hiacc, p.ks);
-        body += buf;
+        body += "plan " + y2_plan_line_text(kv.first.first, kv.first.second.first, kv.first.second.second, p) + "\n";
     }
     snprintf(buf, sizeof(buf), "sum %016llx\n", (unsigned long long)y2_hash_bytes(0, body.data(), body.size()));
     const std::string tmp = path + ".tmp." + std::to_string((long)getpid());
diff --git a/yolo-fpga-accelerator_amd/yolo2_amd/hipdrv.py b/yolo-fpga-accelerator_amd/yolo2_amd/hipdrv.py
--- a/yolo-fpga-accelerator_amd/yolo2_amd/hipdrv.py
+++ b/yolo-fpga-accelerator_amd/yolo2_amd/hipdrv.py
@@ -37,7 +37,7 @@
     "yolo2_hip_fp16_layer_kernel", "yolo2_hip_f16_store_check",
     "yolo2_hip_run_images_u8_dets", "yolo2_hip_multi_run_images_u8_dets", "yolo2_hip_set_fp16_lanes", "yolo2_hip_conv_plan_string", "yolo2_hip_plan_source",
     "yolo2_hip_set_option", "yolo2_hip_options_string", "yolo2_hip_set_plan_cache", "yolo2_hip_plan_cache_info", "yolo2_hip_plan_cache_check",
-    "yolo2_hip_i16_plan_check", "yolo2_hip_ks_scratch_bytes", "yolo2_hip_i16_edge_map", "yolo2_hip_last_layer_edge",
+    "yolo2_hip_i16_plan_check", "yolo2_hip_ks_scratch_bytes", "yolo2_hip_i16_edge_map", "yolo2_hip_i16_edge_map2", "yolo2_hip_last_layer_edge",
     "yolo2_hip_run_batch_f32tol", "yolo2_hip_run_batch_f32tol_host", "yolo2_hip_f32tol_layer_kernel", "yolo2_hip_num_lanes_f32tol",
     "yolo2_hip_debug_f16_tensor",
     "yolo2_hip_run_images_u8_f16_host", "yolo2_hip_run_images_u8_dets_f16", "yolo2_hip_multi_run_images_u8_dets_f16",
@@ -164,6 +164,7 @@
     sig("yolo2_hip_plan_cache_check", [C.c_char_p, u64, pi32])
     sig("yolo2_hip_i16_plan_check", [i32, i32, i32, C.c_size_t])
     sig("yolo2_hip_i16_edge_map", [i32, i32, i32, i32, vp, vp, vp, vp])
+    sig("yolo2_hip_i16_edge_map2", [i32, i32, i32, i32, i32, vp, vp, vp, vp])
     sig("yolo2_hip_last_layer_edge", [], i32)
     sig("yolo2_hip_run_batch_f32tol", [vp, u64, i32, u64, vp])
     sig("yolo2_hip_run_batch_f32tol_host", [vp, vp, i32, vp])
```
